# cjpurackal/nice-slam-cpp

Hardware: AMD Instinct MI355X
Metric: mapping rays/sec (and ms/iter) on CoFusion room1 at 1/2/4/8 MI355X (higher is better)
Workload: dtype f32

## Files before the change

nice-slam-cpp_amd/csrc/nsk.hip:

```cpp
#include "../../include/nsk.h"
#include "nsk_device.h"
#include "nsk_train.h"
#include "nsk_bf16.h"
#include "nsk_mesh.h"
#include "nsk_buf.h"

#include <dlfcn.h>
#include <cstdarg>
#include <algorithm>
#include <cmath>
#include <cstdio>
#include <cstring>
#include <memory>
#include <string>
#include <vector>

#define NSK_VERSION 100

static thread_local std::string g_err;
static int fail(const char* fmt, ...)
{
    char buf[512];
    va_list ap; va_start(ap, fmt); vsnprintf(buf, sizeof(buf), fmt, ap); va_end(ap);
    g_err = buf;
// ... 505 lines not shown
    float incl = act ? (1.f - alpha + 1e-10f) : 1.f;
#pragma unroll
    for (int o = 1; o < 64; o <<= 1) { float up = __shfl_up(incl, o); if (lane >= o) incl *= up; }
    float T = __shfl_up(incl, 1);
    if (lane == 0) T = 1.f;
    const float w = act ? alpha * T : 0.f;
    const float D = wave_sum(w * z);
    const float cr = wave_sum(w * r4[0]), cg = wave_sum(w * r4[1]), cb = wave_sum(w * r4[2]);
    const float V = wave_sum(w * (z - D) * (z - D));
    if (weights && act) weights[m] = w;
    if (lane == 0) { depth[n] = D; var[n] = V; rgb[3 * n] = cr; rgb[3 * n + 1] = cg; rgb[3 * n + 2] = cb; }
}

__device__ __forceinline__ void voxel_point(const float* b, int Z, int Y, int X, int v, float (&p)[3])
{
    int ix = v % X, iy = (v / X) % Y, iz = v / (X * Y);
    p[0] = add_rn(b[0], mul_rn(sub_rn(b[1], b[0]), linspace01(ix, X)));
    p[1] = add_rn(b[2], mul_rn(sub_rn(b[3], b[2]), linspace01(iy, Y)));
    p[2] = add_rn(b[4], mul_rn(sub_rn(b[5], b[4]), linspace01(iz, Z)));
}
struct FrustumArgs { float bound[6]; float w2c[16]; float cam[3]; int Z, Y, X, H, W; float fx, fy, cx, cy; };
__global__ void k_frustum_pass1(FrustumArgs A, const float* __restrict__ img, float* __restrict__ dep, float* __restrict__ zz,
                                uint8_t* __restrict__ inimg, unsigned int* __restrict__ dmax_bits)
{
    const int n = A.Z * A.Y * A.X;
    const int v = blockIdx.x * blockDim.x + threadIdx.x;
    float d = 0.f;
    if (v < n) {
        float p[3], cam[3];
        voxel_point(A.bound, A.Z, A.Y, A.X, v, p);
        for (int a = 0; a < 3; ++a)
            cam[a] = add_rn(add_rn(add_rn(mul_rn(A.w2c[4 * a], p[0]), mul_rn(A.w2c[4 * a + 1], p[1])), mul_rn(A.w2c[4 * a + 2], p[2])), A.w2c[4 * a + 3]);
        cam[0] = -cam[0];
        const float z = add_rn(cam[2], 1e-5f);
        const float u = div_rn(add_rn(mul_rn(A.fx, cam[0]), mul_rn(A.cx, cam[2])), z);
        const float w = div_rn(add_rn(mul_rn(A.fy, cam[1]), mul_rn(A.cy, cam[2])), z);
        const float x0 = floorf(u), y0 = floorf(w);
        const float ax = sub_rn(u, x0), ay = sub_rn(w, y0);
        const int ix = (int)x0, iy = (int)y0;
        float s = 0.f;
        for (int dy = 0; dy < 2; ++dy) for (int dx = 0; dx < 2; ++dx) {
            int x = ix + dx, y = iy + dy;
            if (x < 0 || x >= A.W || y < 0 || y >= A.H) continue;
            s = add_rn(s, mul_rn(mul_rn(dx ? ax : sub_rn(1.f, ax), dy ? ay : sub_rn(1.f, ay)), img[(size_t)y * A.W + x]));
        }
        d = s;
        dep[v] = d; zz[v] = z;
        inimg[v] = (u < (float)A.W && u > 0.f && w < (float)A.H && w > 0.f) ? 1 : 0;
    }
    float m = wave_max(fmaxf(d, 0.f));
    if ((threadIdx.x & 63) == 0) atomicMax(dmax_bits, __float_as_uint(m));
}
__global__ void k_frustum_pass2(FrustumArgs A, const float* __restrict__ dep, const float* __restrict__ zz, const uint8_t* __restrict__ inimg,
                                const unsigned int* __restrict__ dmax_bits, uint8_t* __restrict__ mask)
{
    const int n = A.Z * A.Y * A.X;
    const int v = blockIdx.x * blockDim.x + threadIdx.x;
    if (v >= n) return;
    const float dmax = __uint_as_float(*dmax_bits);
    const float d = dep[v] == 0.f ? dmax : dep[v];
    const float nz = -zz[v];
    int m = inimg[v] && (0.f <= nz) && (nz <= add_rn(d, 0.5f));
    float p[3];
    voxel_point(A.bound, A.Z, A.Y, A.X, v, p);
    const float dx = sub_rn(p[0], A.cam[0]), dy = sub_rn(p[1], A.cam[1]), dz = sub_rn(p[2], A.cam[2]);
    if (add_rn(add_rn(mul_rn(dx, dx), mul_rn(dy, dy)), mul_rn(dz, dz)) < 0.25f) m = 1;
    mask[v] = (uint8_t)m;
}

struct OverlapArgs { int N, ns, H, W, K; float fx, fy, cx, cy; };
__global__ __launch_bounds__(256) void k_keyframe_overlap(OverlapArgs A, const float* __restrict__ ro, const float* __restrict__ rd,
                                                           const float* __restrict__ gd, const float* __restrict__ w2c_all,
                                                           float* __restrict__ percent)
{
    __shared__ int sh[4];
    const float* w2c = w2c_all + 16 * blockIdx.x;
    const int total = A.N * A.ns;
    int count = 0;
    for (int i = threadIdx.x; i < total; i += blockDim.x) {
        const int n = i / A.ns, s = i - n * A.ns;
        const float nearv = mul_rn(gd[n], 0.8f), farv = add_rn(gd[n], 0.5f);
        const float t = linspace01(s, A.ns);
        const float z = add_rn(mul_rn(nearv, sub_rn(1.f, t)), mul_rn(farv, t));
        float p[3], cam[3];
        for (int a = 0; a < 3; ++a) p[a] = add_rn(ro[3 * n + a], mul_rn(rd[3 * n + a], z));
        for (int a = 0; a < 3; ++a)
            cam[a] = add_rn(add_rn(add_rn(mul_rn(w2c[4 * a], p[0]), mul_rn(w2c[4 * a + 1], p[1])), mul_rn(w2c[4 * a + 2], p[2])), w2c[4 * a + 3]);
        cam[0] = -cam[0];
        const float zc = add_rn(cam[2], 1e-5f);
        const float u = div_rn(add_rn(mul_rn(A.fx, cam[0]), mul_rn(A.cx, cam[2])), zc);
        const float v = div_rn(add_rn(mul_rn(A.fy, cam[1]), mul_rn(A.cy, cam[2])), zc);
        if (u < (float)(A.W - 20) && u > 20.f && v < (float)(A.H - 20) && v > 20.f && zc < 0.f) ++count;
    }
#pragma unroll
    for (int o = 32; o > 0; o >>= 1) count += __shfl_xor(count, o);
    if ((threadIdx.x & 63) == 0) sh[threadIdx.x >> 6] = count;
    __syncthreads();
    if (threadIdx.x == 0) percent[blockIdx.x] = div_rn((float)(sh[0] + sh[1] + sh[2] + sh[3]), (float)total);
}

__global__ void k_sample_pixels(unsigned long long seed, int n, int H0, int W0, int Ww, unsigned long long total, int* __restrict__ pi,
                                int* __restrict__ pj)
{
    const int r = blockIdx.x * blockDim.x + threadIdx.x;
    if (r >= n) return;
    const unsigned long long ind = ((unsigned long long)hash_u32(seed, (uint32_t)r, 0x51u) * total) >> 32;
    pi[r] = W0 + (int)(ind % (unsigned long long)Ww);
    pj[r] = H0 + (int)(ind / (unsigned long long)Ww);
}
__global__ void k_gather_pixels(int n, const int* __restrict__ pi, const int* __restrict__ pj, int W, const float* __restrict__ depth,
                                const float* __restrict__ color, float* __restrict__ gd, float* __restrict__ gc)
{
    const int r = blockIdx.x * blockDim.x + threadIdx.x;
    if (r >= n) return;
    const size_t p = (size_t)pj[r] * W + pi[r];
    gd[r] = depth[p];
    if (color && gc) { gc[3 * r] = color[3 * p]; gc[3 * r + 1] = color[3 * p + 1]; gc[3 * r + 2] = color[3 * p + 2]; }
}

struct HipAlloc {
    static int alloc(void** p, size_t bytes) { return (int)hipMalloc(p, bytes); }
    static void free(void* p) { (void)hipFree(p); }
};
template <typename T> using Buf = DevBuf<T, HipAlloc>;

struct GridState {
    int C = 0, Z = 0, Y = 0, X = 0;
    size_t n = 0;
    Buf<float> v, m, s;
    Buf<uint8_t> mask;
    size_t g_off = 0;
    Buf<int> midx; int nmask = 0; bool midx_dirty = true;
};
struct DecState {
    int n = 0;
    Buf<float> p, m, s;
    Buf<float> fimg, bimg;
    Buf<int> fidx, bidx;
    Buf<int> finv, binv;
    Buf<int> inv16;
    Buf<int> invh;
    Buf<float> bimg16; Buf<int> bidx16; int bfrag16_n = 0; bool bimg16_dirty = true;
    Buf<float> fimg16; Buf<int> fidx16; int frag16_n = 0, fimg16_f = 0, tail_off = 0, tail16_off = 0, np16 = 3, cq16 = 2;
    int fimg_n = 0, bimg_n = 0;
    int trainable = 0;
    bool loaded = false;
    size_t g_off = 0;
};
struct Workspace {
    int capM = 0, capN = 0;
    Buf<float> z, occ[3], rgb4;
    Buf<unsigned long long> masks[4];
    Buf<f4> hsave[4];
    int hsave_M[4] = {0, 0, 0, 0};
    Buf<float> g_raw, ray_loss;
    Buf<float> tmp_rgb, tmp_depth, tmp_var;
    Buf<float> dec_slabs;
    Buf<int> perm, skey, srank;
    Buf<int> hist_raw, offs;
    int* hist() const { return hist_raw ? hist_raw.get() + 16 : nullptr; }
    Buf<float> z_alt; Buf<int> perm_alt, skey_alt, srank_alt, offs_alt;
};
struct nsk_ctx {
    int device = 0;
    hipStream_t stream = nullptr;
    bool own_stream = false;
    int num_cu = 256;
    RParams R;
    Buf<float> d_bound;
    GridState grid[4];
    DecState dec[4];
    Buf<float> slab; size_t slab_n = 0;
    Buf<float> xbuf; size_t xbuf_n = 0;
    bool x_identity = false;
    bool xlevels[4] = {false, false, false, false}; bool xdecs[4] = {false, false, false, false};
    Workspace ws;
    Buf<float> scal;
    Buf<uint8_t> fr_tmp;
    int adam_step[NSK_NUM_GROUPS] = {0, 0, 0, 0, 0, 0};
    bool capturing = false;
    struct CapAdam { AdamArgs args; int group[8]; float lr[8]; };
    std::vector<CapAdam> cap_adams;
    struct CapVec { int n; float* p; const float* g; float* m; float* v; float lr, b1, b2, eps; int step; hipGraphNode_t node; float ss, bc2s; };
    std::vector<CapVec> cap_vecs;
    int cap_rollback[NSK_NUM_GROUPS] = {0, 0, 0, 0, 0, 0};
    int ws_flip = 0;
    struct GraphRec { bool stale = false; int flip = 0; hipGraph_t graph = nullptr; hipGraphExec_t exec = nullptr; hipGraphNode_t adam_node = nullptr; bool has_adam = false; CapAdam adam; std::vector<CapVec> vecs; };
    std::vector<GraphRec> graphs;
    bool touched[NSK_NUM_GROUPS] = {false, false, false, false, false, false};
    bool deterministic = false;
    bool roctx = false;
    int tune_fwd_occ_cost = 0, tune_no_occ_role = 0;
    int tune_fwd_fine_cost = 0, tune_fwd_color_cost = 0;
    bool median_fused_pending = false;
    int tune_no_deferred_median = 0;
    int tune_no_fused_median = 0;
    int tune_frozen_cost = 0;
    int tune_frozen_cost_rays = 0;
    int tune_frozen_mid_pct = 100;
    int tune_no_frozen_kernel = 0;
    const uint8_t* ray_mask = nullptr;
    struct DMax { const float* gt = nullptr; const uint8_t* keep = nullptr; int n = 0; } dmax;
    float* xextra = nullptr; size_t xextra_n = 0;
    int sort_mode = -1;
    bool sorted = false;
    struct Prep { bool valid = false; int stage = 0, N = 0, S = 0; const float* ro = nullptr; const float* rd = nullptr; const float* gt = nullptr;
                  float gtmax = 0.f; const uint8_t* mask = nullptr; bool sorted = false; int done = 0; RParams R; DMax dmax; } prep, req;
    int tune_no_piggyback = 0;
    int pend_w = -1, pend_nb = 0;
    int dbg_M = 0, dbg_S = 0;
    int bwd_mode = 2;
    int matmul_mode = 2;
    double last_bytes = 0, last_flops = 0; int last_samples = 0;
    struct Mesh {
        Buf<float> lat_pts;
        int slab = 0;
        Buf<uint8_t> cellcase; Buf<int> emap;
        Buf<unsigned> scan;
        Buf<int8_t> table; Buf<uint8_t> ntri;
        Buf<float> verts; Buf<int> tris;
        int nv = 0, nt = 0;
    } mesh;
    bool prof = false;
    struct ProfRec { const char* name; hipEvent_t a, b; };
    std::vector<ProfRec> prof_recs;
    ~nsk_ctx();
};

typedef int (*roctx_push_t)(const char*);
typedef int (*roctx_pop_t)(void);
static roctx_push_t g_roctx_push = nullptr;
static roctx_pop_t g_roctx_pop = nullptr;
static bool roctx_ready()
{
    static int state = 0;
    if (state == 0) {
        void* h = dlopen("libroctx64.so", RTLD_NOW | RTLD_GLOBAL);
        if (!h) h = dlopen("libroctx64.so.4", RTLD_NOW | RTLD_GLOBAL);
        if (h) { g_roctx_push = (roctx_push_t)dlsym(h, "roctxRangePushA"); g_roctx_pop = (roctx_pop_t)dlsym(h, "roctxRangePop"); }
        state = (g_roctx_push && g_roctx_pop) ? 1 : -1;
    }
    return state == 1;
}

struct ProfScope {
    nsk_ctx* c; hipEvent_t a = nullptr, b = nullptr; const char* name; bool ranged = false;
    ProfScope(nsk_ctx* c_, const char* n, bool on = true) : c(c_), name(n)
    {
        if (!on) return;
        if (c->roctx && roctx_ready()) { g_roctx_push(n); ranged = true; }
        if (!c->prof) return;
        hipEventCreate(&a); hipEventCreate(&b);
        hipEventRecord(a, c->stream);
    }
    ~ProfScope()
    {
        if (ranged) g_roctx_pop();
        if (!c->prof || !a) return;
        hipEventRecord(b, c->stream);
        c->prof_recs.push_back({name, a, b});
    }
};

static void invalidate_graphs(nsk_ctx* c)
{
    for (auto& R : c->graphs) {
        if (R.stale) continue;
        if (R.exec) { hipGraphExecDestroy(R.exec); R.exec = nullptr; }
        if (R.graph) { hipGraphDestroy(R.graph); R.graph = nullptr; }
        R.stale = true;
    }
}

nsk_ctx::~nsk_ctx()
{
    hipSetDevice(device);
    if (stream) hipStreamSynchronize(stream);
    invalidate_graphs(this);
    for (auto& r : prof_recs) { hipEventDestroy(r.a); hipEventDestroy(r.b); }
    if (own_stream && stream) hipStreamDestroy(stream);
}

template <typename T>
static int dev_alloc(Buf<T>& b, size_t n, const char* what)
{
    const int e = b.alloc(n);
    if (e == 0) return 0;
    (void)hipGetLastError();
    return fail("cannot allocate %zu bytes for %s (%s)", n * sizeof(T), what, hipGetErrorString((hipError_t)e));
}
enum { GROW_NO_CAPTURE = 1,
       GROW_STALE_GRAPHS = 2 };
static int grow_begin(nsk_ctx* c, unsigned flags)
{
    if ((flags & GROW_NO_CAPTURE) && c->capturing) return fail("graph capture: the workspace must grow (run the same step once before nsk_graph_begin)");
    HIPCHK(hipStreamSynchronize(c->stream));
    if (flags & GROW_STALE_GRAPHS) invalidate_graphs(c);
    return 0;
}
template <typename T>
static int grow(nsk_ctx* c, Buf<T>& b, size_t n, const char* what, unsigned flags)
{
    if (n <= b.cap()) return 0;
    CHK(grow_begin(c, flags));
    return dev_alloc(b, n, what);
}

extern "C" const char* nsk_last_error(void) { return g_err.c_str(); }
extern "C" int nsk_version(void) { return NSK_VERSION; }

static int which_ok(int w) { return w >= 0 && w < 4; }

template <typename K>
static int set_lds(K kern, size_t bytes)
{
    HIPCHK(hipFuncSetAttribute(reinterpret_cast<const void*>(kern), hipFuncAttributeMaxDynamicSharedMemorySize, (int)bytes));
    return 0;
}

static size_t fwd_img_floats(int w) { return w == 0 ? CoarseFwdImg::TOTAL : (w == 2 ? MlpFwdImg<4>::TOTAL : MlpFwdImg<2>::TOTAL); }
static size_t bwd_img_floats(int w) { return w == 0 ? CoarseBwdImg::TOTAL : MlpBwdImg::TOTAL; }
static size_t bwd_lds_bytes(int w, bool train)
{
    size_t scratch = 8 * 3840;
    if (!train) return bwd_img_floats(w) * 4 + scratch;
    if (w == 1 || w == 3) return PM_LDS_BYTES;
    size_t img = w == 2 ? 0 : bwd_img_floats(w);
    return (img + PN_FLOATS(w == 2 ? 4 : 2)) * 4;
}

extern "C" int nsk_ctx_create(int device, void* hip_stream, nsk_ctx** out)
{
    if (!out) return fail("nsk_ctx_create: out is NULL");
    int ndev = 0;
    hipError_t e = hipGetDeviceCount(&ndev);
    if (e != hipSuccess || ndev <= 0) return fail("nsk_ctx_create: no HIP device (the MI355X kernels have no CPU fallback)");
    if (device < 0 || device >= ndev) return fail("nsk_ctx_create: device %d out of range (%d devices)", device, ndev);
    HIPCHK(hipSetDevice(device));
    hipDeviceProp_t prop;
    HIPCHK(hipGetDeviceProperties(&prop, device));
    if (strncmp(prop.gcnArchName, "gfx950", 6) != 0) return fail("nsk_ctx_create: device arch %s, this library is built for gfx950 only", prop.gcnArchName);
    std::unique_ptr<nsk_ctx> owner(new nsk_ctx());
    nsk_ctx* c = owner.get();
    c->device = device;
    c->num_cu = prop.multiProcessorCount;
    if (hip_stream) { c->stream = (hipStream_t)hip_stream; c->own_stream = false; }
    else { HIPCHK(hipStreamCreateWithFlags(&c->stream, hipStreamNonBlocking)); c->own_stream = true; }
    const float b[6] = {-4.5f, 3.82f, -1.5f, 2.02f, -3.0f, 2.76f};
    memcpy(c->R.bound, b, sizeof(b));
    c->R.n_samples = 32; c->R.n_surface = 16; c->R.lindisp = 0; c->R.occupancy = 0; c->R.perturb = 0.f; c->R.seed = 0;
    CHK(dev_alloc(c->d_bound, 6, "the bound"));
    HIPCHK(hipMemcpy(c->d_bound, b, sizeof(b), hipMemcpyHostToDevice));
    CHK(dev_alloc(c->scal, 16, "the scalars"));
    HIPCHK(hipMemset(c->scal, 0, 16 * sizeof(float)));
    CHK(set_lds(k_decode_fwd<0>, fwd_img_floats(0) * 4)); CHK(set_lds(k_decode_fwd<1>, fwd_img_floats(1) * 4));
    CHK(set_lds(k_decode_fwd<2>, fwd_img_floats(2) * 4)); CHK(set_lds(k_decode_fwd<3>, fwd_img_floats(3) * 4));
#define SETB(W) \
    CHK(set_lds(k_decode_bwd<W, false>, bwd_lds_bytes(W, false))); CHK(set_lds(k_decode_bwd<W, true>, bwd_lds_bytes(W, false))); \
    CHK(set_lds(k_decode_bwd_train<W, false>, bwd_lds_bytes(W, true))); CHK(set_lds(k_decode_bwd_train<W, true>, bwd_lds_bytes(W, true)));
    SETB(0) SETB(1) SETB(2) SETB(3)
#undef SETB
    CHK(set_lds(k_median_thr, 16384 * 4));
    CHK(set_lds(k_decode_fwd_multi, 160 * 1024)); CHK(set_lds(k_decode_fwd_multi_bf16<8>, 160 * 1024)); CHK(set_lds(k_decode_fwd_multi_bf16<8, 2>, 160 * 1024)); CHK(set_lds(k_decode_fwd_multi_occ<8>, 160 * 1024));
    CHK(set_lds(k_decode_bwd_multi<false>, 160 * 1024 - 256)); CHK(set_lds(k_decode_bwd_multi<true>, 160 * 1024));
    CHK(set_lds(k_decode_bwd_frozen<false>, 160 * 1024 - 256));
    CHK(set_lds(k_decode_bwd_track, 160 * 1024)); CHK(set_lds(k_decode_bwd_multi_full<false>, 160 * 1024)); CHK(set_lds(k_decode_bwd_multi_full<true>, 160 * 1024));
    CHK(set_lds(k_decode_fwd_dump<0>, 160 * 1024)); CHK(set_lds(k_decode_fwd_dump<1>, 160 * 1024)); CHK(set_lds(k_decode_fwd_dump<2>, 160 * 1024));
    *out = owner.release();
    return 0;
}

extern "C" int nsk_ctx_destroy(nsk_ctx* c)
{
    delete c;
    return 0;
}

extern "C" int nsk_sync(nsk_ctx* c)
{
    if (!c) return fail("null ctx");
    HIPCHK(hipStreamSynchronize(c->stream));
    if (c->median_fused_pending) {
        c->median_fused_pending = false;
        unsigned bar[3] = {0, 0, 0};
        HIPCHK(hipMemcpy(bar, c->scal + 5, sizeof(bar), hipMemcpyDeviceToHost));
        if (bar[2]) {
            HIPCHK(hipMemset(c->scal + 5, 0, sizeof(bar)));
            return fail("nsk_track_step: the grid barrier of the fused median timed out (threshold was infinite for that step); nsk_set_tuning(\"no_fused_median\", 1) selects the three-launch form");
        }
    }
    return 0;
}
extern "C" void* nsk_stream(nsk_ctx* c) { return c ? (void*)c->stream : nullptr; }

static int repack16(nsk_ctx* c, int w);
extern "C" int nsk_set_matmul_mode(nsk_ctx* c, int mode)
{
    if (!c) return fail("null ctx");
    if (mode < 0 || mode > 2) return fail("nsk_set_matmul_mode: mode must be 0 (fp32 MFMA), 1 (bf16 3-piece split) or 2 (fp16 2-piece split)");
    if (c->capturing) return fail("nsk_set_matmul_mode: not while a graph is being captured");
    const bool relayout = (mode == 2) != (c->matmul_mode == 2);
    c->matmul_mode = mode;
    if (relayout) {
        HIPCHK(hipSetDevice(c->device));
        for (int w = 1; w < 4; ++w) if (c->dec[w].loaded && c->dec[w].fimg16) CHK(repack16(c, w));
        invalidate_graphs(c);
    }
    return 0;
}

extern "C" int nsk_set_backward_mode(nsk_ctx* c, int mode)
{
    if (!c) return fail("null ctx");
    if (mode != 0 && mode != 2) return fail("nsk_set_backward_mode: 0 (fp32 MFMA chains) or 2 (two fp16 pieces, default)");
    c->bwd_mode = mode;
    return 0;
}

extern "C" int nsk_set_tuning(nsk_ctx* c, const char* key, int value)
{
    if (!c || !key) return fail("nsk_set_tuning: null argument");
    if (!strcmp(key, "frozen_cost")) { c->tune_frozen_cost = value; return 0; }
    if (!strcmp(key, "frozen_cost_rays")) { c->tune_frozen_cost_rays = value; return 0; }
    if (!strcmp(key, "no_frozen_kernel")) { c->tune_no_frozen_kernel = value; return 0; }
    if (!strcmp(key, "no_piggyback")) { c->tune_no_piggyback = value; return 0; }
    if (!strcmp(key, "frozen_mid_pct")) { if (value < 10 || value > 1000) return fail("nsk_set_tuning: frozen_mid_pct out of range"); c->tune_frozen_mid_pct = value; return 0; }
    if (!strcmp(key, "no_fused_median")) { c->tune_no_fused_median = value; return 0; }
    if (!strcmp(key, "no_deferred_median")) { c->tune_no_deferred_median = value; return 0; }
    if (!strcmp(key, "fwd_fine_cost")) { c->tune_fwd_fine_cost = value; return 0; }
    if (!strcmp(key, "fwd_occ_cost")) { c->tune_fwd_occ_cost = value; return 0; }
    if (!strcmp(key, "no_occ_role")) { c->tune_no_occ_role = value; return 0; }
    if (!strcmp(key, "fwd_color_cost")) { c->tune_fwd_color_cost = value; return 0; }
    if (!strcmp(key, "deterministic")) { c->deterministic = value != 0; return 0; }
    if (!strcmp(key, "roctx")) { c->roctx = value != 0; return 0; }
    if (!strcmp(key, "lattice_slab")) { if (value < 0 || value >= (1 << 26)) return fail("nsk_set_tuning: lattice_slab must be 0 (automatic) or a node count below 2^26"); c->mesh.slab = value; return 0; }
    return fail("nsk_set_tuning: unknown key '%s'", key);
}

extern "C" int nsk_set_ray_mask(nsk_ctx* c, const uint8_t* d_keep)
{
    if (!c) return fail("null ctx");
    c->ray_mask = d_keep;
    return 0;
}

extern "C" int nsk_set_sort_mode(nsk_ctx* c, int mode)
{
    if (!c) return fail("null ctx");
    if (mode < -1 || mode > 1) return fail("nsk_set_sort_mode: mode must be -1 (automatic), 0 (never) or 1 (always)");
    c->sort_mode = mode;
    return 0;
}

extern "C" int nsk_set_bound(nsk_ctx* c, const float h_bound[6])
{
    if (!c || !h_bound) return fail("nsk_set_bound: null argument");
    for (int k = 0; k < 3; ++k) if (!(h_bound[2 * k + 1] > h_bound[2 * k])) return fail("nsk_set_bound: empty axis %d", k);
    memcpy(c->R.bound, h_bound, 6 * sizeof(float));
    HIPCHK(hipMemcpyAsync(c->d_bound, c->R.bound, 6 * sizeof(float), hipMemcpyHostToDevice, c->stream));
    HIPCHK(hipStreamSynchronize(c->stream));
    return 0;
}

extern "C" int nsk_set_render_opts(nsk_ctx* c, int n_samples, int n_surface, int lindisp, float perturb, int occupancy, uint64_t seed)
{
    if (!c) return fail("null ctx");
    if (n_samples < 1 || n_surface < 0 || n_samples + n_surface > 64) return fail("nsk_set_render_opts: need 1 <= n_samples, n_samples+n_surface <= 64 (got %d+%d)", n_samples, n_surface);
    c->R.n_samples = n_samples; c->R.n_surface = n_surface; c->R.lindisp = lindisp ? 1 : 0; c->R.perturb = perturb;
    c->R.occupancy = occupancy ? 1 : 0; c->R.seed = seed;
    return 0;
}

static int rebuild_slab(nsk_ctx* c)
{
    size_t n = 0;
    for (int i = 0; i < 4; ++i) { c->grid[i].g_off = n; n += c->grid[i].n; }
    for (int i = 0; i < 4; ++i) { c->dec[i].g_off = n; n += (size_t)((c->dec[i].n + 3) & ~3); }
    n += 4;
    if (n != c->slab_n) {
        CHK(grow_begin(c, GROW_STALE_GRAPHS));
        c->slab_n = 0;
        CHK(dev_alloc(c->slab, n, "the gradient slab"));
        c->slab_n = n;
    }
    HIPCHK(hipMemsetAsync(c->slab, 0, n * sizeof(float), c->stream));
    return 0;
}

static int grid_upload(nsk_ctx* c, GridState& G, const float* h, int C, int Z, int Y, int X)
{
    size_t nvox = (size_t)Z * Y * X, n = nvox * 32;
    bool realloc_ = n != G.n;
    if (realloc_) {
        CHK(grow_begin(c, GROW_STALE_GRAPHS));
        G = GridState();
        CHK(dev_alloc(G.v, n, "a grid level")); CHK(dev_alloc(G.m, n, "a grid level's first moment")); CHK(dev_alloc(G.s, n, "a grid level's second moment"));
    }
    if (G.Z != Z || G.Y != Y || G.X != X) { if (G.mask) { CHK(grow_begin(c, GROW_STALE_GRAPHS)); G.mask.reset(); } }
    G.C = C; G.Z = Z; G.Y = Y; G.X = X; G.n = n; G.midx_dirty = true;
    std::vector<float> t(n);
    for (int ch = 0; ch < 32; ++ch)
        for (size_t v = 0; v < nvox; ++v) t[v * 32 + ch] = h[(size_t)ch * nvox + v];
    HIPCHK(hipMemcpyAsync(G.v, t.data(), n * 4, hipMemcpyHostToDevice, c->stream));
    HIPCHK(hipMemsetAsync(G.m, 0, n * 4, c->stream));
    HIPCHK(hipMemsetAsync(G.s, 0, n * 4, c->stream));
    HIPCHK(hipStreamSynchronize(c->stream));
    if (realloc_) CHK(rebuild_slab(c));
    return 0;
}
extern "C" int nsk_grid_upload(nsk_ctx* c, int level, const float* h, int C, int Z, int Y, int X)
{
    if (!c || !h) return fail("nsk_grid_upload: null argument");
    if (!which_ok(level)) return fail("nsk_grid_upload: bad level %d", level);
    if (C != 32) return fail("nsk_grid_upload: C must be 32 (got %d)", C);
    if (Z < 1 || Y < 1 || X < 1) return fail("nsk_grid_upload: bad shape");
    if ((size_t)Z * Y * X >= ((size_t)1 << 25)) return fail("nsk_grid_upload: at most 2^25 - 1 voxels per level (32-bit byte offsets in the forward's gather: 128 B per voxel)");
    HIPCHK(hipSetDevice(c->device));
    GridState& G = c->grid[level];
    const bool fresh = (size_t)Z * Y * X * 32 != G.n;
    const int r = grid_upload(c, G, h, C, Z, Y, X);
    if (r != 0 && fresh) { invalidate_graphs(c); G = GridState(); }
    return r;
}

static int grid_fetch(nsk_ctx* c, int level, const float* src, float* h)
{
    GridState& G = c->grid[level];
    if (!G.n) return fail("grid level %d not uploaded", level);
    std::vector<float> t(G.n);
    HIPCHK(hipMemcpyAsync(t.data(), src, G.n * 4, hipMemcpyDeviceToHost, c->stream));
    HIPCHK(hipStreamSynchronize(c->stream));
    size_t nvox = G.n / 32;
    for (int ch = 0; ch < 32; ++ch)
        for (size_t v = 0; v < nvox; ++v) h[(size_t)ch * nvox + v] = t[v * 32 + ch];
    return 0;
}
extern "C" int nsk_grid_download(nsk_ctx* c, int level, float* h)
{
    if (!c || !h || !which_ok(level)) return fail("nsk_grid_download: bad argument");
    return grid_fetch(c, level, c->grid[level].v, h);
}
extern "C" int nsk_grid_grad_download(nsk_ctx* c, int level, float* h)
{
    if (!c || !h || !which_ok(level)) return fail("nsk_grid_grad_download: bad argument");
    CHK(grid_fetch(c, level, c->slab + c->grid[level].g_off, h));
    GridState& G = c->grid[level];
    if (G.mask) {
        const size_t nvox = G.n / 32;
        std::vector<uint8_t> m(nvox);
        HIPCHK(hipMemcpy(m.data(), G.mask, nvox, hipMemcpyDeviceToHost));
        for (int ch = 0; ch < 32; ++ch)
            for (size_t v = 0; v < nvox; ++v) if (!m[v]) h[(size_t)ch * nvox + v] = 0.f;
    }
    return 0;
}

extern "C" int nsk_set_mask(nsk_ctx* c, int level, const uint8_t* h_mask)
{
    if (!c || !which_ok(level)) return fail("nsk_set_mask: bad argument");
    GridState& G = c->grid[level];
    if (!G.n) return fail("nsk_set_mask: grid level %d not uploaded", level);
    if (c->capturing) return fail("nsk_set_mask: not while a graph is being captured");
    HIPCHK(hipStreamSynchronize(c->stream));
    size_t nvox = G.n / 32;
    G.midx_dirty = true;
    invalidate_graphs(c);
    if (c->slab) HIPCHK(hipMemsetAsync(c->slab + G.g_off, 0, G.n * 4, c->stream));
    if (!h_mask) { G.mask.reset(); return 0; }
    if (!G.mask) CHK(dev_alloc(G.mask, nvox, "the voxel mask"));
    HIPCHK(hipMemcpy(G.mask, h_mask, nvox, hipMemcpyHostToDevice));
    return 0;
}

static void seg_fwd(std::vector<int>& idx, int quad0, int KQ, int Wofs, int ld, int col0, int kvalid)
{
    for (int rt = 0; rt < 2; ++rt) for (int q = 0; q < KQ; ++q) for (int lane = 0; lane < 64; ++lane) for (int i = 0; i < 4; ++i) {
        int o = 16 * rt + (lane & 15), k = 16 * q + 4 * (lane >> 4) + i;
// ... 125 lines not shown
    k_pack<<<(D.bimg_n + 255) / 256, 256, 0, c->stream>>>(D.bimg, D.bidx, D.p, D.bimg_n);
    HIPCHK(hipGetLastError());
    CHK(repack16(c, w));
    D.bimg16_dirty = true;
    return 0;
}

static int flush_pending(nsk_ctx* c);
static int ensure_midx(nsk_ctx* c, int l);
static void adam_consts(float lr, float b1, float b2, int step, float& step_size, float& bc2s);

extern "C" size_t nsk_decoder_param_count(int which) { return which_ok(which) ? (size_t)nsk_dec_layout(which).total : 0; }

static int dec_setup(int w, size_t n, DecState& D)
{
    const size_t n4 = (n + 3) & ~(size_t)3;
    auto table = [](Buf<int>& d, const std::vector<int>& h, const char* what) -> int {
        CHK(dev_alloc(d, h.size(), what));
        HIPCHK(hipMemcpy(d, h.data(), h.size() * 4, hipMemcpyHostToDevice));
        return 0;
    };
    auto inverse = [&](Buf<int>& d, const std::vector<int>& idx, const char* image) -> int {
        std::vector<int> inv(n4, -1);
        for (size_t k = 0; k < idx.size(); ++k) if (idx[k] >= 0) { if (inv[idx[k]] != -1) return fail("decoder %d: parameter %d appears twice in the %s image", w, idx[k], image); inv[idx[k]] = (int)k; }
        return table(d, inv, "a decoder's inverse index table");
    };
    CHK(dev_alloc(D.p, n4, "a decoder's parameters")); CHK(dev_alloc(D.m, n4, "a decoder's first moment")); CHK(dev_alloc(D.s, n4, "a decoder's second moment"));
    HIPCHK(hipMemset(D.p, 0, n4 * 4));
    std::vector<int> fi, bi;
    build_idx(w, fi, bi);
    D.fimg_n = (int)fi.size(); D.bimg_n = (int)bi.size();
    CHK(dev_alloc(D.fimg, fi.size(), "a decoder's forward image")); CHK(dev_alloc(D.bimg, bi.size(), "a decoder's backward image"));
    CHK(table(D.fidx, fi, "a decoder's index table")); CHK(table(D.bidx, bi, "a decoder's index table"));
    if (w != 0) {
        std::vector<int> i16;
        if (w == 2) { build_idx16<4>(nsk_dec_layout(w), i16); D.cq16 = 4; D.tail_off = MlpFwdImg<4>::P_B; }
        else { build_idx16<2>(nsk_dec_layout(w), i16); D.cq16 = 2; D.tail_off = MlpFwdImg<2>::P_B; }
        set_np16(D, 3);
        D.frag16_n = (int)i16.size();
        CHK(dev_alloc(D.fimg16, (size_t)D.fimg16_f, "a decoder's forward image in pieces")); CHK(table(D.fidx16, i16, "a decoder's index table"));
        HIPCHK(hipMemset(D.fimg16, 0, (size_t)D.fimg16_f * 4));
        std::vector<int> ib;
        build_idx16b(nsk_dec_layout(w), ib);
        D.bfrag16_n = (int)ib.size();
        CHK(dev_alloc(D.bimg16, (size_t)MlpBwdImgH::TOTAL_F, "a decoder's backward image in pieces")); CHK(table(D.bidx16, ib, "a decoder's index table"));
        HIPCHK(hipMemset(D.bimg16, 0, (size_t)MlpBwdImgH::TOTAL_F * 4));
        CHK(inverse(D.invh, ib, "fp16 backward"));
        CHK(inverse(D.inv16, i16, "bf16"));
    }
    CHK(inverse(D.finv, fi, "forward"));
    CHK(inverse(D.binv, bi, "backward"));
    D.n = (int)n;
    return 0;
}

extern "C" int nsk_decoder_upload(nsk_ctx* c, int w, const float* h, size_t n)
{
    if (!c || !h || !which_ok(w)) return fail("nsk_decoder_upload: bad argument");
    if (n != nsk_decoder_param_count(w)) return fail("nsk_decoder_upload: decoder %d expects %zu parameters, got %zu", w, nsk_decoder_param_count(w), n);
    HIPCHK(hipSetDevice(c->device));
    DecState& D = c->dec[w];
    if (!D.n) {
        DecState fresh;
        fresh.trainable = D.trainable;
        CHK(dec_setup(w, n, fresh));
        D = std::move(fresh);
        const int r = rebuild_slab(c);
        if (r != 0) { const int t = D.trainable; D = DecState(); D.trainable = t; return r; }
    }
    HIPCHK(hipMemcpyAsync(D.p, h, n * 4, hipMemcpyHostToDevice, c->stream));
    size_t n4 = (n + 3) & ~(size_t)3;
    HIPCHK(hipMemsetAsync(D.m, 0, n4 * 4, c->stream));
    HIPCHK(hipMemsetAsync(D.s, 0, n4 * 4, c->stream));
    CHK(repack(c, w));
    HIPCHK(hipStreamSynchronize(c->stream));
    D.loaded = true;
    return 0;
}

static int dec_fetch(nsk_ctx* c, int w, const float* src, float* h, size_t n)
{
    if (!c->dec[w].loaded) return fail("decoder %d not uploaded", w);
    if (n != (size_t)c->dec[w].n) return fail("decoder %d has %d parameters, buffer has %zu", w, c->dec[w].n, n);
    HIPCHK(hipMemcpyAsync(h, src, n * 4, hipMemcpyDeviceToHost, c->stream));
    HIPCHK(hipStreamSynchronize(c->stream));
    return 0;
}
extern "C" int nsk_decoder_download(nsk_ctx* c, int w, float* h, size_t n)
{
    if (!c || !h || !which_ok(w)) return fail("nsk_decoder_download: bad argument");
    return dec_fetch(c, w, c->dec[w].p, h, n);
}
extern "C" int nsk_decoder_grad_download(nsk_ctx* c, int w, float* h, size_t n)
{
    if (!c || !h || !which_ok(w)) return fail("nsk_decoder_grad_download: bad argument");
    CHK(flush_pending(c));
    return dec_fetch(c, w, c->slab + c->dec[w].g_off, h, n);
}
extern "C" int nsk_decoder_set_trainable(nsk_ctx* c, int w, int t)
{
    if (!c || !which_ok(w)) return fail("nsk_decoder_set_trainable: bad argument");
    c->dec[w].trainable = t ? 1 : 0;
    return 0;
}

static int prep_drop(nsk_ctx* c);
static int ensure_ws(nsk_ctx* c, int N, int M)
{
    Workspace& w = c->ws;
    if (M <= w.capM && N <= w.capN) return 0;
    CHK(grow_begin(c, GROW_NO_CAPTURE | GROW_STALE_GRAPHS));
    CHK(prep_drop(c));
    const int capM = std::max(M, w.capM), capN = std::max(N, w.capN);
    w = Workspace();
    const size_t m = (size_t)capM + 64, n = (size_t)capN + 64, slabs = (size_t)c->num_cu * 20920;
    const int r = [&]() -> int {
        CHK(dev_alloc(w.z, m, "the sample depths"));
        for (int i = 0; i < 3; ++i) CHK(dev_alloc(w.occ[i], m, "the occupancies"));
        CHK(dev_alloc(w.rgb4, m * 4, "the colours"));
        for (int i = 0; i < 4; ++i) CHK(dev_alloc(w.masks[i], m * 4, "the ReLU bits"));
        CHK(dev_alloc(w.g_raw, m * 4, "the sample gradients"));
        CHK(dev_alloc(w.ray_loss, n, "the ray losses"));
        CHK(dev_alloc(w.tmp_rgb, n * 3, "the ray colours")); CHK(dev_alloc(w.tmp_depth, n, "the ray depths")); CHK(dev_alloc(w.tmp_var, n, "the ray variances"));
        CHK(dev_alloc(w.dec_slabs, slabs, "the decoder gradient slabs"));
        HIPCHK(hipMemsetAsync(w.dec_slabs, 0, slabs * 4, c->stream));
        CHK(dev_alloc(w.perm, m, "the cell sort")); CHK(dev_alloc(w.skey, m, "the cell sort")); CHK(dev_alloc(w.srank, m, "the cell sort"));
        return 0;
    }();
    if (r != 0) { w = Workspace(); return r; }
    w.capM = capM; w.capN = capN;
    return 0;
}

static int ensure_hist(nsk_ctx* c, size_t bins)
{
    Workspace& w = c->ws;
    if (bins <= w.offs.cap()) return 0;
    CHK(grow_begin(c, GROW_NO_CAPTURE | GROW_STALE_GRAPHS));
    c->prep.valid = false; c->req.valid = false;
    const size_t slots = ((bins / 8 + 1) / 2) * 16 + 16;
    const int r = [&]() -> int {
        CHK(dev_alloc(w.hist_raw, slots, "the cell histogram")); CHK(dev_alloc(w.offs, bins, "the cell offsets"));
        HIPCHK(hipMemsetAsync(w.hist_raw, 0, slots * 4, c->stream));
        return 0;
    }();
    if (r != 0) reset_all(w.hist_raw, w.offs);
    return r;
}

static bool saves_h(nsk_ctx* c, int w, bool save_masks) { return save_masks && w != 2 && c->dec[w].trainable; }
static int ensure_hsave(nsk_ctx* c, int w, int M)
{
    const size_t tiles = (size_t)(M + 15) / 16 + 1;
    return grow(c, c->ws.hsave[w], tiles * 10 * 64, "the saved block outputs", GROW_NO_CAPTURE | GROW_STALE_GRAPHS);
}

static const int STAGE_DEC[4][3] = {{0, -1, -1}, {1, -1, -1}, {1, 2, -1}, {1, 2, 3}};

static GridD grid_dev(nsk_ctx* c, int level, bool with_grad)
{
    GridD g;
    GridState& G = c->grid[level];
    g.v = G.v; g.g = with_grad ? c->slab + G.g_off : nullptr; g.mask = G.mask; g.Z = G.Z; g.Y = G.Y; g.X = G.X;
    return g;
}

static int check_stage(nsk_ctx* c, int stage)
{
    if (stage < 0 || stage > 3) return fail("bad stage %d", stage);
    for (int q = 0; q < 3; ++q) {
        int w = STAGE_DEC[stage][q];
        if (w < 0) break;
        if (!c->grid[w].n) return fail("stage %d needs grid level %d (nsk_grid_upload)", stage, w);
        if (!c->dec[w].loaded) return fail("stage %d needs decoder %d (nsk_decoder_upload)", stage, w);
    }
    if (!c->slab) return fail("the gradient slab is not allocated (its last allocation failed: upload a grid level or a decoder again)");
    return 0;
}

static void fill_args(nsk_ctx* c, DecArgs& A, int w, int M, int S, const float* ro, const float* rd, const float* pts)
{
    memset(&A, 0, sizeof(A));
    A.rays_o = ro; A.rays_d = rd; A.z = c->ws.z; A.pts = pts; A.M = M; A.S = S; A.S_magic = S > 1 ? (unsigned)((0x100000000ull + (unsigned)S - 1) / (unsigned)S) : 0u;
    A.perm = (c->sorted && !pts) ? c->ws.perm : nullptr;
    memcpy(A.bound, c->R.bound, sizeof(A.bound));
    A.grid = grid_dev(c, w, false);
    if (w == 2) A.grid_mid = grid_dev(c, 1, false);
    A.img = reinterpret_cast<const f4*>(c->dec[w].fimg.get());
    A.bimg = reinterpret_cast<const f4*>(c->dec[w].bimg.get());
    A.img_f4 = c->dec[w].fimg_n / 4;
    A.img16 = c->dec[w].fimg16;
    A.bimg16 = c->dec[w].bimg16;
    A.out = w == 3 ? c->ws.rgb4 : c->ws.occ[w];
}

static int launch_decode_fwd(nsk_ctx* c, int w, int M, int S, const float* ro, const float* rd, const float* pts, bool save_masks)
{
    DecArgs A;
    fill_args(c, A, w, M, S, ro, rd, pts);
    A.masks = save_masks ? c->ws.masks[w] : nullptr;
    if (save_masks) c->ws.hsave_M[w] = 0;
    if (saves_h(c, w, save_masks)) { CHK(ensure_hsave(c, w, M)); A.hsave = c->ws.hsave[w]; c->ws.hsave_M[w] = M; }
    int ntasks = (M + 15) / 16;
    size_t lds = fwd_img_floats(w) * 4;
    int maxwg = c->num_cu;
    int grid = std::max(1, std::min((ntasks + 7) / 8, maxwg));
    static const char* names[4] = {"decode_fwd_coarse", "decode_fwd_middle", "decode_fwd_fine", "decode_fwd_color"};
    ProfScope ps(c, names[w]);
    switch (w) {
    case 0: k_decode_fwd<0><<<grid, 512, lds, c->stream>>>(A); break;
    case 1: k_decode_fwd<1><<<grid, 512, lds, c->stream>>>(A); break;
    case 2: k_decode_fwd<2><<<grid, 512, lds, c->stream>>>(A); break;
    default: k_decode_fwd<3><<<grid, 512, lds, c->stream>>>(A); break;
    }
    HIPCHK(hipGetLastError());
    return 0;
}

static int launch_decode_bwd(nsk_ctx* c, int w, int M, int S, const float* ro, const float* rd, bool train, bool rays, unsigned flags,
                             float* g_ro, float* g_rd)
{
    DecArgs A;
    fill_args(c, A, w, M, S, ro, rd, nullptr);
    A.grid = grid_dev(c, w, (flags & NSK_GRAD_GRIDS) != 0);
    A.masks = c->ws.masks[w];
    A.g_raw = c->ws.g_raw;
    A.g_rays_o = g_ro; A.g_rays_d = g_rd;
    A.g_dec = train ? c->ws.dec_slabs : c->slab + c->dec[w].g_off;
    A.flags = flags;
    if (w != 0 && (!train || w != 2)) CHK(ensure_bimg16(c, w));
    if (train && w != 2) {
        if (c->ws.hsave_M[w] != M) return fail("backward of trainable decoder %d: its forward must run with the decoder already trainable (block outputs not saved)", w);
        A.hsave = c->ws.hsave[w];
    }
    int ntasks = (M + 15) / 16;
    size_t lds = bwd_lds_bytes(w, train);
    int grid = std::max(1, std::min((ntasks + 7) / 8, c->num_cu));
    if (c->deterministic) { grid = 1; A.flags |= 0x8000u; }
    static const char* names[8] = {"decode_bwd_coarse", "decode_bwd_middle", "decode_bwd_fine", "decode_bwd_color",
                                   "decode_bwd_coarse_train", "decode_bwd_middle_train", "decode_bwd_fine_train", "decode_bwd_color_train"};
    {
    ProfScope ps(c, names[w + (train ? 4 : 0)]);
#define LB(W) \
    if (train) { if (rays) k_decode_bwd_train<W, true><<<grid, 512, lds, c->stream>>>(A); else k_decode_bwd_train<W, false><<<grid, 512, lds, c->stream>>>(A); } \
    else { if (rays) k_decode_bwd<W, true><<<grid, 512, lds, c->stream>>>(A); else k_decode_bwd<W, false><<<grid, 512, lds, c->stream>>>(A); }
    switch (w) {
    case 0: LB(0) break;
    case 1: LB(1) break;
    case 2: LB(2) break;
    default: LB(3) break;
    }
#undef LB
    }
    HIPCHK(hipGetLastError());
    if (train) {
        int n = c->dec[w].n, n4 = (n + 3) & ~3;
        ProfScope ps2(c, "dec_grad_reduce");
        k_dec_grad_reduce<<<dim3((n + 255) / 256, 8), 256, 0, c->stream>>>(n, n4, grid, c->ws.dec_slabs, c->slab + c->dec[w].g_off);
        HIPCHK(hipGetLastError());
    }
    return 0;
}

static void split_wgs(int num_cu, int ntasks, int n, const int* cost, int* wg_end, int waves = 8)
{
    int cap = std::max(1, (ntasks + waves - 1) / waves), tot = 0, used = 0;
    for (int r = 0; r < n; ++r) tot += cost[r];
    for (int r = 0; r < n; ++r) {
        int k = std::max(1, (int)((double)num_cu * cost[r] / tot));
        k = std::min(k, cap);
        used += k;
        wg_end[r] = used;
    }
}

static void split_wgs_balanced(int num_cu, int ntasks, int n, const int* cost, int* wg_end, int waves = 8)
{
    split_wgs(num_cu, ntasks, n, cost, wg_end, waves);
    int w[4];
    for (int r = 0; r < n; ++r) w[r] = wg_end[r] - (r ? wg_end[r - 1] : 0);
    int used = wg_end[n - 1];
    const int cap = std::max(1, (ntasks + waves - 1) / waves);
    auto t_of = [&](int r, int wr) { return (long)((ntasks + waves * wr - 1) / (waves * wr)) * cost[r]; };
    for (int r = 0; used < num_cu && r < 8 * n; ++r) {
        int worst = 0;
        for (int q = 1; q < n; ++q) if (t_of(q, w[q]) > t_of(worst, w[worst])) worst = q;
        if (w[worst] >= cap) break;
        ++w[worst]; ++used;
    }
    for (int it = 0; it < 64; ++it) {
        int worst = 0;
        for (int q = 1; q < n; ++q) if (t_of(q, w[q]) > t_of(worst, w[worst])) worst = q;
        const long cur = t_of(worst, w[worst]);
        if (w[worst] >= cap) break;
        int donor = -1; long best = cur;
        for (int q = 0; q < n; ++q) {
            if (q == worst || w[q] <= 1) continue;
            long m = std::max(t_of(q, w[q] - 1), t_of(worst, w[worst] + 1));
            for (int o = 0; o < n; ++o) if (o != q && o != worst) m = std::max(m, t_of(o, w[o]));
            if (m < best) { best = m; donor = q; }
        }
        if (donor < 0) break;
        --w[donor]; ++w[worst];
    }
    int acc = 0;
    for (int r = 0; r < n; ++r) { acc += w[r]; wg_end[r] = acc; }
}

static void split_wgs_train(int num_cu, int ntasks, int n, const int* cost, int train_role, int* wg_end)
{
    const int groups = std::max(1, (ntasks + 7) / 8);
    int fsum = 0;
    for (int r = 0; r < n; ++r) if (r != train_role) fsum += cost[r];
    long best = -1; int best_wt = 1;
    const int wt_max = std::min(groups, num_cu - (n - 1));
    for (int iters = (groups + wt_max - 1) / wt_max; iters <= groups; ++iters) {
        const int wt = (groups + iters - 1) / iters;
        if (wt > wt_max) continue;
        long t = (long)iters * cost[train_role];
        const int rest = num_cu - wt;
        for (int r = 0; r < n; ++r) {
            if (r == train_role) continue;
            const int wr = std::max(1, (int)((long)rest * cost[r] / std::max(1, fsum)));
            t = std::max(t, (long)((ntasks + 8 * wr - 1) / (8 * wr)) * cost[r]);
        }
        if (best < 0 || t < best) { best = t; best_wt = wt; }
        if ((long)iters * cost[train_role] > best) break;
    }
    const int rest = num_cu - best_wt;
    int used = 0;
    for (int r = 0; r < n; ++r) {
        int k = r == train_role ? best_wt : std::max(1, (int)((long)rest * cost[r] / std::max(1, fsum)));
        k = std::min(k, std::max(1, (ntasks + 7) / 8));
        used += k;
        wg_end[r] = used;
    }
}

static long split_makespan(int ntasks, int n, const int* cost, const int* wg_end, int waves = 8)
{
    long t = 0;
    for (int r = 0; r < n; ++r) {
        const int w = std::max(1, wg_end[r] - (r ? wg_end[r - 1] : 0));
        t = std::max(t, (long)((ntasks + waves * w - 1) / (waves * w)) * cost[r]);
    }
    return t;
}

static int launch_decode_fwd_stage(nsk_ctx* c, int stage, int M, int S, const float* ro, const float* rd, bool save_masks)
{
    int n = 0;
    for (int q = 0; q < 3; ++q) if (STAGE_DEC[stage][q] >= 0) ++n;
    if (n == 1) return launch_decode_fwd(c, STAGE_DEC[stage][0], M, S, ro, rd, nullptr, save_masks);
    static const int fcost[4] = {96, 240, 292, 248};
    MultiArgs MA;
    memset(&MA, 0, sizeof(MA));
    if (c->matmul_mode == 2 && c->tune_no_occ_role != 1 && STAGE_DEC[stage][0] == 1 && STAGE_DEC[stage][1] == 2 && !saves_h(c, 1, save_masks) && !saves_h(c, 2, save_masks)) {
        const bool colour = STAGE_DEC[stage][2] == 3;
        for (int r = 0; r < (colour ? 3 : 2); ++r) {
            const int w = STAGE_DEC[stage][r];
            fill_args(c, MA.a[r], w, M, S, ro, rd, nullptr);
            MA.a[r].masks = save_masks ? c->ws.masks[w] : nullptr;
            if (save_masks) c->ws.hsave_M[w] = 0;
            MA.which[r] = w;
        }
        if (colour && saves_h(c, 3, save_masks)) { CHK(ensure_hsave(c, 3, M)); MA.a[2].hsave = c->ws.hsave[3]; c->ws.hsave_M[3] = M; }
        int cost[2] = {c->tune_fwd_occ_cost > 0 ? c->tune_fwd_occ_cost : 460, c->tune_fwd_color_cost > 0 ? c->tune_fwd_color_cost : fcost[3]};
        MA.n = colour ? 2 : 1;
        split_wgs_balanced(c->num_cu, (M + 15) / 16, MA.n, cost, MA.wg_end, 8);
        if (!colour) MA.wg_end[1] = MA.wg_end[0];
        bool merged = true;
        if (c->tune_no_occ_role != 2) {
            int cost3[3], wg3[3], n3 = colour ? 3 : 2;
            for (int r = 0; r < n3; ++r) {
                const int w = STAGE_DEC[stage][r];
                cost3[r] = (w == 2 && c->tune_fwd_fine_cost > 0) ? c->tune_fwd_fine_cost : ((w == 3 && c->tune_fwd_color_cost > 0) ? c->tune_fwd_color_cost : fcost[w]);
            }
            split_wgs_balanced(c->num_cu, (M + 15) / 16, n3, cost3, wg3, 8);
            merged = split_makespan((M + 15) / 16, MA.n, cost, MA.wg_end) <= split_makespan((M + 15) / 16, n3, cost3, wg3);
        }
        if (merged) {
            size_t lds_occ = ((size_t)c->dec[1].fimg16_f + (size_t)c->dec[2].fimg16_f) * 4;
            if (colour) lds_occ = std::max(lds_occ, (size_t)c->dec[3].fimg16_f * 4);
            ProfScope ps(c, "decode_fwd_multi");
            k_decode_fwd_multi_occ<8><<<MA.wg_end[MA.n - 1], 512, lds_occ, c->stream>>>(MA);
            HIPCHK(hipGetLastError());
            return 0;
        }
        memset(&MA, 0, sizeof(MA));
    }
    int cost[3]; size_t lds = 0;
    for (int r = 0; r < n; ++r) {
        int w = STAGE_DEC[stage][r];
        fill_args(c, MA.a[r], w, M, S, ro, rd, nullptr);
        MA.a[r].masks = save_masks ? c->ws.masks[w] : nullptr;
        if (save_masks) c->ws.hsave_M[w] = 0;
        if (saves_h(c, w, save_masks)) { CHK(ensure_hsave(c, w, M)); MA.a[r].hsave = c->ws.hsave[w]; c->ws.hsave_M[w] = M; }
        MA.which[r] = w; cost[r] = (w == 2 && c->tune_fwd_fine_cost > 0) ? c->tune_fwd_fine_cost : ((w == 3 && c->tune_fwd_color_cost > 0) ? c->tune_fwd_color_cost : fcost[w]);
        lds = std::max(lds, fwd_img_floats(w) * 4);
    }
    MA.n = n;
    split_wgs_balanced(c->num_cu, (M + 15) / 16, n, cost, MA.wg_end, 8);
    ProfScope ps(c, "decode_fwd_multi");
    if (c->matmul_mode != 0) {
        size_t lds16 = 0;
        for (int r = 0; r < n; ++r) lds16 = std::max(lds16, MA.which[r] == 0 ? fwd_img_floats(0) * 4 : (size_t)c->dec[MA.which[r]].fimg16_f * 4);
        if (c->matmul_mode == 2) k_decode_fwd_multi_bf16<8, 2><<<MA.wg_end[n - 1], 512, lds16, c->stream>>>(MA);
        else k_decode_fwd_multi_bf16<8><<<MA.wg_end[n - 1], 512, lds16, c->stream>>>(MA);
    } else
    k_decode_fwd_multi<<<MA.wg_end[n - 1], 512, lds, c->stream>>>(MA);
    HIPCHK(hipGetLastError());
    return 0;
}

static void account(nsk_ctx* c, int stage, int M, int N, bool bwd, unsigned flags)
{
    static const double fwd_b[4] = {1024, 1024, 2048, 3072}, fwd_f[4] = {12.4e3, 31.0e3, 72.2e3, 103.3e3};
    double b = fwd_b[stage] + 5.0, f = fwd_f[stage];
    if (bwd) {
        int lv = stage == 0 ? 1 : stage;
        if (flags & NSK_GRAD_GRIDS) b += 2048.0 * lv;
        f *= 2.0;
        if (flags & NSK_GRAD_DECODERS) for (int q = 0; q < 3; ++q) { int w = STAGE_DEC[stage][q]; if (w >= 0 && c->dec[w].trainable) f += 2.0 * (w == 0 ? 6176 : (w == 2 ? 20599 : 15500)); }
    }
    c->last_bytes = b * M; c->last_flops = f * M; c->last_samples = M; (void)N;
}

static bool sort_pays(nsk_ctx* c, int stage, int M, unsigned flags)
{
    if (c->deterministic) return false;
    if (c->sort_mode >= 0) return c->sort_mode == 1;
    if (!(flags & NSK_GRAD_GRIDS)) return false;
    int key_level = 0;
    for (int q = 0; q < 3; ++q) if (STAGE_DEC[stage][q] >= 0) key_level = std::max(key_level, STAGE_DEC[stage][q] == 3 ? 3 : STAGE_DEC[stage][q]);
    const long cells = (long)(c->grid[key_level].n / 32);
    return M >= 14336 || (cells > 0 && (long)M >= 4 * cells);
}

static int stage_key_level(int stage)
{
    int key_level = 0;
    for (int q = 0; q < 3; ++q) if (STAGE_DEC[stage][q] >= 0) key_level = STAGE_DEC[stage][q];
    return key_level;
}
static void samp_args(nsk_ctx* c, SampArgs& A, const RParams& R, int stage, int N, int S, const float* ro, const float* rd, const float* gt, float gtmax,
                      const float* gmax_dev, const uint8_t* mask, bool sorted, float* z, int* skey, int* srank, const nsk_ctx::DMax& dm)
{
    const GridState& KG = c->grid[stage_key_level(stage)];
    const GridState* PG = stage >= 2 ? &c->grid[1] : nullptr;
    const size_t bins = KG.n / 32 * 8;
    memset(&A, 0, sizeof(A));
    A.R = R; A.N = N; A.S = S; A.rays_o = ro; A.rays_d = rd; A.gt_depth = gt; A.gtmax_host = gtmax; A.gtmax_dev = gmax_dev; A.keep = mask; A.z_out = z;
    A.kX = KG.X; A.kY = KG.Y; A.kZ = KG.Z; A.pX = PG ? PG->X : 0; A.pY = PG ? PG->Y : 0; A.pZ = PG ? PG->Z : 0; A.ncell2 = (int)((bins / 8 + 1) / 2);
    A.skey = sorted ? skey : nullptr; A.srank = srank; A.hist = c->ws.hist();
    if (dm.n > 0) { A.mx_gt = dm.gt; A.mx_keep = dm.keep; A.mx_n = dm.n; } else { A.mx_gt = gt; A.mx_keep = mask; A.mx_n = N; }
}
static ScanArgs scan_args(nsk_ctx* c, int stage, int* offs, int halves)
{
    const size_t bins = c->grid[stage_key_level(stage)].n / 32 * 8;
    ScanArgs A; A.nkeys = (int)bins; A.ncell2 = (int)((bins / 8 + 1) / 2); A.hist = c->ws.hist(); A.offs = offs;
    A.nblocks = (int)((bins + 2048 * (size_t)halves - 1) / (2048 * (size_t)halves));
    return A;
}
static PlaceArgs place_args(int M, const int* skey, const int* srank, const int* offs, int* perm)
{
    PlaceArgs A; A.M = M; A.skey = skey; A.srank = srank; A.offs = offs; A.perm = perm; A.nblocks = (M + 255) / 256;
    return A;
}
static bool needs_depth_max(const float* gt, float gtmax, int N, const nsk_ctx::DMax& dm) { return gt && gtmax < 0.f && (dm.n > 0 ? dm.n : N) > 8192; }

static int launch_sampling(nsk_ctx* c, const RParams& R, int stage, int N, int S, const float* ro, const float* rd, const float* gt, float gtmax,
                           const uint8_t* mask, bool sorted, float* z, int* skey, int* srank, int* offs, int* perm, const nsk_ctx::DMax& dm, int done = 0)
{
    const int M = N * S;
    hipStream_t st = c->stream;
    if (!(done & 1)) {
        const float* gmax_dev = nullptr;
        if (needs_depth_max(gt, gtmax, N, dm)) {
            ProfScope ps(c, "depth_max");
            if (dm.n > 0) k_depth_max<<<1, 1024, 0, st>>>(dm.n, dm.gt, dm.keep, c->scal);
            else k_depth_max<<<1, 1024, 0, st>>>(N, gt, mask, c->scal);
            gmax_dev = c->scal;
        }
        ProfScope ps(c, "sample");
        SampArgs A;
        samp_args(c, A, R, stage, N, S, ro, rd, gt, gtmax, gmax_dev, mask, sorted, z, skey, srank, dm);
        k_sample<<<(N + NSK_SAMPLE_RAYS - 1) / NSK_SAMPLE_RAYS, 64 * NSK_SAMPLE_RAYS, 0, st>>>(A);
    }
    if (sorted && (done & 6) != 6) {
        ProfScope ps(c, "cell_sort");
        if (!(done & 2)) { const ScanArgs A = scan_args(c, stage, offs, 1); k_sort_scan<<<A.nblocks, 256, 0, st>>>(A); }
        if (!(done & 4)) { const PlaceArgs A = place_args(M, skey, srank, offs, perm); k_sort_place<<<A.nblocks, 256, 0, st>>>(A); }
    }
    HIPCHK(hipGetLastError());
    return 0;
}

static int prep_finish(nsk_ctx* c)
{
    nsk_ctx::Prep& P = c->prep;
    if (!P.valid) return 0;
    const int all = P.sorted ? 7 : 1;
    if ((P.done & all) == all) return 0;
    Workspace& w = c->ws;
    CHK(launch_sampling(c, P.R, P.stage, P.N, P.S, P.ro, P.rd, P.gt, P.gtmax, P.mask, P.sorted, w.z_alt, w.skey_alt, w.srank_alt, w.offs_alt, w.perm_alt, P.dmax, P.done));
    P.done = all;
    return 0;
}
static int prep_drop(nsk_ctx* c)
{
    nsk_ctx::Prep& P = c->prep;
    if (P.valid && P.sorted && (P.done & 1) && !(P.done & 2)) { const ScanArgs A = scan_args(c, P.stage, c->ws.offs_alt, 1); k_sort_scan<<<A.nblocks, 256, 0, c->stream>>>(A); HIPCHK(hipGetLastError()); }
    P.valid = false; c->req.valid = false;
    return 0;
}

static size_t stage_bins(nsk_ctx* c, int stage) { return c->grid[stage_key_level(stage)].n / 32 * 8; }

static int forward_core(nsk_ctx* c, int stage, int N, int S, const float* ro, const float* rd, const float* gt, float gtmax, bool save_masks,
                        bool sorted = false)
{
    const int M = N * S;
    const uint8_t* mask = save_masks ? c->ray_mask : nullptr;
    auto is_this_batch = [&](const nsk_ctx::Prep& X) {
        return X.valid && save_masks && !c->capturing && X.stage == stage && X.N == N && X.S == S && X.ro == ro && X.rd == rd && X.gt == gt && X.gtmax == gtmax &&
               X.mask == mask && X.sorted == sorted && memcmp(&X.R, &c->R, sizeof(RParams)) == 0 &&
               X.dmax.gt == c->dmax.gt && X.dmax.keep == c->dmax.keep && X.dmax.n == c->dmax.n;
    };
    nsk_ctx::Prep& P = c->prep;
    if (!c->capturing) CHK(prep_finish(c));
    if (is_this_batch(P)) {
        Workspace& w = c->ws;
        w.z.swap(w.z_alt); w.perm.swap(w.perm_alt); w.skey.swap(w.skey_alt); w.srank.swap(w.srank_alt);
        w.offs.swap(w.offs_alt);
        c->ws_flip ^= 1;
        P.valid = false;
        c->sorted = sorted;
    } else {
        if (is_this_batch(c->req)) c->req.valid = false;
        c->sorted = sorted;
        if (sorted) CHK(ensure_hist(c, stage_bins(c, stage)));
        CHK(launch_sampling(c, c->R, stage, N, S, ro, rd, gt, gtmax, mask, sorted, c->ws.z, c->ws.skey, c->ws.srank, c->ws.offs, c->ws.perm, c->dmax));
    }
    CHK(launch_decode_fwd_stage(c, stage, M, S, ro, rd, save_masks));
    c->dbg_M = M; c->dbg_S = S;
    return 0;
}

static void comp_args(nsk_ctx* c, CompArgs& A, int stage, int N, int S, const float* ro, const float* rd)
{
// ... 104 lines not shown
            CHK(launch_decode_fwd(c, w, cnt, 1, nullptr, nullptr, pts, false));
        }
        { ProfScope ps(c, "lattice_finish");
          k_lattice_finish<<<(cnt + 255) / 256, 256, 0, c->stream>>>(cnt, pts, c->d_bound, st == 0 ? c->ws.occ[0] : c->ws.occ[1], st >= 2 ? c->ws.occ[2] : nullptr, vol + n0); }
        HIPCHK(hipGetLastError());
    }
    return 0;
}

static size_t mc_scan_words(size_t n)
{
    size_t words = 0;
    for (;;) { words += (n + 63) & ~(size_t)63; if (n <= MC_BLOCK) return words; n = (n + MC_BLOCK - 1) / MC_BLOCK; }
}
static int mc_scan(nsk_ctx* c, unsigned* d, int n)
{
    const int nb = (n + MC_BLOCK - 1) / MC_BLOCK;
    unsigned* sums = d + ((n + 63) & ~63);
    k_mc_scan_block<<<nb, MC_BLOCK, 0, c->stream>>>(d, n, nb > 1 ? sums : nullptr);
    HIPCHK(hipGetLastError());
    if (nb == 1) return 0;
    CHK(mc_scan(c, sums, nb));
    k_mc_scan_add<<<nb, MC_BLOCK, 0, c->stream>>>(d, n, sums);
    HIPCHK(hipGetLastError());
    return 0;
}

extern "C" int nsk_mesh_extract(nsk_ctx* c, const float* vol, const uint8_t* valid, int nx, int ny, int nz, const float* o, const float* s,
                                float level, int* n_vertices, int* n_triangles)
{
    CHK(lattice_checks("nsk_mesh_extract", c, o, s, nx, ny, nz, 2));
    if (!vol) return fail("nsk_mesh_extract: d_volume is NULL");
    if (!n_vertices || !n_triangles) return fail("nsk_mesh_extract: n_vertices / n_triangles is NULL");
    if (std::isnan(level)) return fail("nsk_mesh_extract: level is NaN");
    const long long total = (long long)nx * ny * nz;
    if (total > MC_MAX_NODES) return fail("nsk_mesh_extract: %lld nodes, at most %lld per call", total, (long long)MC_MAX_NODES);
    HIPCHK(hipSetDevice(c->device));
    nsk_ctx::Mesh& M = c->mesh;
    M.nv = M.nt = 0;
    *n_vertices = *n_triangles = 0;
    const int nn = (int)total, nb = (nn + MC_BLOCK - 1) / MC_BLOCK;
    if (!M.ntri) {
        const McTable& T = mc_table();
        const int r = [&]() -> int {
            CHK(dev_alloc(M.table, sizeof(T.edges), "the case table")); CHK(dev_alloc(M.ntri, sizeof(T.ntri), "the case table"));
            HIPCHK(hipMemcpy(M.table, T.edges, sizeof(T.edges), hipMemcpyHostToDevice));
            HIPCHK(hipMemcpy(M.ntri, T.ntri, sizeof(T.ntri), hipMemcpyHostToDevice));
            return 0;
        }();
        if (r != 0) { reset_all(M.table, M.ntri); return r; }
    }
    int r = grow(c, M.cellcase, (size_t)nn, "the cell cases", 0);
    if (r == 0) r = grow(c, M.emap, (size_t)nn * 3, "the edge map", 0);
    if (r != 0) { reset_all(M.cellcase, M.emap); return r; }
    const size_t words = mc_scan_words((size_t)nb + 1);
    CHK(grow(c, M.scan, 2 * words, "the scan scratch", 0));
    unsigned* sv = M.scan; unsigned* stri = M.scan + words;
    McGeom G;
    G.nx = nx; G.ny = ny; G.nz = nz; G.nn = nn; G.level = level;
    for (int a = 0; a < 3; ++a) { G.o[a] = o[a]; G.s[a] = s[a]; }
    HIPCHK(hipMemsetAsync(M.scan, 0, 2 * words * 4, c->stream));
    { ProfScope ps(c, "mc_cells"); k_mc_cells<<<nb, MC_BLOCK, 0, c->stream>>>(G, vol, valid, M.ntri, M.cellcase, stri); }
    HIPCHK(hipGetLastError());
    { ProfScope ps(c, "mc_edge_count"); k_mc_edges<false><<<nb, MC_BLOCK, 0, c->stream>>>(G, vol, M.cellcase, sv, nullptr, nullptr, nullptr); }
    HIPCHK(hipGetLastError());
    { ProfScope ps(c, "mc_scan"); CHK(mc_scan(c, sv, nb + 1)); CHK(mc_scan(c, stri, nb + 1)); }
    unsigned tot[2] = {0, 0};
    HIPCHK(hipMemcpyAsync(&tot[0], sv + nb, 4, hipMemcpyDeviceToHost, c->stream));
    HIPCHK(hipMemcpyAsync(&tot[1], stri + nb, 4, hipMemcpyDeviceToHost, c->stream));
    HIPCHK(hipStreamSynchronize(c->stream));
    if (tot[0] > 0x7fffffffu / 3 || tot[1] > 0x7fffffffu / 3) return fail("nsk_mesh_extract: %u vertices, %u triangles do not fit 32-bit indices", tot[0], tot[1]);
    CHK(grow(c, M.verts, (size_t)tot[0] * 3, "the vertices", 0));
    CHK(grow(c, M.tris, (size_t)tot[1] * 3, "the triangles", 0));
    if (tot[0]) {
        { ProfScope ps(c, "mc_vertices"); k_mc_edges<true><<<nb, MC_BLOCK, 0, c->stream>>>(G, vol, M.cellcase, nullptr, sv, M.emap, M.verts); }
        HIPCHK(hipGetLastError());
    }
    if (tot[1]) {
        { ProfScope ps(c, "mc_triangles"); k_mc_tris<<<nb, MC_BLOCK, 0, c->stream>>>(G, M.cellcase, M.ntri, M.table, stri, M.emap, M.tris); }
        HIPCHK(hipGetLastError());
    }
    HIPCHK(hipStreamSynchronize(c->stream));
    M.nv = (int)tot[0]; M.nt = (int)tot[1];
    *n_vertices = M.nv; *n_triangles = M.nt;
    return 0;
}

extern "C" int nsk_mesh_buffers(nsk_ctx* c, float** d_vertices, int32_t** d_triangles)
{
    if (!c) return fail("null ctx");
    if (d_vertices) *d_vertices = c->mesh.nv ? c->mesh.verts : nullptr;
    if (d_triangles) *d_triangles = c->mesh.nt ? c->mesh.tris : nullptr;
    return 0;
}

extern "C" int nsk_mesh_download(nsk_ctx* c, float* h_vertices, int32_t* h_triangles)
{
    if (!c) return fail("null ctx");
    HIPCHK(hipSetDevice(c->device));
    HIPCHK(hipStreamSynchronize(c->stream));
    if (h_vertices && c->mesh.nv) HIPCHK(hipMemcpy(h_vertices, c->mesh.verts, (size_t)c->mesh.nv * 12, hipMemcpyDeviceToHost));
    if (h_triangles && c->mesh.nt) HIPCHK(hipMemcpy(h_triangles, c->mesh.tris, (size_t)c->mesh.nt * 12, hipMemcpyDeviceToHost));
    return 0;
}

extern "C" int nsk_mesh_table(int case_index, int8_t* h_edges, int capacity)
{
    if (case_index < 0 || case_index > 255) return fail("nsk_mesh_table: case %d out of range", case_index);
    const McTable& T = mc_table();
    const int n = 3 * T.ntri[case_index];
    if (h_edges) {
        if (capacity < n) return fail("nsk_mesh_table: case %d has %d entries, capacity %d", case_index, n, capacity);
        memcpy(h_edges, T.edges[case_index], (size_t)n);
    }
    return T.ntri[case_index];
}

static int flush_pending(nsk_ctx* c)
{
    if (c->pend_w < 0) return 0;
    const int w = c->pend_w, np = c->dec[w].n, n4 = (np + 3) & ~3;
    ProfScope ps(c, "dec_grad_reduce");
    k_dec_grad_reduce<<<dim3((np + 255) / 256, 8), 256, 0, c->stream>>>(np, n4, c->pend_nb, c->ws.dec_slabs, c->slab + c->dec[w].g_off);
    HIPCHK(hipGetLastError());
    c->pend_w = -1;
    return 0;
}

static int backward_core(nsk_ctx* c, int stage, int N, int S, const float* ro, const float* rd, unsigned flags, float* g_ro, float* g_rd,
                         float* d_loss = nullptr, const float* dyn_resid = nullptr)
{
    const bool rays = (flags & NSK_GRAD_RAYS) != 0;
    const bool grids = (flags & NSK_GRAD_GRIDS) != 0;
    const int M = N * S;
    CHK(flush_pending(c));
    MultiArgs MA;
    memset(&MA, 0, sizeof(MA));
    int n = 0, cost[3], train_role = -1; size_t lds = 0;
    for (int q = 2; q >= 0; --q) {
        int w = STAGE_DEC[stage][q];
        if (w < 0) continue;
        bool train = (flags & NSK_GRAD_DECODERS) && c->dec[w].trainable;
        if (!train && !grids && !rays) continue;
        DecArgs& A = MA.a[n];
        fill_args(c, A, w, M, S, ro, rd, nullptr);
        A.grid = grid_dev(c, w, grids);
        A.masks = c->ws.masks[w];
        A.g_raw = c->ws.g_raw;
        A.g_rays_o = g_ro; A.g_rays_d = g_rd;
        A.dyn_resid = dyn_resid; A.dyn_n = N;
        A.g_dec = train ? c->ws.dec_slabs : c->slab + c->dec[w].g_off;
        A.flags = flags & 0xffu;
        if (w != 0 && (!train || w != 2)) CHK(ensure_bimg16(c, w));
        if (train && w != 2) {
            if (c->ws.hsave_M[w] != M) return fail("backward of trainable decoder %d: its forward must run with the decoder already trainable (block outputs not saved)", w);
            A.hsave = c->ws.hsave[w];
        }
        MA.which[n] = w; MA.train[n] = train ? 1 : 0;
        const int frozen_cost = rays ? (c->tune_frozen_cost_rays > 0 ? c->tune_frozen_cost_rays : 330) : (c->tune_frozen_cost > 0 ? c->tune_frozen_cost : 205);
        cost[n] = train ? 1000 : (w == 1 ? frozen_cost * c->tune_frozen_mid_pct / 100 : frozen_cost);
        lds = std::max(lds, bwd_lds_bytes(w, train));
        if (train) train_role = (train_role == -1 && w != 2) ? n : -2;
        if (train) c->touched[NSK_GROUP_DECODERS] = true;
        if (grids) c->touched[NSK_GROUP_COARSE + w] = true;
        ++n;
    }
    if (dyn_resid && (train_role != -1 || !rays || c->deterministic || c->bwd_mode == 0 || n == 0 || N > NSK_MEDIAN_FUSED_MAX))
        return fail("backward_core: the deferred median mask needs the Tracker's launch (frozen decoders, ray gradients)");
    const int separate = c->deterministic ? 1 : 0;
    if ((n == 0 || train_role == -2 || separate) && d_loss) { ProfScope ps(c, "loss_sum"); k_sum<<<1, 1024, 0, c->stream>>>(N, c->ws.ray_loss, d_loss); }
    if (n == 0) return 0;
    if (train_role == -2 || separate) {
        for (int r = 0; r < n; ++r)
            CHK(launch_decode_bwd(c, MA.which[r], M, S, ro, rd, MA.train[r] != 0, rays, flags, g_ro, g_rd));
        return 0;
    }
    MA.n = n;
    const bool full = c->bwd_mode == 0;
    const bool frozen_only = train_role == -1 && !rays && !c->tune_no_frozen_kernel && !full;
    if (train_role >= 0 && n > 1) split_wgs_train(c->num_cu, (M + 15) / 16, n, cost, train_role, MA.wg_end);
    else split_wgs_balanced(c->num_cu, (M + 15) / 16, n, cost, MA.wg_end, frozen_only ? NSK_FROZEN_NW : 8);
    const int extra = d_loss ? 1 : 0;
    if (d_loss) { MA.sum_src = c->ws.ray_loss; MA.sum_dst = d_loss; MA.sum_n = N; }
    int scan_wgs = 0;
    {
        nsk_ctx::Prep& P = c->prep;
        if (P.valid && P.sorted && (P.done & 3) == 1 && !rays && !full && !c->capturing && !c->tune_no_piggyback) {
            MA.scan = scan_args(c, P.stage, c->ws.offs_alt, frozen_only ? NSK_FROZEN_NW / 4 : 2);
            scan_wgs = MA.scan.nblocks;
            P.done |= 2;
        }
    }
    {
        ProfScope ps(c, "decode_bwd_multi");
        if (dyn_resid) {
            MA.dyn_seed = c->ws.tmp_rgb; MA.dyn_thr_out = c->scal + 1;
            k_decode_bwd_track<<<MA.wg_end[n - 1] + 1, 512, lds + NSK_DYN_LDS_BYTES, c->stream>>>(MA);
        } else if (full) {
            size_t ldsf = 0;
            for (int r = 0; r < n; ++r) {
                const int w = MA.which[r];
                ldsf = std::max(ldsf, MA.train[r] ? (bwd_img_floats(w) + PN_FLOATS(2)) * 4 : bwd_img_floats(w) * 4 + 8 * 3840);
            }
            if (rays) k_decode_bwd_multi_full<true><<<MA.wg_end[n - 1] + extra, 512, ldsf, c->stream>>>(MA);
            else k_decode_bwd_multi_full<false><<<MA.wg_end[n - 1] + extra, 512, ldsf, c->stream>>>(MA);
        } else if (frozen_only) {
            const size_t lds16 = lds - 8 * 3840 + (size_t)NSK_FROZEN_NW * 3840;
            k_decode_bwd_frozen<false><<<MA.wg_end[n - 1] + scan_wgs + extra, 64 * NSK_FROZEN_NW, lds16, c->stream>>>(MA);
        } else if (rays) k_decode_bwd_multi<true><<<MA.wg_end[n - 1] + extra, 512, lds, c->stream>>>(MA);
        else k_decode_bwd_multi<false><<<MA.wg_end[n - 1] + scan_wgs + extra, 512, lds, c->stream>>>(MA);
    }
    HIPCHK(hipGetLastError());
    if (train_role >= 0) {
        int w = MA.which[train_role];
        int nb = MA.wg_end[train_role] - (train_role == 0 ? 0 : MA.wg_end[train_role - 1]);
        c->pend_w = w; c->pend_nb = nb;
    }
    return 0;
}

extern "C" int nsk_render_backward(nsk_ctx* c, int stage, int N, const float* ro, const float* rd, const float* gt, float gtmax,
                                   const float* g_rgb, const float* g_depth, const float* g_var, unsigned flags, float* g_ro, float* g_rd)
{
    int S;
    CHK(common_checks(c, stage, N, ro, rd, &S, gt));
    if (!g_rgb || !g_depth) return fail("nsk_render_backward: g_rgb / g_depth is NULL");
    if ((flags & NSK_GRAD_RAYS) && (!g_ro || !g_rd)) return fail("nsk_render_backward: NSK_GRAD_RAYS needs g_rays_o and g_rays_d");
    CHK(forward_core(c, stage, N, S, ro, rd, gt, gtmax, true, sort_pays(c, stage, N * S, flags)));
    CompArgs A;
    comp_args(c, A, stage, N, S, ro, rd);
    A.mode = 1; A.g_rgb = g_rgb; A.g_depth = g_depth; A.g_var = g_var;
    if (flags & NSK_GRAD_RAYS) { A.g_rays_o = g_ro; A.g_rays_d = g_rd; }
    { ProfScope ps(c, "composite"); k_composite<<<(N + 3) / 4, 256, 0, c->stream>>>(A); }
    HIPCHK(hipGetLastError());
    CHK(backward_core(c, stage, N, S, ro, rd, flags, g_ro, g_rd));
    account(c, stage, N * S, N, true, flags);
    return 0;
}

static int ensure_alt(nsk_ctx* c, bool need_offs)
{
    Workspace& w = c->ws;
    const size_t m = (size_t)w.capM + 64;
    const int r = [&]() -> int {
        CHK(grow(c, w.z_alt, m, "the second sampling set", 0)); CHK(grow(c, w.perm_alt, m, "the second sampling set", 0));
        CHK(grow(c, w.skey_alt, m, "the second sampling set", 0)); CHK(grow(c, w.srank_alt, m, "the second sampling set", 0));
        return 0;
    }();
    if (r != 0) { reset_all(w.z_alt, w.perm_alt, w.skey_alt, w.srank_alt); return r; }
    if (need_offs) CHK(grow(c, w.offs_alt, w.offs.cap(), "the second sampling set's offsets", 0));
    return 0;
}

extern "C" int nsk_map_prepare(nsk_ctx* c, int stage, int N, const float* ro, const float* rd, const float* gt, float gtmax, unsigned flags)
{
    int S;
    if (!gt) return fail("nsk_map_prepare: gt_depth is NULL");
    if (c && c->capturing) return fail("nsk_map_prepare: not inside a graph capture");
    CHK(common_checks(c, stage, N, ro, rd, &S, gt));
    const bool sorted = sort_pays(c, stage, N * S, flags);
    if (sorted) CHK(ensure_hist(c, stage_bins(c, stage)));
    CHK(ensure_alt(c, sorted));
    nsk_ctx::Prep& P = c->req;
    P.valid = true; P.stage = stage; P.N = N; P.S = S; P.ro = ro; P.rd = rd; P.gt = gt; P.gtmax = gtmax; P.mask = c->ray_mask; P.sorted = sorted; P.done = 0; P.R = c->R; P.dmax = c->dmax;
    return 0;
}

static int prep_promote(nsk_ctx* c, bool* ride)
{
    *ride = false;
    if (!c->req.valid || c->capturing) return 0;
    if (c->prep.valid) { const nsk_ctx::Prep keep = c->req; CHK(prep_drop(c)); c->req = keep; }
    const nsk_ctx::Prep R = c->req;
    if (R.sorted) CHK(ensure_hist(c, stage_bins(c, R.stage)));
    CHK(ensure_alt(c, R.sorted));
    c->prep = R; c->prep.done = 0; c->req.valid = false;
    *ride = !c->tune_no_piggyback && !needs_depth_max(R.gt, R.gtmax, R.N, R.dmax);
    return 0;
}

extern "C" int nsk_map_step(nsk_ctx* c, int stage, int N, const float* ro, const float* rd, const float* gt, const float* gtc,
                            float gtmax, float w_color, int use_color, unsigned flags, float* d_loss, float* rgb, float* depth,
                            float* var, float* g_ro, float* g_rd)
{
    int S;
    if (!gt) return fail("nsk_map_step: gt_depth is NULL");
    if (use_color && !gtc) return fail("nsk_map_step: use_color needs gt_color");
    CHK(common_checks(c, stage, N, ro, rd, &S, gt));
    if ((flags & NSK_GRAD_RAYS) && (!g_ro || !g_rd)) return fail("nsk_map_step: NSK_GRAD_RAYS needs g_rays_o and g_rays_d");
    CHK(forward_core(c, stage, N, S, ro, rd, gt, gtmax, true, sort_pays(c, stage, N * S, flags)));
    CompArgs A;
    comp_args(c, A, stage, N, S, ro, rd);
    A.mode = 2; A.gt_depth = gt; A.gt_color = gtc; A.w_color = w_color; A.use_color = use_color;
    A.rgb = rgb; A.depth = depth; A.var = var; A.loss = c->ws.ray_loss;
    if (flags & NSK_GRAD_RAYS) { A.g_rays_o = g_ro; A.g_rays_d = g_rd; }
    bool ride = false;
    CHK(prep_promote(c, &ride));
    if (ride) {
        nsk_ctx::Prep& P = c->prep;
        SampArgs SA;
        samp_args(c, SA, P.R, P.stage, P.N, P.S, P.ro, P.rd, P.gt, P.gtmax, nullptr, P.mask, P.sorted, c->ws.z_alt, c->ws.skey_alt, c->ws.srank_alt, P.dmax);
        const int cb = (N + 7) / 8, sb = (P.N + NSK_SAMPLE_RAYS - 1) / NSK_SAMPLE_RAYS;
        { ProfScope ps(c, "composite"); k_composite_sample<<<cb + sb, 512, 0, c->stream>>>(A, SA, cb); }
        P.done |= 1;
    } else {
        ProfScope ps(c, "composite"); k_composite<<<(N + 3) / 4, 256, 0, c->stream>>>(A);
    }
    HIPCHK(hipGetLastError());
    CHK(backward_core(c, stage, N, S, ro, rd, flags, g_ro, g_rd, d_loss));
    account(c, stage, N * S, N, true, flags);
    return 0;
}

static int median_thr(nsk_ctx* c, int N, const float* gt, const float* depth)
{
    int P2 = 1; while (P2 < N) P2 <<= 1;
    if (P2 > 16384) return fail("handle_dynamic median supports at most 16384 rays (got %d)", N);
    k_median_thr<<<1, 1024, P2 * 4, c->stream>>>(N, P2, gt, depth, c->ray_mask, c->scal + 1);
    HIPCHK(hipGetLastError());
    return 0;
}

extern "C" int nsk_track_step(nsk_ctx* c, int stage, int N, const float* ro, const float* rd, const float* gt, const float* gtc,
                              float gtmax, float w_color, int use_color, int handle_dynamic, int detach_var, unsigned flags,
                              float* d_loss, float* g_ro, float* g_rd)
{
    int S;
    if (!gt) return fail("nsk_track_step: gt_depth is NULL");
    if (use_color && !gtc) return fail("nsk_track_step: use_color needs gt_color");
    CHK(common_checks(c, stage, N, ro, rd, &S, gt));
    if ((flags & NSK_GRAD_RAYS) && (!g_ro || !g_rd)) return fail("nsk_track_step: NSK_GRAD_RAYS needs g_rays_o and g_rays_d");
    CHK(forward_core(c, stage, N, S, ro, rd, gt, gtmax, true, sort_pays(c, stage, N * S, flags)));
    CompArgs A;
    comp_args(c, A, stage, N, S, ro, rd);
    const bool fused_median = handle_dynamic && !c->deterministic && !c->tune_no_fused_median && N <= NSK_MEDIAN_FUSED_MAX && (N + 3) / 4 <= c->num_cu;
    bool deferred = handle_dynamic && !c->deterministic && !c->tune_no_fused_median && !c->tune_no_deferred_median && N <= NSK_MEDIAN_FUSED_MAX &&
                    (flags & NSK_GRAD_RAYS) && c->bwd_mode != 0;
    for (int q = 0; q < 3 && deferred; ++q) {
        const int w = STAGE_DEC[stage][q];
        if (w >= 0 && (flags & NSK_GRAD_DECODERS) && c->dec[w].trainable) deferred = false;
    }
    if (handle_dynamic && !fused_median && !deferred) {
        A.mode = 0; A.depth = c->ws.tmp_depth;
        k_composite<<<(N + 3) / 4, 256, 0, c->stream>>>(A);
        CHK(median_thr(c, N, gt, c->ws.tmp_depth));
        A.depth = nullptr;
    }
    A.mode = deferred ? 5 : (fused_median ? 4 : 3); A.gt_depth = gt; A.gt_color = gtc; A.w_color = w_color; A.use_color = use_color;
    A.thr = c->scal + 1; A.handle_dynamic = handle_dynamic; A.detach_var = detach_var; A.loss = c->ws.ray_loss;
    if (deferred) { A.resid = c->ws.tmp_depth; A.g_seed = c->ws.tmp_rgb; }
    else if (fused_median) { c->median_fused_pending = true; A.resid = c->ws.tmp_depth; A.bar = reinterpret_cast<unsigned*>(c->scal + 5); A.thr_out = c->scal + 1; }
    if (flags & NSK_GRAD_RAYS) { A.g_rays_o = g_ro; A.g_rays_d = g_rd; }
    { ProfScope ps(c, "composite"); k_composite<<<(N + 3) / 4, 256, 0, c->stream>>>(A); }
    HIPCHK(hipGetLastError());
    CHK(backward_core(c, stage, N, S, ro, rd, flags, g_ro, g_rd, d_loss, deferred ? c->ws.tmp_depth : nullptr));
    account(c, stage, N * S, N, true, flags);
    return 0;
}

extern "C" int nsk_loss_map(nsk_ctx* c, int N, const float* depth, const float* rgb, const float* gt, const float* gtc, float w_color,
                            int use_color, float* g_depth, float* g_rgb, float* d_loss)
// ... 684 lines not shown
```

nice-slam-cpp_amd/csrc/nsk_bf16.h:

```cpp
#pragma once
#include "nsk_device.h"

template <int CQ, int NP = 3>
struct MlpFwdImgB {
    static constexpr int CB = CQ / 2;
    static constexpr int W0E = 0;
    static constexpr int F0 = W0E + 3;
    static constexpr int W1 = F0 + CB;
    static constexpr int F1 = W1 + 1;
    static constexpr int W2 = F1 + CB;
    static constexpr int F2 = W2 + 1;
    static constexpr int W3E = F2 + CB;
    static constexpr int W3H = W3E + 3;
    static constexpr int F3 = W3H + 1;
    static constexpr int W4 = F3 + CB;
    static constexpr int F4 = W4 + 1;
    static constexpr int NBLK = F4 + CB;
    static constexpr int FRAG_BYTES = NBLK * 2 * NP * 1024;
    static constexpr int P_F32 = FRAG_BYTES / 4;
    static constexpr int P_B = P_F32;
    static constexpr int P_BC = P_B + 160;
    static constexpr int P_WO = P_BC + 160;
    static constexpr int P_BO = P_WO + 128;
    static constexpr int P_BM = P_BO + 4;
// ... 16 lines not shown
        return;
    }
    const __bf16 h = (__bf16)x;
    const float r1 = x - (float)h;
    const __bf16 m = (__bf16)r1;
    const __bf16 l = (__bf16)(r1 - (float)m);
    img[base] = __builtin_bit_cast(unsigned short, h);
    img[base + 64 * 8] = __builtin_bit_cast(unsigned short, m);
    img[base + 128 * 8] = __builtin_bit_cast(unsigned short, l);
}

__global__ void k_pack_bf16(unsigned short* __restrict__ img, const int* __restrict__ idx, const float* __restrict__ P, int n, int np = 3)
{
    int t = blockIdx.x * blockDim.x + threadIdx.x;
    if (t >= n) return;
    const int k = idx[t];
    store_pieces(img, t, k >= 0 ? P[k] : 0.f, np);
}

template <int CQ>
struct FwdSchedB {
    static constexpr int CB = CQ / 2;
    static constexpr int NSTEP = 10 + 5 * CB;
    static constexpr int XE = 0, XC = 3, XH = 3 + CB;
    int blk[NSTEP], xs[NSTEP], bnd[NSTEP], lay[NSTEP];
    constexpr FwdSchedB() : blk{}, xs{}, bnd{}, lay{}
    {
        typedef MlpFwdImgB<CQ> I;
        int s = 0;
        for (int l = 0; l < 5; ++l) {
            if (l == 0 || l == 3) { const int b0 = l == 0 ? I::W0E : I::W3E; for (int b = 0; b < 3; ++b) { blk[s] = b0 + b; xs[s] = XE + b; lay[s] = l; bnd[s] = 0; ++s; } }
            if (l != 0) { blk[s] = l == 3 ? I::W3H : I::W(l); xs[s] = XH; lay[s] = l; bnd[s] = 0; ++s; }
            bnd[s - 1] = 1;
            for (int b = 0; b < CB; ++b) { blk[s] = I::F(l) + b; xs[s] = XC + b; lay[s] = l; bnd[s] = 0; ++s; }
            bnd[s - 1] = 2;
        }
    }
};

template <int CQ, bool DUMP = false>
__device__ __forceinline__ void mlp_forward_bf16(const bf8* __restrict__ img, const float* __restrict__ imgf, int lane, Act<CQ>& A, float* dump = nullptr)
{
    typedef MlpFwdImgB<CQ> I;
    constexpr FwdSchedB<CQ> S{};
    const int g = lane >> 4;
    B3 X[S.XH + 1];
#pragma unroll
    for (int b = 0; b < 3; ++b) X[S.XE + b] = split_block(A.xe[2 * b], A.xe[2 * b + 1]);
#pragma unroll
    for (int b = 0; b < S.CB; ++b) X[S.XC + b] = split_block(A.xc[2 * b], A.xc[2 * b + 1]);
    Frag3 ring[2][2];
    ring[0][0] = load_frag(img, 2 * S.blk[0], lane); ring[0][1] = load_frag(img, 2 * S.blk[0] + 1, lane);
    unsigned long long mask = 0;
    f4 acc[2];
    load_bias(imgf + I::P_B, g, acc);
#pragma unroll
    for (int s = 0; s < S.NSTEP; ++s) {
        if (s + 1 < S.NSTEP) { ring[(s + 1) & 1][0] = load_frag(img, 2 * S.blk[s + 1], lane); ring[(s + 1) & 1][1] = load_frag(img, 2 * S.blk[s + 1] + 1, lane); }
        __builtin_amdgcn_sched_barrier(0);
        mac_block(ring[s & 1][0], ring[s & 1][1], X[S.xs[s]], acc);
        if (S.bnd[s] == 1) {
            if constexpr (DUMP) dump_preact(dump, S.lay[s], g, acc);
            mask |= (unsigned long long)relu_mask(acc) << (8 * S.lay[s]);
            f4 bc[2]; load_bias(imgf + I::P_BC + 32 * S.lay[s], g, bc); acc[0] += bc[0]; acc[1] += bc[1];
        } else if (S.bnd[s] == 2) {
            const int l = S.lay[s];
            A.h[l][0] = acc[0]; A.h[l][1] = acc[1];
            if (l < 4) { X[S.XH] = split_block(acc[0], acc[1]); load_bias(imgf + I::P_B + 32 * (l + 1), g, acc); }
        }
    }
    A.mask = mask;
}

template <int CQ, bool DUMP = false>
__device__ __forceinline__ void mlp_forward_f16(const h8* __restrict__ img, const float* __restrict__ imgf, int lane, Act<CQ>& A, float* dump = nullptr)
{
    typedef MlpFwdImgB<CQ, 2> I;
    constexpr FwdSchedB<CQ> S{};
    const int g = lane >> 4;
    constexpr float INV = 1.f / NSK_H16_SCALE;
    H2 X[S.XH + 1];
#pragma unroll
    for (int b = 0; b < 3; ++b) X[S.XE + b] = split_block_h(A.xe[2 * b], A.xe[2 * b + 1]);
#pragma unroll
    for (int b = 0; b < S.CB; ++b) X[S.XC + b] = split_block_h(A.xc[2 * b], A.xc[2 * b + 1]);
    FragH ring[2][2];
    ring[0][0] = load_frag_h(img, 2 * S.blk[0], lane); ring[0][1] = load_frag_h(img, 2 * S.blk[0] + 1, lane);
    unsigned long long mask = 0;
    f4 acc[2], accL[2] = {(f4)(0.f), (f4)(0.f)};
    load_bias(imgf + I::P_B, g, acc);
#pragma unroll
    for (int s = 0; s < S.NSTEP; ++s) {
        if (s + 1 < S.NSTEP) { ring[(s + 1) & 1][0] = load_frag_h(img, 2 * S.blk[s + 1], lane); ring[(s + 1) & 1][1] = load_frag_h(img, 2 * S.blk[s + 1] + 1, lane); }
        __builtin_amdgcn_sched_barrier(0);
        mac_block_h(ring[s & 1][0], ring[s & 1][1], X[S.xs[s]], acc, accL);
        if (S.bnd[s] != 0) {
            acc[0] += accL[0] * INV; acc[1] += accL[1] * INV;
            accL[0] = (f4)(0.f); accL[1] = (f4)(0.f);
        }
        if (S.bnd[s] == 1) {
            if constexpr (DUMP) dump_preact(dump, S.lay[s], g, acc);
            mask |= (unsigned long long)relu_mask(acc) << (8 * S.lay[s]);
            f4 bc[2]; load_bias(imgf + I::P_BC + 32 * S.lay[s], g, bc); acc[0] += bc[0]; acc[1] += bc[1];
        } else if (S.bnd[s] == 2) {
            const int l = S.lay[s];
            A.h[l][0] = acc[0]; A.h[l][1] = acc[1];
            if (l < 4) { X[S.XH] = split_block_h(acc[0], acc[1]); load_bias(imgf + I::P_B + 32 * (l + 1), g, acc); }
        }
    }
    A.mask = mask;
}

template <int WHICH, int NW = 8, int NP = 3, bool DUMP = false>
__device__ __forceinline__ void decode_fwd_bf16_body(const DecArgs& A, int bid, int nb)
{
    constexpr int CQ = WHICH == 2 ? 4 : 2;
    constexpr int OD = WHICH == 3 ? 4 : 1;
    typedef MlpFwdImgB<CQ, NP> I;
    extern __shared__ __attribute__((aligned(16))) f4 smem[];
    const f4* src = reinterpret_cast<const f4*>(A.img16);
    copy_image_to_lds<64 * NW>(smem, src, I::TOTAL_F / 4);
    __syncthreads();
    const int wave = __builtin_amdgcn_readfirstlane(threadIdx.x >> 6), lane = threadIdx.x & 63, j = lane & 15, g = lane >> 4;
    const bf8* img = reinterpret_cast<const bf8*>(smem);
    const float* imgf = reinterpret_cast<const float*>(smem);
    const int ntasks = (A.M + 15) >> 4;
    const int nw = nb * NW, wg = bid * NW + wave;
    const int tsh = tile_shift(ntasks, nw);
    const int kmax = tiles_per_wave(ntasks, nw, tsh);
    SampleRaw nx;
    int m = slot_sample(A, tile_of(0, wg, nw, tsh) * 16 + j);
    sample_load(A, m, nx);
    int m_next = slot_sample(A, tile_of(1, wg, nw, tsh) * 16 + j);
    for (int k = 0; k < kmax; ++k) {
        const int task = tile_of(k, wg, nw, tsh);
        if (task >= ntasks) break;
        asm volatile("" ::: "memory");
        const int slot = task * 16 + j;
        float px, py, pz;
        sample_finish(A, nx, px, py, pz);
        Tri T;
        tri_setup(A.grid, A.bound, px, py, pz, T);
        Act<CQ> C;
        GatherRaw R;
        tri_gather_issue<true>(A.grid, T, g, R);
        sample_load(A, m_next, nx);
        const int m_cur = m;
        m = m_next;
        m_next = slot_sample(A, tile_of(k + 2, wg, nw, tsh) * 16 + j);
        f4 dummy[6];
        embed<false>(imgf + I::P_BM, g, px, py, pz, C.xe, dummy);
        asm volatile("" ::: "memory");
        tri_gather_reduce(T, R, C.xc[0], C.xc[1]);
        if constexpr (WHICH == 2) {
            Tri Tm;
            tri_setup(A.grid_mid, A.bound, px, py, pz, Tm);
            tri_gather<true>(A.grid_mid, Tm, g, C.xc[CQ - 2], C.xc[CQ - 1]);
        }
        float* dump = nullptr;
        if constexpr (DUMP) dump = slot < A.M ? A.dump + (size_t)m_cur * 160 : nullptr;
        if constexpr (NP == 2) mlp_forward_f16<CQ, DUMP>(reinterpret_cast<const h8*>(smem), imgf, lane, C, dump);
        else mlp_forward_bf16<CQ, DUMP>(img, imgf, lane, C, dump);
        float out[OD];
        mlp_output<OD>(imgf + I::P_WO, imgf + I::P_BO, g, C.h[4], out);
        if (slot < A.M) {
            if (g == 0) {
                if constexpr (OD == 4) *reinterpret_cast<f4*>(A.out + (unsigned)m_cur * 4u) = (f4){out[0], out[1], out[2], out[OD - 1]};
                else A.out[(unsigned)m_cur] = out[0];
            }
            if (A.masks) A.masks[(unsigned)slot * 4u + (unsigned)g] = C.mask;
        }
        if (A.hsave) save_h(A.hsave, task, lane, C.h);
    }
}

template <int NW>
__device__ __forceinline__ void decode_fwd_occ_body(const DecArgs& Am, const DecArgs& Af, int bid, int nb)
{
    typedef MlpFwdImgB<2, 2> IM;
    typedef MlpFwdImgB<4, 2> IF;
    extern __shared__ __attribute__((aligned(16))) f4 smem[];
    copy_image_to_lds<64 * NW>(smem, reinterpret_cast<const f4*>(Am.img16), IM::TOTAL_F / 4);
    copy_image_to_lds<64 * NW>(smem + IM::TOTAL_F / 4, reinterpret_cast<const f4*>(Af.img16), IF::TOTAL_F / 4);
    __syncthreads();
    const int wave = __builtin_amdgcn_readfirstlane(threadIdx.x >> 6), lane = threadIdx.x & 63, j = lane & 15, g = lane >> 4;
    const float* imgf_m = reinterpret_cast<const float*>(smem);
    const float* imgf_f = imgf_m + IM::TOTAL_F;
    const h8* img_m = reinterpret_cast<const h8*>(imgf_m);
    const h8* img_f = reinterpret_cast<const h8*>(imgf_f);
    const int ntasks = (Af.M + 15) >> 4;
    const int nw = nb * NW, wg = bid * NW + wave;
    const int tsh = tile_shift(ntasks, nw);
    const int kmax = tiles_per_wave(ntasks, nw, tsh);
    SampleRaw nx;
    int m = slot_sample(Af, tile_of(0, wg, nw, tsh) * 16 + j);
    sample_load(Af, m, nx);
    int m_next = slot_sample(Af, tile_of(1, wg, nw, tsh) * 16 + j);
    for (int k = 0; k < kmax; ++k) {
        const int task = tile_of(k, wg, nw, tsh);
        if (task >= ntasks) break;
        asm volatile("" ::: "memory");
        const int slot = task * 16 + j;
        float px, py, pz;
        sample_finish(Af, nx, px, py, pz);
        f4 dummy[6];
        f4 xm0, xm1;
        unsigned long long mask_m;
        {
            Tri T;
            tri_setup(Am.grid, Am.bound, px, py, pz, T);
            Act<2> C;
            GatherRaw R;
            tri_gather_issue<true>(Am.grid, T, g, R);
            sample_load(Af, m_next, nx);
            embed<false>(imgf_m + IM::P_BM, g, px, py, pz, C.xe, dummy);
            asm volatile("" ::: "memory");
            tri_gather_reduce(T, R, xm0, xm1);
            C.xc[0] = xm0; C.xc[1] = xm1;
            mlp_forward_f16<2>(img_m, imgf_m, lane, C);
            float out[1];
            mlp_output<1>(imgf_m + IM::P_WO, imgf_m + IM::P_BO, g, C.h[4], out);
            if (slot < Am.M && g == 0) Am.out[(unsigned)m] = out[0];
            mask_m = C.mask;
        }
        const int m_cur = m;
        m = m_next;
        m_next = slot_sample(Af, tile_of(k + 2, wg, nw, tsh) * 16 + j);
        {
            Tri T;
            tri_setup(Af.grid, Af.bound, px, py, pz, T);
            Act<4> C;
            GatherRaw R;
            tri_gather_issue<true>(Af.grid, T, g, R);
            embed<false>(imgf_f + IF::P_BM, g, px, py, pz, C.xe, dummy);
            asm volatile("" ::: "memory");
            tri_gather_reduce(T, R, C.xc[0], C.xc[1]);
            C.xc[2] = xm0; C.xc[3] = xm1;
            mlp_forward_f16<4>(img_f, imgf_f, lane, C);
            float out[1];
            mlp_output<1>(imgf_f + IF::P_WO, imgf_f + IF::P_BO, g, C.h[4], out);
            if (slot < Af.M) {
                if (g == 0) Af.out[(unsigned)m_cur] = out[0];
                if (Af.masks) Af.masks[(unsigned)slot * 4u + (unsigned)g] = C.mask;
                if (Am.masks) Am.masks[(unsigned)slot * 4u + (unsigned)g] = mask_m;
            }
        }
    }
}

template <int NW>
__global__ __launch_bounds__(64 * NW) void k_decode_fwd_multi_occ(MultiArgs MA)
{
    if ((int)blockIdx.x < MA.wg_end[0]) decode_fwd_occ_body<NW>(MA.a[0], MA.a[1], blockIdx.x, MA.wg_end[0]);
    else decode_fwd_bf16_body<3, NW, 2>(MA.a[2], (int)blockIdx.x - MA.wg_end[0], MA.wg_end[1] - MA.wg_end[0]);
}

template <int NW, int NP = 3>
__global__ __launch_bounds__(64 * NW) void k_decode_fwd_multi_bf16(MultiArgs MA)
{
    int r = 0;
    while (r < MA.n - 1 && (int)blockIdx.x >= MA.wg_end[r]) ++r;
    const int b0 = r == 0 ? 0 : MA.wg_end[r - 1];
    const int bid = blockIdx.x - b0, nb = MA.wg_end[r] - b0;
    switch (MA.which[r]) {
    case 0: decode_fwd_body<0, NW>(MA.a[r], bid, nb); break;
    case 1: decode_fwd_bf16_body<1, NW, NP>(MA.a[r], bid, nb); break;
    case 2: decode_fwd_bf16_body<2, NW, NP>(MA.a[r], bid, nb); break;
    default: decode_fwd_bf16_body<3, NW, NP>(MA.a[r], bid, nb); break;
    }
}

template <int MODE>
__global__ __launch_bounds__(512) void k_decode_fwd_dump(DecArgs A, int which)
{
    if constexpr (MODE == 0) {
        switch (which) {
        case 1: decode_fwd_body<1, 8, true>(A, blockIdx.x, gridDim.x); break;
        case 2: decode_fwd_body<2, 8, true>(A, blockIdx.x, gridDim.x); break;
        default: decode_fwd_body<3, 8, true>(A, blockIdx.x, gridDim.x); break;
        }
    } else {
        constexpr int NP = MODE == 2 ? 2 : 3;
        switch (which) {
        case 1: decode_fwd_bf16_body<1, 8, NP, true>(A, blockIdx.x, gridDim.x); break;
        case 2: decode_fwd_bf16_body<2, 8, NP, true>(A, blockIdx.x, gridDim.x); break;
        default: decode_fwd_bf16_body<3, 8, NP, true>(A, blockIdx.x, gridDim.x); break;
        }
    }
}
```

nice-slam-cpp_amd/csrc/nsk_device.h:

```cpp
#pragma once
#include <hip/hip_runtime.h>
#include <stdint.h>
#include "nsk_layout.h"

typedef float f4 __attribute__((ext_vector_type(4)));

struct RParams {
    float bound[6];
    int n_samples, n_surface, lindisp, occupancy;
    float perturb;
    unsigned long long seed;
};

struct GridD {
    const float* v;
    float* g;
    const uint8_t* mask;
    int Z, Y, X;
};

#define NSK_INF __builtin_huge_valf()

__device__ __forceinline__ f4 mfma4(float a, float b, f4 c) { return __builtin_amdgcn_mfma_f32_16x16x4f32(a, b, c, 0, 0, 0); }
__device__ __forceinline__ void lds_fence() { asm volatile("s_waitcnt lgkmcnt(0)" ::: "memory"); }
// ... 529 lines not shown
            a[r][i] = __int_as_float(y);
            unsigned t;
            asm("v_min_u32 %0, %1, 1" : "=v"(t) : "v"(y));
            asm("v_lshl_or_b32 %0, %1, %2, %3" : "=v"(m) : "v"(t), "n"(r * 4 + i), "v"(m));
        }
    return m;
}

__device__ __forceinline__ void dump_preact(float* __restrict__ row, int l, int g, const f4 (&acc)[2])
{
    if (!row) return;
    *reinterpret_cast<f4*>(row + 32 * l + 4 * g) = acc[0];
    *reinterpret_cast<f4*>(row + 32 * l + 16 + 4 * g) = acc[1];
}

template <int CQ>
struct Act {
    f4 xe[6];
    f4 xc[CQ];
    f4 h[5][2];
    unsigned long long mask;
};

__device__ __forceinline__ float nsk_rev(float x)
{
    const float k = rintf(x * 0.15915494309189535f);
    const float f = fmaf(x, 0.159154936671257019f, -k);
    return fmaf(x, 6.42063833e-09f, f);
}
__device__ __forceinline__ float nsk_sin(float x) { return __builtin_amdgcn_sinf(nsk_rev(x)); }
__device__ __forceinline__ void nsk_sincos(float x, float& sn, float& cs)
{
    const float f = nsk_rev(x);
    sn = __builtin_amdgcn_sinf(f);
    cs = __builtin_amdgcn_cosf(f);
}

template <bool WANT_COS>
__device__ __forceinline__ void embed(const float* __restrict__ Bm , int g, float px, float py, float pz,
                                      f4 (&xe)[6], f4 (&xcos)[6])
{
#pragma unroll
    for (int q = 0; q < 6; ++q) {
        f4 b0 = *reinterpret_cast<const f4*>(Bm + 16 * q + 4 * g);
        f4 b1 = *reinterpret_cast<const f4*>(Bm + 96 + 16 * q + 4 * g);
        f4 b2 = *reinterpret_cast<const f4*>(Bm + 192 + 16 * q + 4 * g);
#pragma unroll
        for (int i = 0; i < 4; ++i) {
            int k = 16 * q + 4 * g + i;
            float s = __builtin_fmaf(pz, b2[i], __builtin_fmaf(py, b1[i], mul_rn(px, b0[i])));
            float sv, cv = 0.f;
            if (WANT_COS) nsk_sincos(s, sv, cv); else sv = nsk_sin(s);
            xe[q][i] = k < NSK_E ? sv : 0.f;
            xcos[q][i] = (WANT_COS && k < NSK_E) ? cv : 0.f;
        }
    }
}

template <int CQ, bool DUMP = false>
__device__ __forceinline__ void mlp_forward(const f4* __restrict__ img, int lane, Act<CQ>& A, float* dump = nullptr)
{
    typedef MlpFwdImg<CQ> I;
    const float* imgf = reinterpret_cast<const float*>(img);
    const int g = lane >> 4;
    unsigned long long mask = 0;
    f4 acc[2];
    load_bias(imgf + I::P_B, g, acc);
    gemm<2, 6>(img, I::W0E, lane, A.xe, acc);
    if constexpr (DUMP) dump_preact(dump, 0, g, acc);
    mask |= (unsigned long long)relu_mask(acc);
    { f4 bc[2]; load_bias(imgf + I::P_BC, g, bc); acc[0] += bc[0]; acc[1] += bc[1]; }
    gemm<2, CQ>(img, I::F0, lane, A.xc, acc);
    A.h[0][0] = acc[0]; A.h[0][1] = acc[1];
#pragma unroll
    for (int l = 1; l < 5; ++l) {
        load_bias(imgf + I::P_B + 32 * l, g, acc);
        if (l == 3) {
            gemm<2, 6>(img, I::W3E, lane, A.xe, acc);
            gemm<2, 2>(img, I::W3H, lane, A.h[2], acc);
        } else {
            gemm<2, 2>(img, I::W(l), lane, A.h[l - 1], acc);
        }
        if constexpr (DUMP) dump_preact(dump, l, g, acc);
        mask |= (unsigned long long)relu_mask(acc) << (8 * l);
        { f4 bc[2]; load_bias(imgf + I::P_BC + 32 * l, g, bc); acc[0] += bc[0]; acc[1] += bc[1]; }
        gemm<2, CQ>(img, I::F(l), lane, A.xc, acc);
        A.h[l][0] = acc[0]; A.h[l][1] = acc[1];
    }
    A.mask = mask;
}

template <int OD>
__device__ __forceinline__ void mlp_output(const float* __restrict__ Wo, const float* __restrict__ bo, int g,
                                           const f4 (&h4)[2], float (&out)[OD])
{
#pragma unroll
    for (int o = 0; o < OD; ++o) {
        f4 w0 = *reinterpret_cast<const f4*>(Wo + 32 * o + 4 * g);
        f4 w1 = *reinterpret_cast<const f4*>(Wo + 32 * o + 16 + 4 * g);
        float s = 0.f;
#pragma unroll
        for (int i = 0; i < 4; ++i) s += w0[i] * h4[0][i] + w1[i] * h4[1][i];
        s += __shfl_xor(s, 16);
        s += __shfl_xor(s, 32);
        out[o] = s + bo[o];
    }
}

struct ActC { f4 xc[2]; f4 h[5][2]; unsigned long long mask; };
__device__ __forceinline__ void coarse_forward(const f4* __restrict__ img, int lane, ActC& A)
{
    typedef CoarseFwdImg I;
    const float* imgf = reinterpret_cast<const float*>(img);
    const int g = lane >> 4;
    unsigned long long mask = 0;
    f4 acc[2];
    const int Wq[5] = {I::W0, I::W1, I::W2, I::W3H, I::W4};
#pragma unroll
    for (int l = 0; l < 5; ++l) {
        load_bias(imgf + I::P_B + 32 * l, g, acc);
        if (l == 0) gemm<2, 2>(img, I::W0, lane, A.xc, acc);
        else {
            if (l == 3) gemm<2, 2>(img, I::W3C, lane, A.xc, acc);
            gemm<2, 2>(img, Wq[l], lane, A.h[l - 1], acc);
        }
        mask |= (unsigned long long)relu_mask(acc) << (8 * l);
        A.h[l][0] = acc[0]; A.h[l][1] = acc[1];
    }
    A.mask = mask;
}

struct DecArgs {
    const float* rays_o; const float* rays_d; const float* z; const float* pts;
    const int* perm;
    int M, S;
    unsigned S_magic;
    float bound[6];
    GridD grid, grid_mid;
    const f4* img;
    const void* img16;
    const f4* bimg;
    const void* bimg16;
    int img_f4;
    float* out;
    unsigned long long* masks;
    f4* hsave;
    const float* g_raw;
    float* g_rays_o; float* g_rays_d;
    float* g_dec;
    unsigned flags;
    float* dump;
    const float* dyn_resid;
    int dyn_n;
};

template <typename T>
__device__ __forceinline__ T ld32(const void* base, unsigned byte_off) { return *reinterpret_cast<const T*>(reinterpret_cast<const char*>(base) + byte_off); }
__device__ __forceinline__ int ray_of(const DecArgs& A, int mm) { return A.S_magic ? (int)__umulhi((unsigned)mm, A.S_magic) : mm; }
struct __attribute__((packed, aligned(4))) Ray3 { float x, y, z; };
__device__ __forceinline__ void sample_point(const DecArgs& A, int mm, float& px, float& py, float& pz, float& zz, int& n)
{
    if (A.pts) { px = A.pts[3 * mm]; py = A.pts[3 * mm + 1]; pz = A.pts[3 * mm + 2]; zz = 0.f; n = 0; return; }
    n = ray_of(A, mm);
    zz = A.z[mm];
    const Ray3 o = *reinterpret_cast<const Ray3*>(A.rays_o + 3 * n), d = *reinterpret_cast<const Ray3*>(A.rays_d + 3 * n);
    px = add_rn(o.x, mul_rn(d.x, zz));
    py = add_rn(o.y, mul_rn(d.y, zz));
    pz = add_rn(o.z, mul_rn(d.z, zz));
}

struct SampleRaw { float z, o[3], d[3]; };

__device__ __forceinline__ void sample_load(const DecArgs& A, int mm, SampleRaw& R)
{
    if (A.pts) { R.o[0] = A.pts[3 * mm]; R.o[1] = A.pts[3 * mm + 1]; R.o[2] = A.pts[3 * mm + 2]; R.z = 0.f; R.d[0] = R.d[1] = R.d[2] = 0.f; return; }
    const int n = ray_of(A, mm);
    R.z = ld32<float>(A.z, (unsigned)mm * 4u);
    const Ray3 o = ld32<Ray3>(A.rays_o, (unsigned)n * 12u), d = ld32<Ray3>(A.rays_d, (unsigned)n * 12u);
    R.o[0] = o.x; R.o[1] = o.y; R.o[2] = o.z; R.d[0] = d.x; R.d[1] = d.y; R.d[2] = d.z;
}
__device__ __forceinline__ void sample_finish(const DecArgs& A, const SampleRaw& R, float& px, float& py, float& pz)
{
    if (A.pts) { px = R.o[0]; py = R.o[1]; pz = R.o[2]; return; }
    px = add_rn(R.o[0], mul_rn(R.d[0], R.z));
    py = add_rn(R.o[1], mul_rn(R.d[1], R.z));
    pz = add_rn(R.o[2], mul_rn(R.d[2], R.z));
}

__device__ __forceinline__ int slot_sample(const DecArgs& A, int slot)
{
    const int s = min(slot, A.M - 1);
    return A.perm ? ld32<int>(A.perm, (unsigned)s * 4u) : s;
}

__device__ __forceinline__ int tile_shift(int, int) { return 0; }
__device__ __forceinline__ int tile_of(int k, int wg, int nw, int sh) { return ((((k >> sh) * nw + wg)) << sh) + (k & ((1 << sh) - 1)); }
__device__ __forceinline__ int tiles_per_wave(int ntasks, int nw, int sh) { return ((((ntasks + (1 << sh) - 1) >> sh) + nw - 1) / nw) << sh; }

__device__ __forceinline__ void save_h(f4* __restrict__ hsave, int task, int lane, const f4 (&h)[5][2])
{
    f4* dst = hsave + ((size_t)task * 10) * 64 + lane;
#pragma unroll
    for (int l = 0; l < 5; ++l) { dst[(2 * l) * 64] = h[l][0]; dst[(2 * l + 1) * 64] = h[l][1]; }
}

template <int WHICH, int NW = 8, bool DUMP = false>
__device__ __forceinline__ void decode_fwd_body(const DecArgs& A, int bid, int nb)
{
    extern __shared__ __attribute__((aligned(16))) f4 smem[];
    copy_image_to_lds<64 * NW>(smem, A.img, A.img_f4);
    __syncthreads();
    const int wave = __builtin_amdgcn_readfirstlane(threadIdx.x >> 6), lane = threadIdx.x & 63, j = lane & 15, g = lane >> 4;
    const float* imgf = reinterpret_cast<const float*>(smem);
    const int ntasks = (A.M + 15) >> 4;
    const int tsh = tile_shift(ntasks, nb * NW);
    const int kmax = tiles_per_wave(ntasks, nb * NW, tsh);
    for (int k = 0; k < kmax; ++k) {
        const int task = tile_of(k, bid * NW + wave, nb * NW, tsh);
        if (task >= ntasks) break;
        asm volatile("" ::: "memory");
        const int slot = task * 16 + j;
        const bool valid = slot < A.M;
        const int mm = slot_sample(A, slot);
        const int m = mm;
        float px, py, pz, zz; int n;
        sample_point(A, mm, px, py, pz, zz, n);
        Tri T;
        tri_setup(A.grid, A.bound, px, py, pz, T);
        if constexpr (WHICH == 0) {
            ActC C;
            tri_gather(A.grid, T, g, C.xc[0], C.xc[1]);
            coarse_forward(smem, lane, C);
            float out[1];
            mlp_output<1>(imgf + CoarseFwdImg::P_WO, imgf + CoarseFwdImg::P_BO, g, C.h[4], out);
            if (valid) {
                if (g == 0) A.out[m] = out[0];
                if (A.masks) A.masks[(size_t)slot * 4 + g] = C.mask;
            }
            if (A.hsave) save_h(A.hsave, task, lane, C.h);
        } else {
            constexpr int CQ = WHICH == 2 ? 4 : 2;
            constexpr int OD = WHICH == 3 ? 4 : 1;
            typedef MlpFwdImg<CQ> I;
            Act<CQ> C;
            tri_gather(A.grid, T, g, C.xc[0], C.xc[1]);
            if constexpr (WHICH == 2) {
                Tri Tm;
                tri_setup(A.grid_mid, A.bound, px, py, pz, Tm);
                tri_gather(A.grid_mid, Tm, g, C.xc[CQ - 2], C.xc[CQ - 1]);
            }
            f4 dummy[6];
            embed<false>(imgf + I::P_BM, g, px, py, pz, C.xe, dummy);
            float* dump = nullptr;
            if constexpr (DUMP) dump = valid ? A.dump + (size_t)m * 160 : nullptr;
            mlp_forward<CQ, DUMP>(smem, lane, C, dump);
            float out[OD];
            mlp_output<OD>(imgf + I::P_WO, imgf + I::P_BO, g, C.h[4], out);
            if (valid) {
                if (g == 0) {
                    if constexpr (OD == 4) *reinterpret_cast<f4*>(A.out + (size_t)m * 4) = (f4){out[0], out[1], out[2], out[OD - 1]};
                    else A.out[m] = out[0];
                }
                if (A.masks) A.masks[(size_t)slot * 4 + g] = C.mask;
            }
            if (A.hsave) save_h(A.hsave, task, lane, C.h);
        }
    }
}

template <int WHICH>
__global__ __launch_bounds__(512) void k_decode_fwd(DecArgs A) { decode_fwd_body<WHICH>(A, blockIdx.x, gridDim.x); }

struct MultiArgs {
    DecArgs a[3]; int which[3]; int train[3]; int wg_end[3]; int n;
    const float* sum_src; float* sum_dst; int sum_n;
    ScanArgs scan;
    const float* dyn_seed; float* dyn_thr_out;
};

__device__ __forceinline__ void block_sum(const float* __restrict__ x, int n, float* __restrict__ out)
{
    extern __shared__ __attribute__((aligned(16))) f4 smem[];
    float* sh = reinterpret_cast<float*>(smem);
    float s = 0.f;
    for (int i = threadIdx.x; i < n; i += blockDim.x) s += x[i];
    s = wave_sum(s);
    if ((threadIdx.x & 63) == 0) sh[threadIdx.x >> 6] = s;
    __syncthreads();
    if (threadIdx.x == 0) { for (int w = 1; w < (int)(blockDim.x >> 6); ++w) s += sh[w]; *out = s; }
}

__global__ __launch_bounds__(512) void k_decode_fwd_multi(MultiArgs MA)
{
    int r = 0;
    while (r < MA.n - 1 && (int)blockIdx.x >= MA.wg_end[r]) ++r;
    const int b0 = r == 0 ? 0 : MA.wg_end[r - 1];
    const int bid = blockIdx.x - b0, nb = MA.wg_end[r] - b0;
    switch (MA.which[r]) {
    case 0: decode_fwd_body<0, 8>(MA.a[r], bid, nb); break;
    case 1: decode_fwd_body<1, 8>(MA.a[r], bid, nb); break;
    case 2: decode_fwd_body<2, 8>(MA.a[r], bid, nb); break;
    default: decode_fwd_body<3, 8>(MA.a[r], bid, nb); break;
    }
}

struct CompArgs {
    RParams R;
    int N, S, stage;
    const float* rays_o; const float* rays_d; const float* z;
    const float* occ_a; const float* occ_b;
    const float* rgb4;
    float* rgb; float* depth; float* var; float* weights;
    int mode;
    const float* g_rgb; const float* g_depth; const float* g_var;
    const float* gt_depth; const float* gt_color; float w_color; int use_color;
    const float* thr; int handle_dynamic; int detach_var;
    float* resid; unsigned* bar; float* thr_out;
    float* loss;
    float* g_raw;
    float* g_rays_o; float* g_rays_d;
    float* g_seed;
    const uint8_t* keep;
};

__device__ __forceinline__ float sgnf(float x) { return x > 0.f ? 1.f : (x < 0.f ? -1.f : 0.f); }

#define NSK_MEDIAN_FUSED_MAX 1024
template <int NT, int MAXN>
__device__ __forceinline__ float median_select(const float* __restrict__ rs, int n4, int target)
{
    constexpr int PER = (MAXN + NT - 1) / NT;
    __shared__ int part[2][NT / 64];
    const int lane = threadIdx.x & 63, wave = threadIdx.x >> 6;
    unsigned u[PER];
#pragma unroll
    for (int e = 0; e < PER; ++e) { const int i = threadIdx.x + e * NT; u[e] = i < n4 ? __float_as_uint(rs[i]) : 0xffffffffu; }
    unsigned ans = 0u;
    for (int bit = 30; bit >= 0; --bit) {
        const unsigned cand = ans | (1u << bit);
        int cnt = 0;
#pragma unroll
        for (int e = 0; e < PER; ++e) cnt += u[e] < cand ? 1 : 0;
        cnt = (int)wave_sum((float)cnt);
        if (lane == 0) part[bit & 1][wave] = cnt;
        __syncthreads();
        int tot = 0;
#pragma unroll
        for (int w = 0; w < NT / 64; ++w) tot += part[bit & 1][w];
        if (tot <= target) ans = cand;
    }
    return __uint_as_float(ans);
}

template <int NT, int MAXN>
__device__ __forceinline__ float lower_median_x10(const float* __restrict__ rs, int n4, int* __restrict__ part)
{
    constexpr int NWV = NT / 64;
    const int lane = threadIdx.x & 63, wave = threadIdx.x >> 6;
    if (n4 <= 256) {
        unsigned u[4];
#pragma unroll
        for (int e = 0; e < 4; ++e) { const int i = lane + 64 * e; u[e] = i < n4 ? __float_as_uint(rs[i]) : 0xffffffffu; }
        auto below = [&](unsigned cand) {
            int c = 0;
#pragma unroll
            for (int e = 0; e < 4; ++e) c += __popcll(__builtin_amdgcn_ballot_w64(u[e] < cand));
            return c;
        };
        const int target = (max(below(0x7f800000u), 1) - 1) / 2;
        unsigned ans = 0u;
        for (int bit = 30; bit >= 0; --bit) {
            const unsigned cand = ans | (1u << bit);
            if (below(cand) <= target) ans = cand;
        }
        return 10.f * __uint_as_float(ans);
    }
    constexpr int PER = (MAXN + NT - 1) / NT;
    unsigned u[PER];
#pragma unroll
    for (int e = 0; e < PER; ++e) { const int i = threadIdx.x + e * NT; u[e] = i < n4 ? __float_as_uint(rs[i]) : 0xffffffffu; }
    auto below = [&](unsigned cand, int buf) {
        int cnt = 0;
#pragma unroll
        for (int e = 0; e < PER; ++e) cnt += __popcll(__builtin_amdgcn_ballot_w64(u[e] < cand));
        if (lane == 0) part[buf * NWV + wave] = cnt;
        __syncthreads();
        int tot = 0;
#pragma unroll
        for (int w = 0; w < NWV; ++w) tot += part[buf * NWV + w];
        return tot;
    };
    const int valid = below(0x7f800000u, 2);
    const int target = (max(valid, 1) - 1) / 2;
    unsigned ans = 0u;
    for (int bit = 30; bit >= 0; --bit) {
        const unsigned cand = ans | (1u << bit);
        if (below(cand, bit & 1) <= target) ans = cand;
    }
// ... 533 lines not shown
```

nice-slam-cpp_amd/csrc/nsk_train.h:

```cpp
#pragma once
#include "nsk_device.h"
#include <type_traits>
#include <utility>

#define PN_RB 272
#define PN_GROWS 32
#define PN_EROWS(CQ) (PN_GROWS + 16 * (CQ))
#define PN_ROWS(CQ) (PN_EROWS(CQ) + 96)
#define PN_MOFF(CQ) (PN_ROWS(CQ) * PN_RB)
#define PN_FLOATS(CQ) (2 * PN_MOFF(CQ) / 4)

struct TrainPhase {
    int RT, NC, rowsum;
    int slot0, nslots;
    int w_base, ld, col0;
    int rows, cols_total;
    int b_base;
};

template <int WHICH>
struct TrainPlan {
    static constexpr bool XYZ = WHICH != 0;
    static constexpr int CQ = WHICH == 2 ? 4 : 2;
    static constexpr int OD = WHICH == 3 ? 4 : 1;
// ... 48 lines not shown
    int s0 = blockIdx.y * per, s1 = min(nslabs, s0 + per);
    float acc = 0.f;
    for (int s = s0; s < s1; ++s) acc += slabs[(size_t)s * n4 + i];
    if (acc != 0.f) atomicAdd(g + i, acc);
}

typedef unsigned int u4v __attribute__((ext_vector_type(4)));
__device__ __forceinline__ void split2_pair(float x0, float x1, unsigned& h01, unsigned& m01)
{
    typedef __bf16 bf2 __attribute__((ext_vector_type(2)));
    typedef float f2 __attribute__((ext_vector_type(2)));
    h01 = __builtin_bit_cast(unsigned, __builtin_convertvector((f2){x0, x1}, bf2));
    const float r0 = x0 - __uint_as_float(h01 << 16), r1 = x1 - __uint_as_float(h01 & 0xffff0000u);
    m01 = __builtin_bit_cast(unsigned, __builtin_convertvector((f2){r0, r1}, bf2));
}

__device__ __forceinline__ void pair_words(unsigned v01, unsigned v23, bool odd, unsigned selA, unsigned selB, unsigned& wA, unsigned& wB)
{
    const unsigned keep = odd ? v23 : v01, send = odd ? v01 : v23;
    const unsigned recv = (unsigned)__builtin_amdgcn_mov_dpp((int)send, 0xB1, 0xF, 0xF, true);
    wA = __builtin_amdgcn_perm(keep, recv, selA);
    wB = __builtin_amdgcn_perm(keep, recv, selB);
}
struct PairSel { bool odd; unsigned selA, selB; int rowoff, col2; };
__device__ __forceinline__ PairSel pair_sel(int wave, int lane)
{
    PairSel P;
    P.odd = (lane & 1) != 0;
    P.selA = P.odd ? 0x05040100u : 0x01000504u; P.selB = P.odd ? 0x07060302u : 0x03020706u;
    P.rowoff = 4 * (lane >> 4) + (P.odd ? 2 : 0);
    P.col2 = (16 * wave + (lane & 14)) * 2;
    return P;
}
__device__ __forceinline__ void pn_put(char* __restrict__ pn, int moff, int row0, int wave, int lane, f4 x, float us = 1.f)
{
    x *= us;
    const PairSel P = pair_sel(wave, lane);
    char* ph = pn + (row0 + P.rowoff) * PN_RB + P.col2;
    unsigned h01, m01, h23, m23, a, b;
    split2_pair(x[0], x[1], h01, m01);
    split2_pair(x[2], x[3], h23, m23);
    pair_words(h01, h23, P.odd, P.selA, P.selB, a, b);
    *reinterpret_cast<unsigned*>(ph) = a; *reinterpret_cast<unsigned*>(ph + PN_RB) = b;
    pair_words(m01, m23, P.odd, P.selA, P.selB, a, b);
    *reinterpret_cast<unsigned*>(ph + moff) = a; *reinterpret_cast<unsigned*>(ph + moff + PN_RB) = b;
}

struct Mask4 { unsigned d[4]; };
__device__ __forceinline__ Mask4 relu_mask_dwords(unsigned long long mask, int l)
{
    const unsigned w = l < 4 ? (unsigned)mask : (unsigned)(mask >> 32);
    const int sh = l < 4 ? 8 * l : 0;
    Mask4 M;
#pragma unroll
    for (int d = 0; d < 4; ++d) {
        const unsigned lo = (unsigned)__builtin_amdgcn_sbfe((int)w, sh + 2 * d, 1), hi = (unsigned)__builtin_amdgcn_sbfe((int)w, sh + 2 * d + 1, 1);
        M.d[d] = (lo & 0xffffu) | (hi & 0xffff0000u);
    }
    return M;
}
__device__ __forceinline__ H2 mask_block_h4(const H2& x, const Mask4& M)
{
    u4v h = __builtin_bit_cast(u4v, x.h), l = __builtin_bit_cast(u4v, x.l);
#pragma unroll
    for (int d = 0; d < 4; ++d) { h[d] &= M.d[d]; l[d] &= M.d[d]; }
    H2 r;
    r.h = __builtin_bit_cast(h8, h); r.l = __builtin_bit_cast(h8, l);
    return r;
}
__device__ __forceinline__ void pn_put_masked(char* __restrict__ pn, int moff, int row1, int row2, int wave, int lane, f4 x, float us, unsigned k01, unsigned k23)
{
    x *= us;
    const PairSel P = pair_sel(wave, lane);
    char* p1 = pn + (row1 + P.rowoff) * PN_RB + P.col2;
    char* p2 = p1 + (row2 - row1) * PN_RB;
    unsigned h01, m01, h23, m23, a, b;
    split2_pair(x[0], x[1], h01, m01);
    split2_pair(x[2], x[3], h23, m23);
    pair_words(h01, h23, P.odd, P.selA, P.selB, a, b);
    *reinterpret_cast<unsigned*>(p1) = a; *reinterpret_cast<unsigned*>(p1 + PN_RB) = b;
    pair_words(m01, m23, P.odd, P.selA, P.selB, a, b);
    *reinterpret_cast<unsigned*>(p1 + moff) = a; *reinterpret_cast<unsigned*>(p1 + moff + PN_RB) = b;
    pair_words(h01 & k01, h23 & k23, P.odd, P.selA, P.selB, a, b);
    *reinterpret_cast<unsigned*>(p2) = a; *reinterpret_cast<unsigned*>(p2 + PN_RB) = b;
    pair_words(m01 & k01, m23 & k23, P.odd, P.selA, P.selB, a, b);
    *reinterpret_cast<unsigned*>(p2 + moff) = a; *reinterpret_cast<unsigned*>(p2 + moff + PN_RB) = b;
}

template <int NSL>
__device__ __forceinline__ void pn_tiles(const char* __restrict__ pn, int moff, int RT, int NC, int rowsum, int wave, int lane, f4* acc, int xrow0 = PN_GROWS,
                                         int grow0 = 0)
{
    const int r = lane & 15, sq = lane >> 4;
    const int ntiles = RT * NC + (rowsum ? RT : 0);
#pragma unroll
    for (int k = 0; k < NSL; ++k) {
        const int tile = 8 * k + wave;
        if (tile < ntiles) {
            const bool rs = tile >= RT * NC;
            const int rt = rs ? tile - RT * NC : tile / NC;
            const int ch = rs ? 0 : tile % NC;
            const char* ga = pn + (grow0 + 16 * rt + r) * PN_RB + 16 * sq;
            const char* xb = pn + (xrow0 + 16 * ch + r) * PN_RB + 16 * sq;
            f4 d0 = acc[k], d1 = (f4)(0.f);
#pragma unroll
            for (int b = 0; b < 4; ++b) {
                const bf8 ah = *reinterpret_cast<const bf8*>(ga + 64 * b);
                const bf8 am = *reinterpret_cast<const bf8*>(ga + moff + 64 * b);
                if (rs) {
                    const bf8 one = __builtin_bit_cast(bf8, (u4v)(0x3f803f80u));
                    d0 = mfma_b(ah, one, d0);
                    d1 = mfma_b(am, one, d1);
                } else {
                    const bf8 xh = *reinterpret_cast<const bf8*>(xb + 64 * b);
                    const bf8 xm = *reinterpret_cast<const bf8*>(xb + moff + 64 * b);
                    d0 = mfma_b(ah, xh, d0);
                    d1 = mfma_b(am, xm, d1);
                    d0 = mfma_b(ah, xm, d0);
                    d1 = mfma_b(am, xh, d1);
                }
            }
            acc[k] = d0 + d1;
        }
    }
}

template <int NSL>
__device__ __forceinline__ void pn_flush(float* __restrict__ g_dec, const TrainPhase P, int wave, int lane, const f4* acc)
{
    const int x = lane & 15, g = lane >> 4;
    const int ntiles = P.RT * P.NC + (P.rowsum ? P.RT : 0);
#pragma unroll
    for (int k = 0; k < NSL; ++k) {
        const int tile = 8 * k + wave;
        if (tile < ntiles) {
            const bool rs = tile >= P.RT * P.NC;
            const int rt = rs ? tile - P.RT * P.NC : tile / P.NC;
            const int ch = rs ? 0 : tile % P.NC;
#pragma unroll
            for (int i = 0; i < 4; ++i) {
                const int o = 16 * rt + 4 * g + i;
                const float v = acc[k][i];
                if (o < P.rows) {
                    if (rs) { if (x == 0) g_dec[P.b_base + o] = v; }
                    else if (16 * ch + x < P.cols_total) g_dec[P.w_base + o * P.ld + P.col0 + 16 * ch + x] = v;
                }
            }
        }
    }
}

__device__ __forceinline__ void lds_barrier() { asm volatile("s_waitcnt lgkmcnt(0)\n\ts_barrier" ::: "memory"); }

template <int WHICH, bool RAYS, bool FULL = false>
__device__ __forceinline__ void decode_bwd_train_body(const DecArgs& A, int bid, int nb)
{
    constexpr bool XYZ = WHICH != 0;
    constexpr int CQ = WHICH == 2 ? 4 : 2;
    constexpr int OD = WHICH == 3 ? 4 : 1;
    constexpr bool SAVED = WHICH != 2;
    constexpr bool H16 = XYZ && SAVED && !FULL;
    typedef MlpFwdImg<CQ> FI;
    typedef TrainPlan<WHICH> PL;
    constexpr PL plan{};
    constexpr int BWD_F = XYZ ? MlpBwdImg::TOTAL : CoarseBwdImg::TOTAL;
    constexpr int IMG_F = SAVED ? BWD_F : 0;
    extern __shared__ __attribute__((aligned(16))) f4 smem[];
    const int wave = __builtin_amdgcn_readfirstlane(threadIdx.x >> 6), lane0 = threadIdx.x & 63;
    int lane = lane0, j = lane & 15, g = lane >> 4;
    float* smf = reinterpret_cast<float*>(smem);
    char* pn = reinterpret_cast<char*>(smf + IMG_F);
    constexpr int PM = PN_MOFF(CQ);
    float* scratch = smf + IMG_F + wave * 1056;
    static_assert(!H16 || MlpBwdImgH::TOTAL_F == BWD_F, "the fp16 backward image takes the fp32 image's place in LDS");
    copy_image_to_lds<512>(smem, H16 ? reinterpret_cast<const f4*>(A.bimg16) : A.bimg, IMG_F / 4);
    __syncthreads();
    const h8* imgh = reinterpret_cast<const h8*>(smem);
    const f4* fimg = A.img;
    const float* fimgf = reinterpret_cast<const float*>(fimg);
    const f4* bimg = SAVED ? smem : A.bimg;
    const float* bimgf = reinterpret_cast<const float*>(bimg);
    const float* Bm = nullptr;
    if constexpr (XYZ) Bm = SAVED ? bimgf + MlpBwdImg::P_BM : fimgf + FI::P_BM;
    static_assert(MlpBwdImgH::P_BM == MlpBwdImg::P_BM && MlpBwdImgH::P_WO == MlpBwdImg::P_WO, "same fp32 tail in both images");
    const float* Bmb = Bm;
    const float* Wo = SAVED ? bimgf + (XYZ ? MlpBwdImg::P_WO : CoarseBwdImg::P_WO) : fimgf + FI::P_WO;

    f4 acc[plan.nslots];
#pragma unroll
    for (int k = 0; k < plan.nslots; ++k) acc[k] = (f4)(0.f);

    const int ntasks = (A.M + 15) >> 4;
    const int iters = tiles_per_wave(ntasks, nb * 8, 0);
    const bool scat = (A.flags & 1u) && A.grid.g;
    struct Staged { float px, py, pz, zz; int n; bool valid; f4 gr; f4 xc[CQ]; f4 h4[2]; unsigned long long mask; } nx;
    auto task_of = [&](int it_) { return tile_of(it_, bid * 8 + wave, nb * 8, 0); };
    auto slot_of = [&](int it_) { return task_of(it_) * 16 + j; };
    auto stage_a = [&](int it_, int mm, Staged& S_) {
        const int task = task_of(it_);
        const int slot = task * 16 + j;
        S_.valid = slot < A.M;
        sample_point(A, mm, S_.px, S_.py, S_.pz, S_.zz, S_.n);
        S_.gr = *reinterpret_cast<const f4*>(A.g_raw + (size_t)mm * 4);
        if constexpr (SAVED) {
            const int tk = min(task, ntasks - 1);
            S_.mask = A.masks[(size_t)min(slot, A.M - 1) * 4 + g];
            S_.h4[0] = A.hsave[((size_t)tk * 10 + 8) * 64 + lane]; S_.h4[1] = A.hsave[((size_t)tk * 10 + 9) * 64 + lane];
        }
    };
    auto stage_b = [&](Staged& S_) {
        Tri T_;
        tri_setup(A.grid, A.bound, S_.px, S_.py, S_.pz, T_);
        tri_gather(A.grid, T_, g, S_.xc[0], S_.xc[1]);
        if constexpr (WHICH == 2) {
            Tri Tm;
            tri_setup(A.grid_mid, A.bound, S_.px, S_.py, S_.pz, Tm);
            tri_gather(A.grid_mid, Tm, g, S_.xc[CQ - 2], S_.xc[CQ - 1]);
        }
    };
    int mm_next = 0;
    if (iters > 0) { stage_a(0, slot_sample(A, slot_of(0)), nx); stage_b(nx); mm_next = slot_sample(A, slot_of(1)); }
    if constexpr (SAVED) asm volatile("" : "+v"(nx.h4[0]), "+v"(nx.h4[1]), "+v"(nx.gr), "+v"(nx.mask), "+v"(mm_next));
    for (int it = 0; it < iters; ++it) {
        asm volatile("" ::: "memory");
        lane = lane0; asm volatile("" : "+v"(lane)); j = lane & 15; g = lane >> 4;
        if (it > 0) lds_barrier();
        const bool valid = nx.valid;
        float px = nx.px, py = nx.py, pz = nx.pz, zz = nx.zz; const int n = nx.n;
        Tri T;
        float gout[OD];
        {
            f4 gr = nx.gr;
            if (!valid) gr = (f4)(0.f);
            if constexpr (OD == 4) { gout[0] = gr[0]; gout[1] = gr[1]; gout[2] = gr[2]; gout[3] = 0.f; }
            else gout[0] = gr[3];
        }
        f4 go;
#pragma unroll
        for (int i = 0; i < 4; ++i) go[i] = (4 * g + i) < OD ? gout[(4 * g + i) < OD ? (4 * g + i) : 0] : 0.f;
        float us = 1.f;
        if constexpr (H16) us = chain_scale<OD>(gout);
        Act<CQ> C;
        ActC CC;
        f4 xcos[6];
        unsigned long long mask;
        const int htask = min(task_of(it), ntasks - 1);
        if constexpr (XYZ) {
#pragma unroll
            for (int q = 0; q < CQ; ++q) C.xc[q] = nx.xc[q];
            embed<false>(Bm, g, px, py, pz, C.xe, xcos);
#pragma unroll
            for (int q = 0; q < 6; ++q) pn_put(pn, PM, PN_EROWS(CQ) + 16 * q, wave, lane, C.xe[q]);
            if constexpr (SAVED) { C.h[4][0] = nx.h4[0]; C.h[4][1] = nx.h4[1]; mask = nx.mask; }
            else { mlp_forward<CQ>(fimg, lane, C); mask = C.mask; }
        } else {
            CC.xc[0] = nx.xc[0]; CC.xc[1] = nx.xc[1];
            CC.h[4][0] = nx.h4[0]; CC.h[4][1] = nx.h4[1]; mask = nx.mask;
        }
        f4 gh[2];
#pragma unroll
        for (int r = 0; r < 2; ++r)
#pragma unroll
            for (int i = 0; i < 4; ++i) {
                float s = 0.f;
#pragma unroll
                for (int o = 0; o < OD; ++o) s += Wo[32 * o + 16 * r + 4 * g + i] * gout[o];
                gh[r][i] = s;
            }
        {
            pn_put(pn, PM, 0, wave, lane, go);
            const f4* h4 = XYZ ? C.h[4] : CC.h[4];
            pn_put(pn, PM, PN_GROWS, wave, lane, h4[0]);
            pn_put(pn, PM, PN_GROWS + 16, wave, lane, h4[1]);
            lds_barrier();
            constexpr TrainPhase P = plan.p[PL::P_OUT];
            pn_tiles<P.nslots>(pn, PM, P.RT, P.NC, P.rowsum, wave, lane, acc + P.slot0);
            lds_barrier();
        }
        f4 gc[2] = {(f4)(0.f), (f4)(0.f)};
        f4 ge[6];
#pragma unroll
        for (int q = 0; q < 6; ++q) ge[q] = (f4)(0.f);
        H2 xa3;
        auto load_h = [&](auto KC) {
            constexpr int k = decltype(KC)::value;
            const f4* src = A.hsave + ((size_t)htask * 10 + 2 * k) * 64 + lane;
            if constexpr (XYZ) { C.h[k][0] = src[0]; C.h[k][1] = src[64]; }
            else { CC.h[k][0] = src[0]; CC.h[k][1] = src[64]; }
        };
        if constexpr (SAVED) load_h(std::integral_constant<int, 3>{});
        auto layer = [&](auto LC) {
            constexpr int l = decltype(LC)::value;
            if constexpr (SAVED && l >= 2) load_h(std::integral_constant<int, l - 2>{});
            if constexpr (XYZ) {
                if constexpr (H16) {
                    const H2 xg = split_block_h(gh[0], gh[1]);
                    f4 gl[2] = {(f4)(0.f), (f4)(0.f)};
                    gemm_h(imgh, MlpBwdImgH::FT(l), lane, xg, gc, gl);
                    gc[0] += gl[0] * (1.f / NSK_H16_SCALE); gc[1] += gl[1] * (1.f / NSK_H16_SCALE);
                } else gemm<2, 2>(bimg, MlpBwdImg::FT(l), lane, gh, gc);
                pn_put(pn, PM, 0, wave, lane, gh[0], us);
                pn_put(pn, PM, 16, wave, lane, gh[1], us);
#pragma unroll
                for (int q = 0; q < CQ; ++q) pn_put(pn, PM, PN_GROWS + 16 * q, wave, lane, C.xc[q]);
                lds_barrier();
                constexpr TrainPhase P = plan.p[PL::P_FC0 + l];
                pn_tiles<P.nslots>(pn, PM, P.RT, P.NC, P.rowsum, wave, lane, acc + P.slot0);
                lds_barrier();
            }
            f4 ga[2];
#pragma unroll
            for (int r = 0; r < 2; ++r)
#pragma unroll
                for (int i = 0; i < 4; ++i) ga[r][i] = ((mask >> (8 * l + 4 * r + i)) & 1ull) ? gh[r][i] : 0.f;
            H2 xa;
            if constexpr (H16) xa = split_block_h(ga[0], ga[1]);
            {
                pn_put(pn, PM, 0, wave, lane, ga[0], us);
                pn_put(pn, PM, 16, wave, lane, ga[1], us);
                if constexpr (XYZ) {
                    if constexpr (l == 0) {
                    } else if constexpr (l == 3) {
                        pn_put(pn, PM, PN_GROWS, wave, lane, C.h[2][0]);
                        pn_put(pn, PM, PN_GROWS + 16, wave, lane, C.h[2][1]);
                    } else {
                        pn_put(pn, PM, PN_GROWS, wave, lane, C.h[l - 1][0]);
                        pn_put(pn, PM, PN_GROWS + 16, wave, lane, C.h[l - 1][1]);
                    }
                } else {
                    if constexpr (l == 0 || l == 3) { pn_put(pn, PM, PN_GROWS, wave, lane, CC.xc[0]); pn_put(pn, PM, PN_GROWS + 16, wave, lane, CC.xc[1]); }
                    else { pn_put(pn, PM, PN_GROWS, wave, lane, CC.h[l - 1][0]); pn_put(pn, PM, PN_GROWS + 16, wave, lane, CC.h[l - 1][1]); }
                }
                lds_barrier();
                constexpr TrainPhase P = plan.p[PL::P_W0 + l];
                constexpr int xrow0 = (XYZ && (l == 0 || l == 3)) ? PN_EROWS(CQ) : PN_GROWS;
                pn_tiles<P.nslots>(pn, PM, P.RT, P.NC, P.rowsum, wave, lane, acc + P.slot0, xrow0);
                if constexpr (XYZ && l == 3) {
                    constexpr TrainPhase P2 = plan.p[PL::P_W3H];
                    pn_tiles<P2.nslots>(pn, PM, P2.RT, P2.NC, P2.rowsum, (wave + 4) & 7, lane, acc + P2.slot0);
                }
                lds_barrier();
                if constexpr (!XYZ && l == 3) {
                    const f4* h2 = CC.h[2];
                    pn_put(pn, PM, PN_GROWS, wave, lane, h2[0]);
                    pn_put(pn, PM, PN_GROWS + 16, wave, lane, h2[1]);
                    lds_barrier();
                    constexpr TrainPhase P2 = plan.p[PL::P_W3H];
                    pn_tiles<P2.nslots>(pn, PM, P2.RT, P2.NC, P2.rowsum, wave, lane, acc + P2.slot0);
                    lds_barrier();
                }
            }
            if constexpr (H16) {
                if constexpr (l == 3) xa3 = xa;
                if constexpr (l == 0) { gemm_e_h(imgh, MlpBwdImgH::W3ET, lane, xa3, ge); gemm_e_h(imgh, MlpBwdImgH::W0ET, lane, xa, ge); }
                if constexpr (l >= 1) {
                    f4 ghn[2] = {(f4)(0.f), (f4)(0.f)}, ghl[2] = {(f4)(0.f), (f4)(0.f)};
                    gemm_h(imgh, MlpBwdImgH::WT(l), lane, xa, ghn, ghl);
                    gh[0] = ghn[0] + ghl[0] * (1.f / NSK_H16_SCALE); gh[1] = ghn[1] + ghl[1] * (1.f / NSK_H16_SCALE);
                }
            } else if constexpr (XYZ) {
                if constexpr (l == 3) gemm_e(bimg, MlpBwdImg::W3ET, lane, ga, ge);
                if constexpr (l == 0) gemm_e(bimg, MlpBwdImg::W0ET, lane, ga, ge);
                if constexpr (l >= 1) {
                    f4 ghn[2] = {(f4)(0.f), (f4)(0.f)};
                    gemm<2, 2>(bimg, MlpBwdImg::WT(l), lane, ga, ghn);
                    gh[0] = ghn[0]; gh[1] = ghn[1];
                }
            } else {
                if constexpr (l == 3) gemm<2, 2>(bimg, CoarseBwdImg::W3CT, lane, ga, gc);
                if constexpr (l == 0) gemm<2, 2>(bimg, CoarseBwdImg::W0T, lane, ga, gc);
                else {
                    constexpr int q0 = l == 1 ? CoarseBwdImg::W1T : (l == 2 ? CoarseBwdImg::W2T : (l == 3 ? CoarseBwdImg::W3HT : CoarseBwdImg::W4T));
                    f4 ghn[2] = {(f4)(0.f), (f4)(0.f)};
                    gemm<2, 2>(bimg, q0, lane, ga, ghn);
                    gh[0] = ghn[0]; gh[1] = ghn[1];
                }
            }
        };
        layer(std::integral_constant<int, 4>{});
        layer(std::integral_constant<int, 3>{});
        layer(std::integral_constant<int, 2>{});
        layer(std::integral_constant<int, 1>{});
        layer(std::integral_constant<int, 0>{});
        if (it + 1 < iters) { stage_a(it + 1, mm_next, nx); mm_next = slot_sample(A, slot_of(it + 2)); }
        if constexpr (H16) {
            gc[0] *= us; gc[1] *= us;
        }
        float gp[3] = {0.f, 0.f, 0.f};
        asm volatile("" : "+v"(px), "+v"(py), "+v"(pz));
        tri_setup(A.grid, A.bound, px, py, pz, T);
        if constexpr (XYZ) {
            { f4 e2[6]; embed<true>(Bmb, g, px, py, pz, e2, xcos); }
#pragma unroll
            for (int q = 0; q < 6; ++q) ge[q] *= xcos[q];
            {
                f4 pq;
#pragma unroll
                for (int i = 0; i < 4; ++i) { int row = 4 * g + i; pq[i] = !valid ? 0.f : (row == 0 ? px : (row == 1 ? py : (row == 2 ? pz : 0.f))); }
                pn_put(pn, PM, 0, wave, lane, pq, us);
#pragma unroll
                for (int q = 0; q < 6; ++q) pn_put(pn, PM, PN_EROWS(CQ) + 16 * q, wave, lane, ge[q]);
                lds_barrier();
                constexpr TrainPhase P = plan.p[PL::P_DB];
                pn_tiles<P.nslots>(pn, PM, P.RT, P.NC, P.rowsum, wave, lane, acc + P.slot0, PN_EROWS(CQ));
                lds_barrier();
            }
            if constexpr (RAYS) {
#pragma unroll
                for (int q = 0; q < 6; ++q) {
                    f4 b0 = *reinterpret_cast<const f4*>(Bmb + 16 * q + 4 * g);
                    f4 b1 = *reinterpret_cast<const f4*>(Bmb + 96 + 16 * q + 4 * g);
                    f4 b2 = *reinterpret_cast<const f4*>(Bmb + 192 + 16 * q + 4 * g);
#pragma unroll
                    for (int i = 0; i < 4; ++i) { gp[0] += ge[q][i] * b0[i]; gp[1] += ge[q][i] * b1[i]; gp[2] += ge[q][i] * b2[i]; }
                }
                if constexpr (H16) { gp[0] *= us; gp[1] *= us; gp[2] *= us; }
            }
        }
        if constexpr (RAYS) {
            tri_grad_p(A.grid, T, g, gc, gp);
#pragma unroll
            for (int k = 0; k < 3; ++k) { gp[k] += __shfl_xor(gp[k], 16); gp[k] += __shfl_xor(gp[k], 32); }
            if (A.g_rays_o) {
                const int n0 = __builtin_amdgcn_readfirstlane(n);
                if (__builtin_amdgcn_ballot_w64(valid && n != n0) == 0ull) {
                    float a[6];
#pragma unroll
                    for (int k = 0; k < 3; ++k) { a[k] = valid ? gp[k] : 0.f; a[3 + k] = valid ? gp[k] * zz : 0.f; }
#pragma unroll
                    for (int o = 1; o < 16; o <<= 1)
#pragma unroll
                        for (int k = 0; k < 6; ++k) a[k] += __shfl_xor(a[k], o);
                    if (lane == 0) {
#pragma unroll
                        for (int k = 0; k < 3; ++k) { atomicAdd(A.g_rays_o + 3 * n0 + k, a[k]); atomicAdd(A.g_rays_d + 3 * n0 + k, a[3 + k]); }
                    }
                } else if (g == 0 && valid) {
#pragma unroll
                    for (int k = 0; k < 3; ++k) {
                        atomicAdd(A.g_rays_o + 3 * n + k, gp[k]);
                        atomicAdd(A.g_rays_d + 3 * n + k, gp[k] * zz);
                    }
                }
            }
        }
        if (it + 1 < iters) {
            stage_b(nx);
        }
        if constexpr (SAVED) asm volatile("" : "+v"(nx.h4[0]), "+v"(nx.h4[1]), "+v"(nx.gr), "+v"(nx.mask), "+v"(mm_next));
        if (scat) {
            if (A.flags & 0x8000u) {
                for (int w = 0; w < 8; ++w) { if (wave == w) { scatter_tile(A.grid, T, gc, lane, valid, scratch); asm volatile("s_waitcnt vmcnt(0)" ::: "memory"); } __syncthreads(); }
            } else scatter_tile(A.grid, T, gc, lane, valid, scratch);
        }
    }
    float* slab = A.g_dec + (size_t)bid * ((plan_total<WHICH>() + 3) & ~3);
    pn_flush<plan.p[PL::P_OUT].nslots>(slab, plan.p[PL::P_OUT], wave, lane, acc + plan.p[PL::P_OUT].slot0);
#define NSK_FLUSH(ID) if constexpr (plan.p[ID].nslots > 0) pn_flush<plan.p[ID].nslots>(slab, plan.p[ID], wave, lane, acc + plan.p[ID].slot0);
    NSK_FLUSH(1) NSK_FLUSH(2) NSK_FLUSH(3) NSK_FLUSH(4) NSK_FLUSH(5) NSK_FLUSH(6) NSK_FLUSH(7) NSK_FLUSH(8) NSK_FLUSH(9)
    NSK_FLUSH(10) NSK_FLUSH(12)
    if constexpr (plan.p[PL::P_W3H].nslots > 0)
        pn_flush<plan.p[PL::P_W3H].nslots>(slab, plan.p[PL::P_W3H], XYZ ? (wave + 4) & 7 : wave, lane, acc + plan.p[PL::P_W3H].slot0);
#undef NSK_FLUSH
}


#define PM_G1 0
#define PM_G2 32
#define PM_XC 64
#define PM_XH 96
#define PM_E 128
#define PM_ROWS 224
#define PM_IMG_FRAG_F (18 * 2 * 1024 / 4)
#define PM_IMG_F (PM_IMG_FRAG_F + 128 + 288)
#define PM_LDS_BYTES (PM_IMG_F * 4 + PM_ROWS * PN_RB * 2)

__device__ __forceinline__ void gemm_e2_lds(const h8* __restrict__ eimg, int lane, const H2& x3, const H2& x0, f4 (&acc)[6])
{
    constexpr int G3 = MlpBwdImgH::W3ET - MlpBwdImgH::W0ET;
#pragma unroll
    for (int a = 0; a < 3; ++a) {
        const FragH a30 = load_frag_h(eimg, G3 + 2 * a, lane), a31 = load_frag_h(eimg, G3 + 2 * a + 1, lane);
        const FragH a00 = load_frag_h(eimg, 2 * a, lane), a01 = load_frag_h(eimg, 2 * a + 1, lane);
        f4 tH[2] = {acc[2 * a], acc[2 * a + 1]}, tL[2] = {(f4)(0.f), (f4)(0.f)};
        mac_block_h(a30, a31, x3, tH, tL);
        mac_block_h(a00, a01, x0, tH, tL);
        acc[2 * a] = tH[0] + tL[0] * (1.f / NSK_H16_SCALE); acc[2 * a + 1] = tH[1] + tL[1] * (1.f / NSK_H16_SCALE);
    }
}
__device__ __forceinline__ void gemm_e2T_lds(const h8* __restrict__ eimg, int lane, const H2& x3, const H2& x0, f4 (&acc)[6])
{
    constexpr int G3 = MlpBwdImgH::W3ET - MlpBwdImgH::W0ET;
#pragma unroll
    for (int q = 0; q < 6; ++q) {
        const FragH f3 = load_frag_h(eimg, G3 + q, lane), f0 = load_frag_h(eimg, q, lane);
        f4 tH = (f4)(0.f), tL = (f4)(0.f);
        tH = mfma_h(x3.h, f3.h, tH); tL = mfma_h(x3.h, f3.l, tL); tL = mfma_h(x3.l, f3.h, tL);
        tH = mfma_h(x0.h, f0.h, tH); tL = mfma_h(x0.h, f0.l, tL); tL = mfma_h(x0.l, f0.h, tL);
        acc[q] = tH + tL * (1.f / NSK_H16_SCALE);
    }
}
typedef short s4v __attribute__((ext_vector_type(4)));
__device__ __forceinline__ f4 mfma_bf16_k16(unsigned a01, unsigned a23, unsigned b01, unsigned b23, f4 c)
{
    typedef unsigned int u2v __attribute__((ext_vector_type(2)));
    return __builtin_amdgcn_mfma_f32_16x16x16bf16_1k(__builtin_bit_cast(s4v, (u2v){a01, a23}), __builtin_bit_cast(s4v, (u2v){b01, b23}), c, 0, 0, 0);
}
struct FragE { FragH a30, a31, a00, a01; };
__device__ __forceinline__ FragE load_frag_e(const h8* __restrict__ gimg, int a, int lane)
{
    FragE F;
    F.a30 = load_frag_h(gimg, MlpBwdImgH::W3ET + 2 * a, lane); F.a31 = load_frag_h(gimg, MlpBwdImgH::W3ET + 2 * a + 1, lane);
    F.a00 = load_frag_h(gimg, MlpBwdImgH::W0ET + 2 * a, lane); F.a01 = load_frag_h(gimg, MlpBwdImgH::W0ET + 2 * a + 1, lane);
    return F;
}
__device__ __forceinline__ void gemm_e2_global(const h8* __restrict__ gimg, int lane, const H2& x3, const H2& x0, f4 (&acc)[6])
{
    FragE F[3];
    F[0] = load_frag_e(gimg, 0, lane);
#pragma unroll
    for (int a = 0; a < 3; ++a) {
        if (a + 1 < 3) F[a + 1] = load_frag_e(gimg, a + 1, lane);
        f4 tH[2] = {acc[2 * a], acc[2 * a + 1]}, tL[2] = {(f4)(0.f), (f4)(0.f)};
        mac_block_h(F[a].a30, F[a].a31, x3, tH, tL);
        mac_block_h(F[a].a00, F[a].a01, x0, tH, tL);
        acc[2 * a] = tH[0] + tL[0] * (1.f / NSK_H16_SCALE); acc[2 * a + 1] = tH[1] + tL[1] * (1.f / NSK_H16_SCALE);
    }
}

struct TJob { int wave, grow, nt; int xrow[4]; int ph[4]; int rt; int ch[4]; };
template <int WHICH>
struct JobPlan {
    typedef TrainPlan<WHICH> PL;
    static constexpr int NJ = 32;
    static constexpr int PH_OUT = 0, PH_DB = 6;
    TJob j[NJ];
    int slot0[NJ];
    int first[8];
    int nslots;
    constexpr JobPlan() : j{}, slot0{}, first{}, nslots(0)
    {
        int n = 0;
        auto add = [&](int wave, int grow, int rt, int nt, int x0, int p0, int c0, int x1, int p1, int c1, int x2 = 0, int p2 = 0, int c2 = 0, int x3 = 0, int p3 = 0, int c3 = 0) {
            j[n] = TJob{wave, grow, nt, {x0, x1, x2, x3}, {p0, p1, p2, p3}, rt, {c0, c1, c2, c3}};
            ++n;
        };
        const int RS = -1;
        first[0] = n;
        add(0, PM_G1, 0, 3, PM_XH, PL::P_OUT, 0, PM_XH + 16, PL::P_OUT, 1, 0, PL::P_OUT, RS);
        for (int l = 4; l >= 0; --l) {
            first[1 + (4 - l)] = n;
            const int FC = PL::P_FC0 + l, W = PL::P_W0 + l;
            if (l == 4 || l == 2 || l == 1) {
                const int w0 = l == 4 ? 0 : 4;
                add(w0 + 0, PM_G1, 0, 3, PM_XC, FC, 0, PM_XC + 16, FC, 1, 0, FC, RS);
                add(w0 + 1, PM_G1 + 16, 1, 3, PM_XC, FC, 0, PM_XC + 16, FC, 1, 0, FC, RS);
                add(w0 + 2, PM_G2, 0, 3, PM_XH, W, 0, PM_XH + 16, W, 1, 0, W, RS);
                add(w0 + 3, PM_G2 + 16, 1, 3, PM_XH, W, 0, PM_XH + 16, W, 1, 0, W, RS);
            } else if (l == 3) {
                add(0, PM_G2, 0, 3, PM_E, W, 0, PM_E + 16, W, 1, 0, W, RS);
                add(4, PM_G1, 0, 3, PM_XC, FC, 0, PM_XC + 16, FC, 1, 0, FC, RS);
                add(1, PM_G2 + 16, 1, 3, PM_E, W, 0, PM_E + 16, W, 1, 0, W, RS);
                add(5, PM_G1 + 16, 1, 3, PM_XC, FC, 0, PM_XC + 16, FC, 1, 0, FC, RS);
                add(2, PM_G2, 0, 4, PM_E + 32, W, 2, PM_E + 48, W, 3, PM_XH, PL::P_W3H, 0, PM_XH + 16, PL::P_W3H, 1);
                add(6, PM_G2, 0, 2, PM_E + 64, W, 4, PM_E + 80, W, 5);
                add(3, PM_G2 + 16, 1, 4, PM_E + 32, W, 2, PM_E + 48, W, 3, PM_XH, PL::P_W3H, 0, PM_XH + 16, PL::P_W3H, 1);
                add(7, PM_G2 + 16, 1, 2, PM_E + 64, W, 4, PM_E + 80, W, 5);
            } else {
                add(0, PM_G2, 0, 3, PM_E, W, 0, PM_E + 16, W, 1, 0, W, RS);
                add(4, PM_G2, 0, 2, PM_E + 32, W, 2, PM_E + 48, W, 3);
                add(1, PM_G2 + 16, 1, 3, PM_E, W, 0, PM_E + 16, W, 1, 0, W, RS);
                add(5, PM_G2 + 16, 1, 2, PM_E + 32, W, 2, PM_E + 48, W, 3);
                add(2, PM_G1, 0, 3, PM_XC, FC, 0, PM_XC + 16, FC, 1, 0, FC, RS);
                add(6, PM_G2, 0, 2, PM_E + 64, W, 4, PM_E + 80, W, 5);
                add(3, PM_G1 + 16, 1, 3, PM_XC, FC, 0, PM_XC + 16, FC, 1, 0, FC, RS);
                add(7, PM_G2 + 16, 1, 2, PM_E + 64, W, 4, PM_E + 80, W, 5);
            }
        }
        first[6] = n;
        add(6, PM_G1, 0, 2, PM_E, PL::P_DB, 0, PM_E + 16, PL::P_DB, 1);
        add(7, PM_G1, 0, 2, PM_E + 32, PL::P_DB, 2, PM_E + 48, PL::P_DB, 3);
        add(1, PM_G1, 0, 2, PM_E + 64, PL::P_DB, 4, PM_E + 80, PL::P_DB, 5);
        first[7] = n;
        int used[8] = {0, 0, 0, 0, 0, 0, 0, 0};
        for (int q = 0; q < n; ++q) { slot0[q] = used[j[q].wave]; used[j[q].wave] += j[q].nt; }
        for (int w = 0; w < 8; ++w) nslots = used[w] > nslots ? used[w] : nslots;
    }
};

template <int WHICH>
constexpr bool jobplan_covers_plan()
{
    constexpr JobPlan<WHICH> JP{};
    constexpr TrainPlan<WHICH> plan{};
    for (int ph = 0; ph < TrainPlan<WHICH>::NPH; ++ph) {
        const TrainPhase P = plan.p[ph];
        for (int rt = 0; rt < P.RT; ++rt)
            for (int ch = -1; ch < P.NC; ++ch) {
                if (ch < 0 && !P.rowsum) continue;
                int owners = 0;
                for (int q = 0; q < JobPlan<WHICH>::NJ; ++q)
                    for (int k = 0; k < JP.j[q].nt; ++k)
                        if (JP.j[q].ph[k] == ph && JP.j[q].rt == rt && (ch < 0 ? JP.j[q].ch[k] < 0 : JP.j[q].ch[k] == ch)) ++owners;
                if (owners != 1) return false;
            }
    }
    int tiles = 0, want = 0;
    for (int q = 0; q < JobPlan<WHICH>::NJ; ++q) tiles += JP.j[q].nt;
    for (int ph = 0; ph < TrainPlan<WHICH>::NPH; ++ph) want += plan.p[ph].RT * plan.p[ph].NC + (plan.p[ph].rowsum ? plan.p[ph].RT : 0);
    return tiles == want && JP.nslots <= 12;
}
static_assert(jobplan_covers_plan<1>() && jobplan_covers_plan<3>(), "JobPlan: a weight-gradient tile is unowned, owned twice, or a wave holds more than 12 tiles");

template <int WHICH, int JJ>
__device__ __forceinline__ void pn_job(const char* __restrict__ pn, int moff, int wave, int lane, f4* acc)
{
    constexpr JobPlan<WHICH> JP{};
    constexpr TJob J = JP.j[JJ];
    constexpr int s0 = JP.slot0[JJ];
    if (wave != J.wave) return;
    const int r = lane & 15, sq = lane >> 4;
    const char* ga = pn + (J.grow + r) * PN_RB + 16 * sq;
    f4 d0[J.nt], d1[J.nt];
#pragma unroll
    for (int k = 0; k < J.nt; ++k) { d0[k] = acc[s0 + k]; d1[k] = (f4)(0.f); }
#pragma unroll
    for (int b = 0; b < 4; ++b) {
        const bf8 ah = *reinterpret_cast<const bf8*>(ga + 64 * b);
        const bf8 am = *reinterpret_cast<const bf8*>(ga + moff + 64 * b);
#pragma unroll
        for (int k = 0; k < J.nt; ++k) {
            if (J.ch[k] < 0) {
                const bf8 one = __builtin_bit_cast(bf8, (u4v)(0x3f803f80u));
                d0[k] = mfma_b(ah, one, d0[k]);
                d1[k] = mfma_b(am, one, d1[k]);
            } else {
                const char* xb = pn + (J.xrow[k] + r) * PN_RB + 16 * sq;
                const bf8 xh = *reinterpret_cast<const bf8*>(xb + 64 * b);
                const bf8 xm = *reinterpret_cast<const bf8*>(xb + moff + 64 * b);
                d0[k] = mfma_b(ah, xh, d0[k]);
                d1[k] = mfma_b(am, xm, d1[k]);
                d0[k] = mfma_b(ah, xm, d0[k]);
                d1[k] = mfma_b(am, xh, d1[k]);
            }
        }
    }
#pragma unroll
    for (int k = 0; k < J.nt; ++k) acc[s0 + k] = d0[k] + d1[k];
}
template <int WHICH, int J0, int... Is>
__device__ __forceinline__ void pn_jobs_seq(const char* __restrict__ pn, int moff, int wave, int lane, f4* acc, std::integer_sequence<int, Is...>)
{
    (pn_job<WHICH, J0 + Is>(pn, moff, wave, lane, acc), ...);
}
template <int WHICH, int PH>
__device__ __forceinline__ void pn_phase_jobs(const char* __restrict__ pn, int moff, int wave, int lane, f4* acc)
{
    constexpr JobPlan<WHICH> JP{};
    pn_jobs_seq<WHICH, JP.first[PH]>(pn, moff, wave, lane, acc, std::make_integer_sequence<int, JP.first[PH + 1] - JP.first[PH]>{});
}
template <int WHICH, int JJ, bool SKIP_DB = false>
__device__ __forceinline__ void pn_job_flush(float* __restrict__ g_dec, int wave, int lane, const f4* acc)
{
    constexpr JobPlan<WHICH> JP{};
    constexpr TrainPlan<WHICH> plan{};
    constexpr TJob J = JP.j[JJ];
    constexpr int s0 = JP.slot0[JJ];
    if (wave != J.wave) return;
    const int x = lane & 15, g = lane >> 4;
#pragma unroll
    for (int k = 0; k < J.nt; ++k) {
        constexpr int dummy = 0; (void)dummy;
        const TrainPhase P = plan.p[J.ph[k]];
        if (SKIP_DB && J.ph[k] == TrainPlan<WHICH>::P_DB) continue;
        const bool rs = J.ch[k] < 0;
#pragma unroll
        for (int i = 0; i < 4; ++i) {
            const int o = 16 * J.rt + 4 * g + i;
            const float v = acc[s0 + k][i];
            if (o < P.rows) {
                if (rs) { if (x == 0) g_dec[P.b_base + o] = v; }
                else if (16 * J.ch[k] + x < P.cols_total) g_dec[P.w_base + o * P.ld + P.col0 + 16 * J.ch[k] + x] = v;
            }
        }
    }
}
template <int WHICH, bool SKIP_DB, int... Is>
__device__ __forceinline__ void pn_jobs_flush_all(float* __restrict__ g_dec, int wave, int lane, const f4* acc, std::integer_sequence<int, Is...>)
{
    (pn_job_flush<WHICH, Is, SKIP_DB>(g_dec, wave, lane, acc), ...);
}

template <int WHICH, bool RAYS>
__device__ __forceinline__ void decode_bwd_train_m_body(const DecArgs& A, int bid, int nb)
{
    static_assert(WHICH == 1 || WHICH == 3, "merged-phase body: middle and colour decoders");
    constexpr int CQ = 2;
    constexpr int OD = WHICH == 3 ? 4 : 1;
    typedef TrainPlan<WHICH> PL;
    constexpr PL plan{};
    extern __shared__ __attribute__((aligned(16))) f4 smem[];
    const int wave = __builtin_amdgcn_readfirstlane(threadIdx.x >> 6), lane0 = threadIdx.x & 63;
    int lane = lane0, j = lane & 15, g = lane >> 4;
    float* smf = reinterpret_cast<float*>(smem);
    char* pn = reinterpret_cast<char*>(smf + PM_IMG_F);
    constexpr int PM = PM_ROWS * PN_RB;
    float* scratch = smf + PM_IMG_F + wave * 1056;
    static_assert(8 * 1056 * 4 <= PM_E * PN_RB, "scatter scratch must end before the E rows");
    const h8* imgh = reinterpret_cast<const h8*>(smem);
    const f4* gimg_e = reinterpret_cast<const f4*>(A.bimg16) + (size_t)MlpBwdImgH::W0ET * 2 * 1024 / 16;
    constexpr int EIMG_F4 = 12 * 2 * 1024 / 16;
    static_assert(EIMG_F4 == 3 * 512 && EIMG_F4 * 16 <= (PM_E - PM_G2) * PN_RB, "e-part image: three float4 per thread, inside plane H of rows 32..127");
    f4* eimg = reinterpret_cast<f4*>(pn + PM_G2 * PN_RB);
    const h8* eimgh = reinterpret_cast<const h8*>(eimg);
    const float* Wo = smf + PM_IMG_FRAG_F;
    const float* Bm = Wo + 128;

    constexpr JobPlan<WHICH> JP{};
    f4 acc[JP.nslots];
#pragma unroll
    for (int k = 0; k < JP.nslots; ++k) acc[k] = (f4)(0.f);

    const int ntasks = (A.M + 15) >> 4;
    const int iters = tiles_per_wave(ntasks, nb * 8, 0);
    const bool scat = (A.flags & 1u) && A.grid.g;
    struct Staged { SampleRaw r; float px, py, pz; int mm; bool valid; f4 gr; f4 xc[CQ]; f4 h4[2]; unsigned long long mask; } nx;
    auto task_of = [&](int it_) { return tile_of(it_, bid * 8 + wave, nb * 8, 0); };
    auto slot_of = [&](int it_) { return task_of(it_) * 16 + j; };
    auto stage_a = [&](int it_, int mm, Staged& S_) {
        const int task = task_of(it_);
        const int slot = task * 16 + j;
        S_.valid = slot < A.M;
        S_.mm = mm;
        sample_load(A, mm, S_.r);
        S_.gr = ld32<f4>(A.g_raw, (unsigned)mm * 16u);
        const int tk = min(task, ntasks - 1);
        S_.mask = ld32<unsigned long long>(A.masks, ((unsigned)min(slot, A.M - 1) * 4u + (unsigned)g) * 8u);
        S_.h4[0] = A.hsave[((size_t)tk * 10 + 8) * 64 + lane]; S_.h4[1] = A.hsave[((size_t)tk * 10 + 9) * 64 + lane];
    };
    Tri Tn; GatherRaw GR;
    auto stage_b1 = [&](Staged& S_) {
        sample_finish(A, S_.r, S_.px, S_.py, S_.pz);
        tri_setup(A.grid, A.bound, S_.px, S_.py, S_.pz, Tn);
        tri_gather_issue<true>(A.grid, Tn, g, GR);
    };
    auto stage_b2 = [&](Staged& S_) { tri_gather_reduce(Tn, GR, S_.xc[0], S_.xc[1]); };
    int mm_next = 0;
    {
        const f4* src = reinterpret_cast<const f4*>(A.bimg16);
        constexpr int K0 = (PM_IMG_FRAG_F / 4 + 511) / 512;
        ImgRegs<K0> ir0; ImgRegs<1> ir1;
        const int mm0 = slot_sample(A, slot_of(0));
        image_issue<512>(ir0, src, PM_IMG_FRAG_F / 4);
        image_issue<512>(ir1, src + MlpBwdImgH::P_WO / 4, (128 + 288) / 4);
        if (iters > 0) stage_a(0, mm0, nx);
        image_commit<512>(smem, ir0, src, PM_IMG_FRAG_F / 4);
        image_commit<512>(smem + PM_IMG_FRAG_F / 4, ir1, src + MlpBwdImgH::P_WO / 4, (128 + 288) / 4);
        __syncthreads();
        if (iters > 0) { stage_b1(nx); stage_b2(nx); mm_next = slot_sample(A, slot_of(1)); }
    }
    asm volatile("" : "+v"(nx.h4[0]), "+v"(nx.h4[1]), "+v"(nx.gr), "+v"(nx.mask), "+v"(mm_next));
    f4 accB[2] = {(f4)(0.f), (f4)(0.f)};
    (void)accB;
    for (int it = 0; it < iters; ++it) {
        asm volatile("" ::: "memory");
        lane = lane0; asm volatile("" : "+v"(lane)); j = lane & 15; g = lane >> 4;
        if (it > 0) lds_barrier();
        const bool valid = nx.valid;
        float px = nx.px, py = nx.py, pz = nx.pz, zz = A.pts ? 0.f : nx.r.z; const int n = A.pts ? 0 : ray_of(A, nx.mm);
        (void)zz; (void)n;
        float gout[OD];
        {
            f4 gr = nx.gr;
            if (!valid) gr = (f4)(0.f);
            if constexpr (OD == 4) { gout[0] = gr[0]; gout[1] = gr[1]; gout[2] = gr[2]; gout[3] = 0.f; }
            else gout[0] = gr[3];
        }
        f4 go;
#pragma unroll
        for (int i = 0; i < 4; ++i) go[i] = (4 * g + i) < OD ? gout[(4 * g + i) < OD ? (4 * g + i) : 0] : 0.f;
        const float us = chain_scale<OD>(gout);
        const unsigned long long mask = nx.mask;
        const int htask = min(task_of(it), ntasks - 1);
        f4 hq[5][2];
        hq[4][0] = nx.h4[0]; hq[4][1] = nx.h4[1];
        auto load_h = [&](auto KC) {
            constexpr int k = decltype(KC)::value;
            const f4* src = A.hsave + ((size_t)htask * 10 + 2 * k) * 64 + lane;
            hq[k][0] = src[0]; hq[k][1] = src[64];
        };
        load_h(std::integral_constant<int, 3>{});
        {
            f4 xe[6], dummy[6];
            embed<false>(Bm, g, px, py, pz, xe, dummy);
#pragma unroll
            for (int q = 0; q < 6; ++q) pn_put(pn, PM, PM_E + 16 * q, wave, lane, xe[q]);
        }
        pn_put(pn, PM, PM_XC, wave, lane, nx.xc[0]);
        pn_put(pn, PM, PM_XC + 16, wave, lane, nx.xc[1]);
        f4 gh[2];
#pragma unroll
        for (int r = 0; r < 2; ++r)
#pragma unroll
            for (int i = 0; i < 4; ++i) {
                float s = 0.f;
#pragma unroll
                for (int o = 0; o < OD; ++o) s += Wo[32 * o + 16 * r + 4 * g + i] * gout[o];
                gh[r][i] = s;
            }
        {
            pn_put(pn, PM, PM_G1, wave, lane, go);
            pn_put(pn, PM, PM_XH, wave, lane, hq[4][0]);
            pn_put(pn, PM, PM_XH + 16, wave, lane, hq[4][1]);
            lds_barrier();
            pn_phase_jobs<WHICH, JobPlan<WHICH>::PH_OUT>(pn, PM, wave, lane, acc);
            lds_barrier();
        }
        f4 gc[2] = {(f4)(0.f), (f4)(0.f)};
        H2 xa3, xa;
        auto layer = [&](auto LC) {
            constexpr int l = decltype(LC)::value;
            if constexpr (l >= 2) load_h(std::integral_constant<int, l - 2>{});
            const Mask4 RM = relu_mask_dwords(mask, l);
            {
                const H2 xg = split_block_h(gh[0], gh[1]);
                f4 gl[2] = {(f4)(0.f), (f4)(0.f)};
                gemm_h(imgh, MlpBwdImgH::FT(l), lane, xg, gc, gl);
                gc[0] += gl[0] * (1.f / NSK_H16_SCALE); gc[1] += gl[1] * (1.f / NSK_H16_SCALE);
                xa = mask_block_h4(xg, RM);
            }
            pn_put_masked(pn, PM, PM_G1, PM_G2, wave, lane, gh[0], us, RM.d[0], RM.d[1]);
            pn_put_masked(pn, PM, PM_G1 + 16, PM_G2 + 16, wave, lane, gh[1], us, RM.d[2], RM.d[3]);
            if constexpr (l >= 1) {
                constexpr int k = l == 3 ? 2 : l - 1;
                pn_put(pn, PM, PM_XH, wave, lane, hq[k][0]);
                pn_put(pn, PM, PM_XH + 16, wave, lane, hq[k][1]);
            }
            lds_barrier();
            pn_phase_jobs<WHICH, 1 + (4 - l)>(pn, PM, wave, lane, acc);
            lds_barrier();
            if constexpr (l == 3) xa3 = xa;
            if constexpr (l >= 1) {
                f4 ghn[2] = {(f4)(0.f), (f4)(0.f)}, ghl[2] = {(f4)(0.f), (f4)(0.f)};
                gemm_h(imgh, MlpBwdImgH::WT(l), lane, xa, ghn, ghl);
                gh[0] = ghn[0] + ghl[0] * (1.f / NSK_H16_SCALE); gh[1] = ghn[1] + ghl[1] * (1.f / NSK_H16_SCALE);
            }
        };
        layer(std::integral_constant<int, 4>{});
        layer(std::integral_constant<int, 3>{});
        layer(std::integral_constant<int, 2>{});
        layer(std::integral_constant<int, 1>{});
        f4 ecp[3];
#pragma unroll
        for (int u = 0; u < 3; ++u) ecp[u] = gimg_e[u * 512 + (int)threadIdx.x];
        layer(std::integral_constant<int, 0>{});
#pragma unroll
        for (int u = 0; u < 3; ++u) eimg[u * 512 + (int)threadIdx.x] = ecp[u];
        lds_barrier();
        gc[0] *= us; gc[1] *= us;
        float gp[3] = {0.f, 0.f, 0.f};
        Tri T;
        f4 ge[6];
        if constexpr (!RAYS) {
            if (it + 1 < iters) { stage_a(it + 1, mm_next, nx); mm_next = slot_sample(A, slot_of(it + 2)); }
            gemm_e2T_lds(eimgh, lane, xa3, xa, ge);
            stage_b1(nx);
            float* xch = reinterpret_cast<float*>(pn + PM + PM_G1 * PN_RB) + wave * 64;
            if (g == 0) *reinterpret_cast<f4*>(xch + 4 * j) = (f4){px, py, pz, valid ? us : 0.f};
            asm volatile("s_waitcnt lgkmcnt(0)" ::: "memory");
            const int nb3 = j / 3, nc = j - 3 * nb3;
            unsigned ph01, pm01, ph23, pm23;
            f4 sp[4];
#pragma unroll
            for (int i = 0; i < 4; ++i) sp[i] = *reinterpret_cast<const f4*>(xch + 4 * (4 * g + i));
            {
                float pv[4];
#pragma unroll
                for (int i = 0; i < 4; ++i) pv[i] = (nc == 0 ? sp[i][0] : (nc == 1 ? sp[i][1] : sp[i][2])) * sp[i][3];
                split2_pair(pv[0], pv[1], ph01, pm01); split2_pair(pv[2], pv[3], ph23, pm23);
            }
#pragma unroll
            for (int q = 0; q < 6; ++q) {
                const int f = 16 * q + j;
                const float b0 = Bm[f], b1 = Bm[96 + f], b2 = Bm[192 + f];
                float gs[4];
#pragma unroll
                for (int i = 0; i < 4; ++i) {
                    const float s = add_rn(add_rn(mul_rn(sp[i][0], b0), mul_rn(sp[i][1], b1)), mul_rn(sp[i][2], b2));
                    const float cv = __builtin_amdgcn_cosf(nsk_rev(s));
                    gs[i] = f < NSK_E ? ge[q][i] * cv : 0.f;
                }
                unsigned ah01, am01, ah23, am23;
                split2_pair(gs[0], gs[1], ah01, am01); split2_pair(gs[2], gs[3], ah23, am23);
                const bool on = nb3 == (q % 5);
                const unsigned bh01 = on ? ph01 : 0u, bh23 = on ? ph23 : 0u, bm01 = on ? pm01 : 0u, bm23 = on ? pm23 : 0u;
                f4& d = accB[q / 5];
                d = mfma_bf16_k16(ah01, ah23, bh01, bh23, d);
                d = mfma_bf16_k16(ah01, ah23, bm01, bm23, d);
                d = mfma_bf16_k16(am01, am23, bh01, bh23, d);
                d = mfma_bf16_k16(am01, am23, bm01, bm23, d);
            }
            tri_setup(A.grid, A.bound, px, py, pz, T);
        } else {
#pragma unroll
            for (int q = 0; q < 6; ++q) ge[q] = (f4)(0.f);
            gemm_e2_lds(eimgh, lane, xa3, xa, ge);
            if (it + 1 < iters) { stage_a(it + 1, mm_next, nx); mm_next = slot_sample(A, slot_of(it + 2)); }
            tri_setup(A.grid, A.bound, px, py, pz, T);
            {
                f4 e2[6], xcos[6];
                embed<true>(Bm, g, px, py, pz, e2, xcos);
#pragma unroll
                for (int q = 0; q < 6; ++q) ge[q] *= xcos[q];
            }
            {
                f4 pq;
#pragma unroll
                for (int i = 0; i < 4; ++i) { int row = 4 * g + i; pq[i] = !valid ? 0.f : (row == 0 ? px : (row == 1 ? py : (row == 2 ? pz : 0.f))); }
                pn_put(pn, PM, PM_G1, wave, lane, pq, us);
#pragma unroll
                for (int q = 0; q < 6; ++q) pn_put(pn, PM, PM_E + 16 * q, wave, lane, ge[q]);
                stage_b1(nx);
                lds_barrier();
                pn_phase_jobs<WHICH, JobPlan<WHICH>::PH_DB>(pn, PM, wave, lane, acc);
                lds_barrier();
            }
        }
        if constexpr (RAYS) {
#pragma unroll
            for (int q = 0; q < 6; ++q) {
                f4 b0 = *reinterpret_cast<const f4*>(Bm + 16 * q + 4 * g);
                f4 b1 = *reinterpret_cast<const f4*>(Bm + 96 + 16 * q + 4 * g);
                f4 b2 = *reinterpret_cast<const f4*>(Bm + 192 + 16 * q + 4 * g);
#pragma unroll
                for (int i = 0; i < 4; ++i) { gp[0] += ge[q][i] * b0[i]; gp[1] += ge[q][i] * b1[i]; gp[2] += ge[q][i] * b2[i]; }
            }
            gp[0] *= us; gp[1] *= us; gp[2] *= us;
            tri_grad_p(A.grid, T, g, gc, gp);
#pragma unroll
            for (int k = 0; k < 3; ++k) { gp[k] += __shfl_xor(gp[k], 16); gp[k] += __shfl_xor(gp[k], 32); }
            if (A.g_rays_o) {
                const int n0 = __builtin_amdgcn_readfirstlane(n);
                if (__builtin_amdgcn_ballot_w64(valid && n != n0) == 0ull) {
                    float a[6];
#pragma unroll
                    for (int k = 0; k < 3; ++k) { a[k] = valid ? gp[k] : 0.f; a[3 + k] = valid ? gp[k] * zz : 0.f; }
#pragma unroll
                    for (int o = 1; o < 16; o <<= 1)
#pragma unroll
                        for (int k = 0; k < 6; ++k) a[k] += __shfl_xor(a[k], o);
                    if (lane == 0) {
#pragma unroll
                        for (int k = 0; k < 3; ++k) { atomicAdd(A.g_rays_o + 3 * n0 + k, a[k]); atomicAdd(A.g_rays_d + 3 * n0 + k, a[3 + k]); }
                    }
                } else if (g == 0 && valid) {
#pragma unroll
                    for (int k = 0; k < 3; ++k) {
                        atomicAdd(A.g_rays_o + 3 * n + k, gp[k]);
                        atomicAdd(A.g_rays_d + 3 * n + k, gp[k] * zz);
                    }
                }
            }
        }
        stage_b2(nx);
        asm volatile("" : "+v"(nx.h4[0]), "+v"(nx.h4[1]), "+v"(nx.gr), "+v"(nx.mask), "+v"(mm_next), "+v"(nx.xc[0]), "+v"(nx.xc[1]));
        if (scat) {
            if (A.flags & 0x8000u) {
                for (int w = 0; w < 8; ++w) { if (wave == w) { scatter_tile(A.grid, T, gc, lane, valid, scratch); asm volatile("s_waitcnt vmcnt(0)" ::: "memory"); } __syncthreads(); }
            } else scatter_tile(A.grid, T, gc, lane, valid, scratch);
        }
    }
    float* slab = A.g_dec + (size_t)bid * ((plan_total<WHICH>() + 3) & ~3);
    pn_jobs_flush_all<WHICH, !RAYS>(slab, wave, lane, acc, std::make_integer_sequence<int, JobPlan<WHICH>::NJ>{});
    if constexpr (!RAYS) {
        __syncthreads();
        f4* red = reinterpret_cast<f4*>(pn);
        red[(wave * 2 + 0) * 64 + lane] = accB[0]; red[(wave * 2 + 1) * 64 + lane] = accB[1];
        __syncthreads();
        if (threadIdx.x < 128) {
            const int a = threadIdx.x >> 6;
            f4 v = red[a * 64 + lane];
#pragma unroll
            for (int w = 1; w < 8; ++w) v += red[(w * 2 + a) * 64 + lane];
            constexpr TrainPhase P = plan.p[PL::P_DB];
            const int q = a == 0 ? j / 3 : 5, k = j - 3 * (j / 3);
            if (a == 0 ? j < 15 : j < 3) {
#pragma unroll
                for (int i = 0; i < 4; ++i) {
                    const int f = 16 * q + 4 * g + i;
                    if (f < NSK_E) slab[P.w_base + k * P.ld + f] = v[i];
                }
            }
        }
    }
}

template <int WHICH, bool RAYS>
__device__ __forceinline__ void decode_bwd_train_any(const DecArgs& A, int bid, int nb)
{
    if constexpr (WHICH == 1 || WHICH == 3) decode_bwd_train_m_body<WHICH, RAYS>(A, bid, nb);
    else decode_bwd_train_body<WHICH, RAYS>(A, bid, nb);
}

template <int WHICH, bool RAYS>
__global__ __launch_bounds__(512) void k_decode_bwd_train(DecArgs A) { decode_bwd_train_any<WHICH, RAYS>(A, blockIdx.x, gridDim.x); }

template <bool RAYS>
__global__ __launch_bounds__(512) void k_decode_bwd_multi(MultiArgs MA)
{
    if (MA.sum_n > 0 && blockIdx.x == gridDim.x - 1) { block_sum(MA.sum_src, MA.sum_n, MA.sum_dst); return; }
    if constexpr (!RAYS) {
        if ((int)blockIdx.x >= MA.wg_end[MA.n - 1]) { sort_scan_body<2>(MA.scan, (int)blockIdx.x - MA.wg_end[MA.n - 1]); return; }
    }
    int r = 0;
    while (r < MA.n - 1 && (int)blockIdx.x >= MA.wg_end[r]) ++r;
    const int b0 = r == 0 ? 0 : MA.wg_end[r - 1];
    const int bid = blockIdx.x - b0, nb = MA.wg_end[r] - b0;
    const int sel = MA.which[r] * 2 + (MA.train[r] ? 1 : 0);
    switch (sel) {
    case 0: decode_bwd_body<0, RAYS>(MA.a[r], bid, nb); break;
    case 1: decode_bwd_train_any<0, RAYS>(MA.a[r], bid, nb); break;
    case 2: decode_bwd_body<1, RAYS>(MA.a[r], bid, nb); break;
    case 3: decode_bwd_train_any<1, RAYS>(MA.a[r], bid, nb); break;
    case 4: decode_bwd_body<2, RAYS>(MA.a[r], bid, nb); break;
    case 5: break;
    case 6: decode_bwd_body<3, RAYS>(MA.a[r], bid, nb); break;
    default: decode_bwd_train_any<3, RAYS>(MA.a[r], bid, nb); break;
    }
}

template <bool RAYS>
__global__ __launch_bounds__(512) void k_decode_bwd_multi_full(MultiArgs MA)
{
    if (MA.sum_n > 0 && blockIdx.x == gridDim.x - 1) { block_sum(MA.sum_src, MA.sum_n, MA.sum_dst); return; }
    int r = 0;
    while (r < MA.n - 1 && (int)blockIdx.x >= MA.wg_end[r]) ++r;
    const int b0 = r == 0 ? 0 : MA.wg_end[r - 1];
    const int bid = blockIdx.x - b0, nb = MA.wg_end[r] - b0;
    const int sel = MA.which[r] * 2 + (MA.train[r] ? 1 : 0);
    switch (sel) {
    case 0: decode_bwd_body<0, RAYS, 8, true>(MA.a[r], bid, nb); break;
    case 1: decode_bwd_train_body<0, RAYS, true>(MA.a[r], bid, nb); break;
    case 2: decode_bwd_body<1, RAYS, 8, true>(MA.a[r], bid, nb); break;
    case 3: decode_bwd_train_body<1, RAYS, true>(MA.a[r], bid, nb); break;
    case 4: decode_bwd_body<2, RAYS, 8, true>(MA.a[r], bid, nb); break;
    case 5: break;
    case 6: decode_bwd_body<3, RAYS, 8, true>(MA.a[r], bid, nb); break;
    default: decode_bwd_train_body<3, RAYS, true>(MA.a[r], bid, nb); break;
    }
}
```

Measured before the change: 14.42 million.

## Save trilinear grid features in forward and reuse them in trainable decoder backward

```diff
diff --git a/nice-slam-cpp_amd/csrc/nsk.hip b/nice-slam-cpp_amd/csrc/nsk.hip
--- a/nice-slam-cpp_amd/csrc/nsk.hip
+++ b/nice-slam-cpp_amd/csrc/nsk.hip
@@ -681,6 +681,7 @@
     Buf<float> z, occ[3], rgb4;
     Buf<unsigned long long> masks[4];
     Buf<f4> hsave[4];
+    Buf<f4> csave[4];
     int hsave_M[4] = {0, 0, 0, 0};
     Buf<float> g_raw, ray_loss;
     Buf<float> tmp_rgb, tmp_depth, tmp_var;
@@ -728,6 +729,7 @@
     int tune_frozen_cost_rays = 0;
     int tune_frozen_mid_pct = 100;
     int tune_no_frozen_kernel = 0;
+    int tune_no_feature_handoff = 0;
     const uint8_t* ray_mask = nullptr;
     struct DMax { const float* gt = nullptr; const uint8_t* keep = nullptr; int n = 0; } dmax;
     float* xextra = nullptr; size_t xextra_n = 0;
@@ -887,11 +889,17 @@
 #define SETB(W) \
     CHK(set_lds(k_decode_bwd<W, false>, bwd_lds_bytes(W, false))); CHK(set_lds(k_decode_bwd<W, true>, bwd_lds_bytes(W, false))); \
     CHK(set_lds(k_decode_bwd_train<W, false>, bwd_lds_bytes(W, true))); CHK(set_lds(k_decode_bwd_train<W, true>, bwd_lds_bytes(W, true)));
+#define SETH(W) \
+    CHK(set_lds(k_decode_bwd_train<W, false, true>, bwd_lds_bytes(W, true))); CHK(set_lds(k_decode_bwd_train<W, true, true>, bwd_lds_bytes(W, true)));
     SETB(0) SETB(1) SETB(2) SETB(3)
+    SETH(0) SETH(1) SETH(3)
 #undef SETB
+#undef SETH
     CHK(set_lds(k_median_thr, 16384 * 4));
     CHK(set_lds(k_decode_fwd_multi, 160 * 1024)); CHK(set_lds(k_decode_fwd_multi_bf16<8>, 160 * 1024)); CHK(set_lds(k_decode_fwd_multi_bf16<8, 2>, 160 * 1024)); CHK(set_lds(k_decode_fwd_multi_occ<8>, 160 * 1024));
     CHK(set_lds(k_decode_bwd_multi<false>, 160 * 1024 - 256)); CHK(set_lds(k_decode_bwd_multi<true>, 160 * 1024));
+    CHK(set_lds(k_decode_bwd_multi<false, true>, 160 * 1024 - 256)); CHK(set_lds(k_decode_bwd_multi<true, true>, 160 * 1024));
+    CHK(set_lds(k_decode_bwd_multi_full<false, true>, 160 * 1024)); CHK(set_lds(k_decode_bwd_multi_full<true, true>, 160 * 1024));
     CHK(set_lds(k_decode_bwd_frozen<false>, 160 * 1024 - 256));
     CHK(set_lds(k_decode_bwd_track, 160 * 1024)); CHK(set_lds(k_decode_bwd_multi_full<false>, 160 * 1024)); CHK(set_lds(k_decode_bwd_multi_full<true>, 160 * 1024));
     CHK(set_lds(k_decode_fwd_dump<0>, 160 * 1024)); CHK(set_lds(k_decode_fwd_dump<1>, 160 * 1024)); CHK(set_lds(k_decode_fwd_dump<2>, 160 * 1024));
@@ -952,6 +960,7 @@
     if (!strcmp(key, "frozen_cost")) { c->tune_frozen_cost = value; return 0; }
     if (!strcmp(key, "frozen_cost_rays")) { c->tune_frozen_cost_rays = value; return 0; }
     if (!strcmp(key, "no_frozen_kernel")) { c->tune_no_frozen_kernel = value; return 0; }
+    if (!strcmp(key, "no_feature_handoff")) { c->tune_no_feature_handoff = value; return 0; }
     if (!strcmp(key, "no_piggyback")) { c->tune_no_piggyback = value; return 0; }
     if (!strcmp(key, "frozen_mid_pct")) { if (value < 10 || value > 1000) return fail("nsk_set_tuning: frozen_mid_pct out of range"); c->tune_frozen_mid_pct = value; return 0; }
     if (!strcmp(key, "no_fused_median")) { c->tune_no_fused_median = value; return 0; }
@@ -1383,7 +1392,23 @@
 static int ensure_hsave(nsk_ctx* c, int w, int M)
 {
     const size_t tiles = (size_t)(M + 15) / 16 + 1;
-    return grow(c, c->ws.hsave[w], tiles * 10 * 64, "the saved block outputs", GROW_NO_CAPTURE | GROW_STALE_GRAPHS);
+    CHK(grow(c, c->ws.hsave[w], tiles * 10 * 64, "the saved block outputs", GROW_NO_CAPTURE | GROW_STALE_GRAPHS));
+    return grow(c, c->ws.csave[w], tiles * 2 * 64, "the saved grid features", GROW_NO_CAPTURE | GROW_STALE_GRAPHS);
+}
+static int attach_saves(nsk_ctx* c, DecArgs& A, int w, int M, bool save_masks)
+{
+    if (save_masks) c->ws.hsave_M[w] = 0;
+    if (!saves_h(c, w, save_masks)) return 0;
+    CHK(ensure_hsave(c, w, M));
+    A.hsave = c->ws.hsave[w]; A.csave = c->ws.csave[w]; c->ws.hsave_M[w] = M;
+    return 0;
+}
+static int use_saves(nsk_ctx* c, DecArgs& A, int w, int M)
+{
+    if (c->ws.hsave_M[w] != M) return fail("backward of trainable decoder %d: its forward must run with the decoder already trainable (block outputs not saved)", w);
+    A.hsave = c->ws.hsave[w];
+    A.csave = c->tune_no_feature_handoff ? nullptr : c->ws.csave[w].get();
+    return 0;
 }
 
 static const int STAGE_DEC[4][3] = {{0, -1, -1}, {1, -1, -1}, {1, 2, -1}, {1, 2, 3}};
@@ -1430,8 +1455,7 @@
     DecArgs A;
     fill_args(c, A, w, M, S, ro, rd, pts);
     A.masks = save_masks ? c->ws.masks[w] : nullptr;
-    if (save_masks) c->ws.hsave_M[w] = 0;
-    if (saves_h(c, w, save_masks)) { CHK(ensure_hsave(c, w, M)); A.hsave = c->ws.hsave[w]; c->ws.hsave_M[w] = M; }
+    CHK(attach_saves(c, A, w, M, save_masks));
     int ntasks = (M + 15) / 16;
     size_t lds = fwd_img_floats(w) * 4;
     int maxwg = c->num_cu;
@@ -1460,10 +1484,8 @@
     A.g_dec = train ? c->ws.dec_slabs : c->slab + c->dec[w].g_off;
     A.flags = flags;
     if (w != 0 && (!train || w != 2)) CHK(ensure_bimg16(c, w));
-    if (train && w != 2) {
-        if (c->ws.hsave_M[w] != M) return fail("backward of trainable decoder %d: its forward must run with the decoder already trainable (block outputs not saved)", w);
-        A.hsave = c->ws.hsave[w];
-    }
+    if (train && w != 2) CHK(use_saves(c, A, w, M));
+    const bool hand = A.csave != nullptr;
     int ntasks = (M + 15) / 16;
     size_t lds = bwd_lds_bytes(w, train);
     int grid = std::max(1, std::min((ntasks + 7) / 8, c->num_cu));
@@ -1472,16 +1494,18 @@
                                    "decode_bwd_coarse_train", "decode_bwd_middle_train", "decode_bwd_fine_train", "decode_bwd_color_train"};
     {
     ProfScope ps(c, names[w + (train ? 4 : 0)]);
-#define LB(W) \
-    if (train) { if (rays) k_decode_bwd_train<W, true><<<grid, 512, lds, c->stream>>>(A); else k_decode_bwd_train<W, false><<<grid, 512, lds, c->stream>>>(A); } \
-    else { if (rays) k_decode_bwd<W, true><<<grid, 512, lds, c->stream>>>(A); else k_decode_bwd<W, false><<<grid, 512, lds, c->stream>>>(A); }
+#define LT(W, H) { if (rays) k_decode_bwd_train<W, true, H><<<grid, 512, lds, c->stream>>>(A); else k_decode_bwd_train<W, false, H><<<grid, 512, lds, c->stream>>>(A); }
+#define LF(W) { if (rays) k_decode_bwd<W, true><<<grid, 512, lds, c->stream>>>(A); else k_decode_bwd<W, false><<<grid, 512, lds, c->stream>>>(A); }
+#define LB(W) if (!train) LF(W) else if (hand) LT(W, true) else LT(W, false)
     switch (w) {
     case 0: LB(0) break;
     case 1: LB(1) break;
-    case 2: LB(2) break;
+    case 2: if (!train) LF(2) else LT(2, false) break;
     default: LB(3) break;
     }
 #undef LB
+#undef LF
+#undef LT
     }
     HIPCHK(hipGetLastError());
     if (train) {
@@ -1592,10 +1616,9 @@
             const int w = STAGE_DEC[stage][r];
             fill_args(c, MA.a[r], w, M, S, ro, rd, nullptr);
             MA.a[r].masks = save_masks ? c->ws.masks[w] : nullptr;
-            if (save_masks) c->ws.hsave_M[w] = 0;
+            CHK(attach_saves(c, MA.a[r], w, M, save_masks));
             MA.which[r] = w;
         }
-        if (colour && saves_h(c, 3, save_masks)) { CHK(ensure_hsave(c, 3, M)); MA.a[2].hsave = c->ws.hsave[3]; c->ws.hsave_M[3] = M; }
         int cost[2] = {c->tune_fwd_occ_cost > 0 ? c->tune_fwd_occ_cost : 460, c->tune_fwd_color_cost > 0 ? c->tune_fwd_color_cost : fcost[3]};
         MA.n = colour ? 2 : 1;
         split_wgs_balanced(c->num_cu, (M + 15) / 16, MA.n, cost, MA.wg_end, 8);
@@ -1625,8 +1648,7 @@
         int w = STAGE_DEC[stage][r];
         fill_args(c, MA.a[r], w, M, S, ro, rd, nullptr);
         MA.a[r].masks = save_masks ? c->ws.masks[w] : nullptr;
-        if (save_masks) c->ws.hsave_M[w] = 0;
-        if (saves_h(c, w, save_masks)) { CHK(ensure_hsave(c, w, M)); MA.a[r].hsave = c->ws.hsave[w]; c->ws.hsave_M[w] = M; }
+        CHK(attach_saves(c, MA.a[r], w, M, save_masks));
         MA.which[r] = w; cost[r] = (w == 2 && c->tune_fwd_fine_cost > 0) ? c->tune_fwd_fine_cost : ((w == 3 && c->tune_fwd_color_cost > 0) ? c->tune_fwd_color_cost : fcost[w]);
         lds = std::max(lds, fwd_img_floats(w) * 4);
     }
@@ -2037,10 +2059,7 @@
         A.g_dec = train ? c->ws.dec_slabs : c->slab + c->dec[w].g_off;
         A.flags = flags & 0xffu;
         if (w != 0 && (!train || w != 2)) CHK(ensure_bimg16(c, w));
-        if (train && w != 2) {
-            if (c->ws.hsave_M[w] != M) return fail("backward of trainable decoder %d: its forward must run with the decoder already trainable (block outputs not saved)", w);
-            A.hsave = c->ws.hsave[w];
-        }
+        if (train && w != 2) CHK(use_saves(c, A, w, M));
         MA.which[n] = w; MA.train[n] = train ? 1 : 0;
         const int frozen_cost = rays ? (c->tune_frozen_cost_rays > 0 ? c->tune_frozen_cost_rays : 330) : (c->tune_frozen_cost > 0 ? c->tune_frozen_cost : 205);
         cost[n] = train ? 1000 : (w == 1 ? frozen_cost * c->tune_frozen_mid_pct / 100 : frozen_cost);
@@ -2062,6 +2081,7 @@
     }
     MA.n = n;
     const bool full = c->bwd_mode == 0;
+    const bool hand = train_role >= 0 && MA.a[train_role].csave != nullptr;
     const bool frozen_only = train_role == -1 && !rays && !c->tune_no_frozen_kernel && !full;
     if (train_role >= 0 && n > 1) split_wgs_train(c->num_cu, (M + 15) / 16, n, cost, train_role, MA.wg_end);
     else split_wgs_balanced(c->num_cu, (M + 15) / 16, n, cost, MA.wg_end, frozen_only ? NSK_FROZEN_NW : 8);
@@ -2087,11 +2107,17 @@
                 const int w = MA.which[r];
                 ldsf = std::max(ldsf, MA.train[r] ? (bwd_img_floats(w) + PN_FLOATS(2)) * 4 : bwd_img_floats(w) * 4 + 8 * 3840);
             }
-            if (rays) k_decode_bwd_multi_full<true><<<MA.wg_end[n - 1] + extra, 512, ldsf, c->stream>>>(MA);
+            if (hand) {
+                if (rays) k_decode_bwd_multi_full<true, true><<<MA.wg_end[n - 1] + extra, 512, ldsf, c->stream>>>(MA);
+                else k_decode_bwd_multi_full<false, true><<<MA.wg_end[n - 1] + extra, 512, ldsf, c->stream>>>(MA);
+            } else if (rays) k_decode_bwd_multi_full<true><<<MA.wg_end[n - 1] + extra, 512, ldsf, c->stream>>>(MA);
             else k_decode_bwd_multi_full<false><<<MA.wg_end[n - 1] + extra, 512, ldsf, c->stream>>>(MA);
         } else if (frozen_only) {
             const size_t lds16 = lds - 8 * 3840 + (size_t)NSK_FROZEN_NW * 3840;
             k_decode_bwd_frozen<false><<<MA.wg_end[n - 1] + scan_wgs + extra, 64 * NSK_FROZEN_NW, lds16, c->stream>>>(MA);
+        } else if (hand) {
+            if (rays) k_decode_bwd_multi<true, true><<<MA.wg_end[n - 1] + extra, 512, lds, c->stream>>>(MA);
+            else k_decode_bwd_multi<false, true><<<MA.wg_end[n - 1] + scan_wgs + extra, 512, lds, c->stream>>>(MA);
         } else if (rays) k_decode_bwd_multi<true><<<MA.wg_end[n - 1] + extra, 512, lds, c->stream>>>(MA);
         else k_decode_bwd_multi<false><<<MA.wg_end[n - 1] + scan_wgs + extra, 512, lds, c->stream>>>(MA);
     }
diff --git a/nice-slam-cpp_amd/csrc/nsk_bf16.h b/nice-slam-cpp_amd/csrc/nsk_bf16.h
--- a/nice-slam-cpp_amd/csrc/nsk_bf16.h
+++ b/nice-slam-cpp_amd/csrc/nsk_bf16.h
@@ -192,6 +192,7 @@
         embed<false>(imgf + I::P_BM, g, px, py, pz, C.xe, dummy);
         asm volatile("" ::: "memory");
         tri_gather_reduce(T, R, C.xc[0], C.xc[1]);
+        if (A.csave) save_c(A.csave, task, lane, C.xc[0], C.xc[1]);
         if constexpr (WHICH == 2) {
             Tri Tm;
             tri_setup(A.grid_mid, A.bound, px, py, pz, Tm);
diff --git a/nice-slam-cpp_amd/csrc/nsk_device.h b/nice-slam-cpp_amd/csrc/nsk_device.h
--- a/nice-slam-cpp_amd/csrc/nsk_device.h
+++ b/nice-slam-cpp_amd/csrc/nsk_device.h
@@ -705,6 +705,7 @@
     float* dump;
     const float* dyn_resid;
     int dyn_n;
+    f4* csave;
 };
 
 template <typename T>
@@ -755,6 +756,12 @@
     f4* dst = hsave + ((size_t)task * 10) * 64 + lane;
 #pragma unroll
     for (int l = 0; l < 5; ++l) { dst[(2 * l) * 64] = h[l][0]; dst[(2 * l + 1) * 64] = h[l][1]; }
+}
+
+__device__ __forceinline__ void save_c(f4* __restrict__ csave, int task, int lane, f4 c0, f4 c1)
+{
+    f4* dst = csave + ((size_t)task * 2) * 64 + lane;
+    dst[0] = c0; dst[64] = c1;
 }
 
 template <int WHICH, int NW = 8, bool DUMP = false>
@@ -783,6 +790,7 @@
         if constexpr (WHICH == 0) {
             ActC C;
             tri_gather(A.grid, T, g, C.xc[0], C.xc[1]);
+            if (A.csave) save_c(A.csave, task, lane, C.xc[0], C.xc[1]);
             coarse_forward(smem, lane, C);
             float out[1];
             mlp_output<1>(imgf + CoarseFwdImg::P_WO, imgf + CoarseFwdImg::P_BO, g, C.h[4], out);
@@ -797,6 +805,7 @@
             typedef MlpFwdImg<CQ> I;
             Act<CQ> C;
             tri_gather(A.grid, T, g, C.xc[0], C.xc[1]);
+            if (A.csave) save_c(A.csave, task, lane, C.xc[0], C.xc[1]);
             if constexpr (WHICH == 2) {
                 Tri Tm;
                 tri_setup(A.grid_mid, A.bound, px, py, pz, Tm);
diff --git a/nice-slam-cpp_amd/csrc/nsk_train.h b/nice-slam-cpp_amd/csrc/nsk_train.h
--- a/nice-slam-cpp_amd/csrc/nsk_train.h
+++ b/nice-slam-cpp_amd/csrc/nsk_train.h
@@ -224,13 +224,14 @@
 
 __device__ __forceinline__ void lds_barrier() { asm volatile("s_waitcnt lgkmcnt(0)\n\ts_barrier" ::: "memory"); }
 
-template <int WHICH, bool RAYS, bool FULL = false>
+template <int WHICH, bool RAYS, bool FULL = false, bool HAND = false>
 __device__ __forceinline__ void decode_bwd_train_body(const DecArgs& A, int bid, int nb)
 {
     constexpr bool XYZ = WHICH != 0;
     constexpr int CQ = WHICH == 2 ? 4 : 2;
     constexpr int OD = WHICH == 3 ? 4 : 1;
     constexpr bool SAVED = WHICH != 2;
+    static_assert(!HAND || SAVED, "the fine decoder's forward saves nothing: its backward gathers");
     constexpr bool H16 = XYZ && SAVED && !FULL;
     typedef MlpFwdImg<CQ> FI;
     typedef TrainPlan<WHICH> PL;
@@ -278,21 +279,25 @@
             const int tk = min(task, ntasks - 1);
             S_.mask = A.masks[(size_t)min(slot, A.M - 1) * 4 + g];
             S_.h4[0] = A.hsave[((size_t)tk * 10 + 8) * 64 + lane]; S_.h4[1] = A.hsave[((size_t)tk * 10 + 9) * 64 + lane];
+            if constexpr (HAND) { S_.xc[0] = A.csave[((size_t)tk * 2) * 64 + lane]; S_.xc[1] = A.csave[((size_t)tk * 2 + 1) * 64 + lane]; }
         }
     };
     auto stage_b = [&](Staged& S_) {
-        Tri T_;
-        tri_setup(A.grid, A.bound, S_.px, S_.py, S_.pz, T_);
-        tri_gather(A.grid, T_, g, S_.xc[0], S_.xc[1]);
-        if constexpr (WHICH == 2) {
-            Tri Tm;
-            tri_setup(A.grid_mid, A.bound, S_.px, S_.py, S_.pz, Tm);
-            tri_gather(A.grid_mid, Tm, g, S_.xc[CQ - 2], S_.xc[CQ - 1]);
+        if constexpr (!HAND) {
+            Tri T_;
+            tri_setup(A.grid, A.bound, S_.px, S_.py, S_.pz, T_);
+            tri_gather(A.grid, T_, g, S_.xc[0], S_.xc[1]);
+            if constexpr (WHICH == 2) {
+                Tri Tm;
+                tri_setup(A.grid_mid, A.bound, S_.px, S_.py, S_.pz, Tm);
+                tri_gather(A.grid_mid, Tm, g, S_.xc[CQ - 2], S_.xc[CQ - 1]);
+            }
         }
     };
     int mm_next = 0;
     if (iters > 0) { stage_a(0, slot_sample(A, slot_of(0)), nx); stage_b(nx); mm_next = slot_sample(A, slot_of(1)); }
     if constexpr (SAVED) asm volatile("" : "+v"(nx.h4[0]), "+v"(nx.h4[1]), "+v"(nx.gr), "+v"(nx.mask), "+v"(mm_next));
+    if constexpr (HAND) asm volatile("" : "+v"(nx.xc[0]), "+v"(nx.xc[1]));
     for (int it = 0; it < iters; ++it) {
         asm volatile("" ::: "memory");
         lane = lane0; asm volatile("" : "+v"(lane)); j = lane & 15; g = lane >> 4;
@@ -520,6 +525,7 @@
             stage_b(nx);
         }
         if constexpr (SAVED) asm volatile("" : "+v"(nx.h4[0]), "+v"(nx.h4[1]), "+v"(nx.gr), "+v"(nx.mask), "+v"(mm_next));
+        if constexpr (HAND) asm volatile("" : "+v"(nx.xc[0]), "+v"(nx.xc[1]));
         if (scat) {
             if (A.flags & 0x8000u) {
                 for (int w = 0; w < 8; ++w) { if (wave == w) { scatter_tile(A.grid, T, gc, lane, valid, scratch); asm volatile("s_waitcnt vmcnt(0)" ::: "memory"); } __syncthreads(); }
@@ -763,7 +769,7 @@
     (pn_job_flush<WHICH, Is, SKIP_DB>(g_dec, wave, lane, acc), ...);
 }
 
-template <int WHICH, bool RAYS>
+template <int WHICH, bool RAYS, bool HAND = false>
 __device__ __forceinline__ void decode_bwd_train_m_body(const DecArgs& A, int bid, int nb)
 {
     static_assert(WHICH == 1 || WHICH == 3, "merged-phase body: middle and colour decoders");
@@ -809,14 +815,18 @@
         const int tk = min(task, ntasks - 1);
         S_.mask = ld32<unsigned long long>(A.masks, ((unsigned)min(slot, A.M - 1) * 4u + (unsigned)g) * 8u);
         S_.h4[0] = A.hsave[((size_t)tk * 10 + 8) * 64 + lane]; S_.h4[1] = A.hsave[((size_t)tk * 10 + 9) * 64 + lane];
+        if constexpr (HAND) { S_.xc[0] = A.csave[((size_t)tk * 2) * 64 + lane]; S_.xc[1] = A.csave[((size_t)tk * 2 + 1) * 64 + lane]; }
     };
     Tri Tn; GatherRaw GR;
+    (void)Tn; (void)GR;
     auto stage_b1 = [&](Staged& S_) {
         sample_finish(A, S_.r, S_.px, S_.py, S_.pz);
-        tri_setup(A.grid, A.bound, S_.px, S_.py, S_.pz, Tn);
-        tri_gather_issue<true>(A.grid, Tn, g, GR);
+        if constexpr (!HAND) {
+            tri_setup(A.grid, A.bound, S_.px, S_.py, S_.pz, Tn);
+            tri_gather_issue<true>(A.grid, Tn, g, GR);
+        }
     };
-    auto stage_b2 = [&](Staged& S_) { tri_gather_reduce(Tn, GR, S_.xc[0], S_.xc[1]); };
+    auto stage_b2 = [&](Staged& S_) { if constexpr (!HAND) tri_gather_reduce(Tn, GR, S_.xc[0], S_.xc[1]); };
     int mm_next = 0;
     {
         const f4* src = reinterpret_cast<const f4*>(A.bimg16);
@@ -832,6 +842,7 @@
         if (iters > 0) { stage_b1(nx); stage_b2(nx); mm_next = slot_sample(A, slot_of(1)); }
     }
     asm volatile("" : "+v"(nx.h4[0]), "+v"(nx.h4[1]), "+v"(nx.gr), "+v"(nx.mask), "+v"(mm_next));
+    if constexpr (HAND) asm volatile("" : "+v"(nx.xc[0]), "+v"(nx.xc[1]));
     f4 accB[2] = {(f4)(0.f), (f4)(0.f)};
     (void)accB;
     for (int it = 0; it < iters; ++it) {
@@ -1036,6 +1047,7 @@
         }
         stage_b2(nx);
         asm volatile("" : "+v"(nx.h4[0]), "+v"(nx.h4[1]), "+v"(nx.gr), "+v"(nx.mask), "+v"(mm_next), "+v"(nx.xc[0]), "+v"(nx.xc[1]));
+        if constexpr (HAND && !RAYS) lds_barrier();
         if (scat) {
             if (A.flags & 0x8000u) {
                 for (int w = 0; w < 8; ++w) { if (wave == w) { scatter_tile(A.grid, T, gc, lane, valid, scratch); asm volatile("s_waitcnt vmcnt(0)" ::: "memory"); } __syncthreads(); }
@@ -1067,17 +1079,17 @@
     }
 }
 
-template <int WHICH, bool RAYS>
+template <int WHICH, bool RAYS, bool HAND = false>
 __device__ __forceinline__ void decode_bwd_train_any(const DecArgs& A, int bid, int nb)
 {
-    if constexpr (WHICH == 1 || WHICH == 3) decode_bwd_train_m_body<WHICH, RAYS>(A, bid, nb);
-    else decode_bwd_train_body<WHICH, RAYS>(A, bid, nb);
-}
-
-template <int WHICH, bool RAYS>
-__global__ __launch_bounds__(512) void k_decode_bwd_train(DecArgs A) { decode_bwd_train_any<WHICH, RAYS>(A, blockIdx.x, gridDim.x); }
-
-template <bool RAYS>
+    if constexpr (WHICH == 1 || WHICH == 3) decode_bwd_train_m_body<WHICH, RAYS, HAND>(A, bid, nb);
+    else decode_bwd_train_body<WHICH, RAYS, false, HAND>(A, bid, nb);
+}
+
+template <int WHICH, bool RAYS, bool HAND = false>
+__global__ __launch_bounds__(512) void k_decode_bwd_train(DecArgs A) { decode_bwd_train_any<WHICH, RAYS, HAND>(A, blockIdx.x, gridDim.x); }
+
+template <bool RAYS, bool HAND = false>
 __global__ __launch_bounds__(512) void k_decode_bwd_multi(MultiArgs MA)
 {
     if (MA.sum_n > 0 && blockIdx.x == gridDim.x - 1) { block_sum(MA.sum_src, MA.sum_n, MA.sum_dst); return; }
@@ -1091,17 +1103,17 @@
     const int sel = MA.which[r] * 2 + (MA.train[r] ? 1 : 0);
     switch (sel) {
     case 0: decode_bwd_body<0, RAYS>(MA.a[r], bid, nb); break;
-    case 1: decode_bwd_train_any<0, RAYS>(MA.a[r], bid, nb); break;
+    case 1: decode_bwd_train_any<0, RAYS, HAND>(MA.a[r], bid, nb); break;
     case 2: decode_bwd_body<1, RAYS>(MA.a[r], bid, nb); break;
-    case 3: decode_bwd_train_any<1, RAYS>(MA.a[r], bid, nb); break;
+    case 3: decode_bwd_train_any<1, RAYS, HAND>(MA.a[r], bid, nb); break;
     case 4: decode_bwd_body<2, RAYS>(MA.a[r], bid, nb); break;
     case 5: break;
     case 6: decode_bwd_body<3, RAYS>(MA.a[r], bid, nb); break;
-    default: decode_bwd_train_any<3, RAYS>(MA.a[r], bid, nb); break;
-    }
-}
-
-template <bool RAYS>
+    default: decode_bwd_train_any<3, RAYS, HAND>(MA.a[r], bid, nb); break;
+    }
+}
+
+template <bool RAYS, bool HAND = false>
 __global__ __launch_bounds__(512) void k_decode_bwd_multi_full(MultiArgs MA)
 {
     if (MA.sum_n > 0 && blockIdx.x == gridDim.x - 1) { block_sum(MA.sum_src, MA.sum_n, MA.sum_dst); return; }
@@ -1112,12 +1124,12 @@
     const int sel = MA.which[r] * 2 + (MA.train[r] ? 1 : 0);
     switch (sel) {
     case 0: decode_bwd_body<0, RAYS, 8, true>(MA.a[r], bid, nb); break;
-    case 1: decode_bwd_train_body<0, RAYS, true>(MA.a[r], bid, nb); break;
+    case 1: decode_bwd_train_body<0, RAYS, true, HAND>(MA.a[r], bid, nb); break;
     case 2: decode_bwd_body<1, RAYS, 8, true>(MA.a[r], bid, nb); break;
-    case 3: decode_bwd_train_body<1, RAYS, true>(MA.a[r], bid, nb); break;
+    case 3: decode_bwd_train_body<1, RAYS, true, HAND>(MA.a[r], bid, nb); break;
     case 4: decode_bwd_body<2, RAYS, 8, true>(MA.a[r], bid, nb); break;
     case 5: break;
     case 6: decode_bwd_body<3, RAYS, 8, true>(MA.a[r], bid, nb); break;
-    default: decode_bwd_train_body<3, RAYS, true>(MA.a[r], bid, nb); break;
-    }
-}
+    default: decode_bwd_train_body<3, RAYS, true, HAND>(MA.a[r], bid, nb); break;
+    }
+}
```

Result: no change. 14.55 million (median of 6 runs) (+0.9%).
